# LLaVA-VL/LLaVA-Plus-Codebase

Measured on NVIDIA H100. Metric: prefill+decode tokens/s, higher is better.
Workload: dtype bf16

## Files before the change

llava-plus-codebase_b200/csrc/decode_mega.cu:

```cuda
#include <limits.h>
#include <math.h>

#include "common.cuh"
#include "kernels.h"

namespace b2 {
namespace {

constexpr int MK_CONS_WARPS = 16;
constexpr int MK_CONS = MK_CONS_WARPS * 32;
constexpr int MK_PROD_WARPS = 4;
constexpr int MK_THREADS = MK_CONS + 32 * MK_PROD_WARPS;
constexpr int MK_D = 128;
constexpr int MK_U = 4;
constexpr int MK_KT = 2048;
constexpr int MK_ROW_PAD = 64;
constexpr int MK_ROW_STRIDE = MK_KT * 2 + MK_ROW_PAD;
constexpr int MK_TILE_BYTES = 8 * MK_ROW_STRIDE;
constexpr int MK_MAXNB = 32;
constexpr int MK_MAXL = 48;
constexpr int MK_MAX_STAGES = 12;

__device__ __forceinline__ void unpack8(const uint4& u, float (&f)[8]) {
    f[0] = bf16_lo(u.x); f[1] = bf16_hi(u.x); f[2] = bf16_lo(u.y); f[3] = bf16_hi(u.y);
    f[4] = bf16_lo(u.z); f[5] = bf16_hi(u.z); f[6] = bf16_lo(u.w); f[7] = bf16_hi(u.w);
}
__device__ __forceinline__ uint4 ldcg16(const void* p) { return __ldcg(reinterpret_cast<const uint4*>(p)); }

__device__ __forceinline__ void cons_sync() { asm volatile("bar.sync 1, %0;" ::"n"(MK_CONS) : "memory"); }

__device__ __forceinline__ void grid_sync(unsigned int* counter, unsigned int target) {
    cons_sync();
    if (threadIdx.x == 0) {
        asm volatile("red.release.gpu.global.add.u32 [%0], 1;" ::"l"(counter) : "memory");
        unsigned int cur, spins = 0;
        do {
            asm volatile("ld.acquire.gpu.global.u32 %0, [%1];" : "=r"(cur) : "l"(counter) : "memory");
            if (++spins > (1u << 26)) asm volatile("trap;");
        } while ((int)(cur - target) < 0);
    }
    cons_sync();
}

__device__ __forceinline__ void bulk_g2s(void* smem_dst, const void* gsrc, uint32_t bytes, uint64_t* bar) {
    asm volatile("cp.async.bulk.shared::cluster.global.mbarrier::complete_tx::bytes [%0], [%1], %2, [%3];" ::"r"(
                     smem_u32(smem_dst)),
                 "l"(gsrc), "r"(bytes), "r"(smem_u32(bar))
                 : "memory");
}

struct GemvCtx {
    const __nv_bfloat16* W;
    int K, act;
    int u_lo, nu;
    int nb;
    int nchunk;
};
struct PhaseIO {
    const __nv_bfloat16* xin;
    const __nv_bfloat16* gamma;
    const __nv_bfloat16* residual;
    void* out;
    int ld_out, out_fp32;
};

__device__ __forceinline__ int mk_phys_row(const GemvCtx& c, int rb, int g, bool& valid) {
    if (c.act == ACT_SWIGLU) {
        const int lc = rb * 4 + (g & 3);
        valid = lc < c.nu;
        const int ch = c.u_lo + lc;
        return (ch >> 6) * 128 + (ch & 63) + ((g >> 2) ? 64 : 0);
    }
    const int lr = rb * 8 + g;
    valid = lr < c.nu;
    return c.u_lo + lr;
}

__device__ __forceinline__ int mk_rows_in_block(const GemvCtx& c, int rb) {
    if (c.act == ACT_SWIGLU) return 2 * min(4, c.nu - rb * 4);
    return min(8, c.nu - rb * 8);
}

__device__ __forceinline__ bool mk_is_attention(const MegaParams& p, int ph) { return ph % 5 == 1 && ph < 5 * p.L; }

__device__ __forceinline__ PhaseIO mk_phase_io(const MegaParams& p, const MegaLayer* layers, int ph) {
    PhaseIO c;
    const int l = ph / 5, k = ph % 5;
    c.gamma = nullptr; c.residual = nullptr; c.out_fp32 = 0;
    if (l >= p.L) { c.xin = p.x; c.gamma = p.final_norm; c.out = p.logits; c.ld_out = p.V; c.out_fp32 = 1; }
    else if (k <= 1) { c.xin = p.x; c.gamma = layers[l].ln1; c.out = p.qkv; c.ld_out = 3 * p.h; }
    else if (k == 2) { c.xin = p.attn; c.residual = p.x; c.out = p.x; c.ld_out = p.h; }
    else if (k == 3) { c.xin = p.x; c.gamma = layers[l].ln2; c.out = p.act; c.ld_out = p.I; }
    else { c.xin = p.act; c.residual = p.x; c.out = p.x; c.ld_out = p.h; }
    return c;
}
__device__ __forceinline__ GemvCtx mk_phase_ctx(const MegaParams& p, const MegaLayer* layers, int ph) {
    GemvCtx c;
    const int l = ph / 5, k = ph % 5;
    int N;
    c.act = ACT_NONE;
    if (l >= p.L) { c.W = p.lm_head; N = p.V; c.K = p.h; }
    else if (k <= 1) { c.W = layers[l].wqkv; N = 3 * p.h; c.K = p.h; }
    else if (k == 2) { c.W = layers[l].wo; N = p.h; c.K = p.h; }
    else if (k == 3) { c.W = layers[l].wgu; N = 2 * p.I; c.K = p.h; c.act = ACT_SWIGLU; }
    else { c.W = layers[l].wd; N = p.h; c.K = p.I; }
    const long long units = c.act == ACT_SWIGLU ? (N >> 1) : N;
    c.u_lo = (int)((units * blockIdx.x) / gridDim.x);
    c.nu = (int)((units * (blockIdx.x + 1)) / gridDim.x) - c.u_lo;
    c.nb = c.act == ACT_SWIGLU ? (c.nu + 3) >> 2 : (c.nu + 7) >> 3;
    c.nchunk = (c.K + MK_KT - 1) / MK_KT;
    return c;
}

template <int NB>
__device__ __forceinline__ void mk_prologue(const PhaseIO& c, int K, int B, float eps, int tid, int lane, int warp,
                                            __nv_bfloat16* xs, float (*s_red)[NB], float* s_rstd,
                                            const __nv_bfloat16* gamma_smem) {
    const int nvec = K >> 3;
    float ss[NB];
#pragma unroll
    for (int b = 0; b < NB; ++b) ss[b] = 0.f;
    for (int i = tid; i < nvec; i += MK_CONS) {
#pragma unroll
        for (int b = 0; b < NB; ++b) {
            uint4 u = make_uint4(0, 0, 0, 0);
            if (b < B) u = ldcg16(c.xin + (size_t)b * K + i * 8);
            *reinterpret_cast<uint4*>(xs + (size_t)b * K + i * 8) = u;
            if (c.gamma != nullptr) {
                float f[8];
                unpack8(u, f);
#pragma unroll
                for (int e = 0; e < 8; ++e) ss[b] += f[e] * f[e];
            }
        }
    }
    if (c.gamma != nullptr) {
#pragma unroll
        for (int b = 0; b < NB; ++b) {
            const float v = warp_sum(ss[b]);
            if (lane == 0) s_red[warp][b] = v;
        }
        cons_sync();
        if (tid < NB) {
            float t = 0.f;
            for (int i = 0; i < MK_CONS_WARPS; ++i) t += s_red[i][tid];
            s_rstd[tid] = rsqrtf(t / K + eps);
        }
        cons_sync();
        if (gamma_smem != nullptr) asm volatile("cp.async.wait_all;" ::: "memory");
        const __nv_bfloat16* gsrc = gamma_smem != nullptr ? gamma_smem : c.gamma;
        for (int i = tid; i < nvec; i += MK_CONS) {
            float gf[8];
            unpack8(*reinterpret_cast<const uint4*>(gsrc + i * 8), gf);
#pragma unroll
            for (int b = 0; b < NB; ++b) {
                uint4* px = reinterpret_cast<uint4*>(xs + (size_t)b * K + i * 8);
                float f[8], o[8];
                unpack8(*px, f);
                const float rstd = s_rstd[b];
#pragma unroll
                for (int e = 0; e < 8; ++e) o[e] = gf[e] * round_bf16(f[e] * rstd);
                *px = make_uint4(pack_bf16(o[0], o[1]), pack_bf16(o[2], o[3]), pack_bf16(o[4], o[5]),
                                 pack_bf16(o[6], o[7]));
            }
        }
    }
    cons_sync();
}

template <int NB>
__device__ __forceinline__ void mk_prologue_fast(const PhaseIO& c, int K, float eps, int tid, int lane, int warp,
                                                 __nv_bfloat16* xs, float (*s_red)[NB], const uint4 (&gpre)[2]) {
    const int nvec = K >> 3;
    if (c.gamma == nullptr) {
        constexpr int J = 3;
        for (int i0 = 0; i0 < nvec; i0 += J * MK_CONS) {
            uint4 u[NB][J];
#pragma unroll
            for (int j = 0; j < J; ++j) {
                const int idx = i0 + j * MK_CONS + tid;
#pragma unroll
                for (int b = 0; b < NB; ++b)
                    u[b][j] = idx < nvec ? ldcg16(c.xin + (size_t)b * K + idx * 8) : make_uint4(0, 0, 0, 0);
            }
#pragma unroll
            for (int j = 0; j < J; ++j) {
                const int idx = i0 + j * MK_CONS + tid;
                if (idx < nvec) {
#pragma unroll
                    for (int b = 0; b < NB; ++b) *reinterpret_cast<uint4*>(xs + (size_t)b * K + idx * 8) = u[b][j];
                }
            }
        }
        cons_sync();
        return;
    }
    uint4 u[NB][2];
    float ss[NB];
#pragma unroll
    for (int b = 0; b < NB; ++b) ss[b] = 0.f;
#pragma unroll
    for (int j = 0; j < 2; ++j) {
        const int idx = j * MK_CONS + tid;
#pragma unroll
        for (int b = 0; b < NB; ++b)
            u[b][j] = idx < nvec ? ldcg16(c.xin + (size_t)b * K + idx * 8) : make_uint4(0, 0, 0, 0);
    }
#pragma unroll
    for (int j = 0; j < 2; ++j) {
#pragma unroll
        for (int b = 0; b < NB; ++b) {
            float f[8];
            unpack8(u[b][j], f);
#pragma unroll
            for (int e = 0; e < 8; ++e) ss[b] += f[e] * f[e];
        }
    }
#pragma unroll
    for (int b = 0; b < NB; ++b) {
        const float v = warp_sum(ss[b]);
        if (lane == 0) s_red[warp][b] = v;
    }
    cons_sync();
    float rstd[NB];
#pragma unroll
    for (int b = 0; b < NB; ++b) {
        float t = 0.f;
#pragma unroll
        for (int i = 0; i < MK_CONS_WARPS; ++i) t += s_red[i][b];
        rstd[b] = rsqrtf(t / K + eps);
    }
#pragma unroll
    for (int j = 0; j < 2; ++j) {
        const int idx = j * MK_CONS + tid;
        if (idx < nvec) {
            float gf[8];
            unpack8(gpre[j], gf);
#pragma unroll
            for (int b = 0; b < NB; ++b) {
                float f[8], o[8];
                unpack8(u[b][j], f);
#pragma unroll
                for (int e = 0; e < 8; ++e) o[e] = gf[e] * round_bf16(f[e] * rstd[b]);
                *reinterpret_cast<uint4*>(xs + (size_t)b * K + idx * 8) =
                    make_uint4(pack_bf16(o[0], o[1]), pack_bf16(o[2], o[3]), pack_bf16(o[4], o[5]), pack_bf16(o[6], o[7]));
            }
        }
    }
    cons_sync();
}

__device__ __forceinline__ bool mk_gamma_preload(const MegaParams& p, const MegaLayer* layers, int ph, int n_phases,
                                                 int tid, uint4 (&gpre)[2]) {
    if (ph >= n_phases || mk_is_attention(p, ph)) return false;
    const PhaseIO io = mk_phase_io(p, layers, ph);
    const int nvec = p.h >> 3;
    if (io.gamma == nullptr || nvec > 2 * MK_CONS) return false;
#pragma unroll
    for (int j = 0; j < 2; ++j) {
        const int idx = j * MK_CONS + tid;
        gpre[j] = idx < nvec ? __ldg(reinterpret_cast<const uint4*>(io.gamma) + idx) : make_uint4(0, 0, 0, 0);
    }
    return true;
}

__device__ __forceinline__ void mk_mma(float (&c)[4], uint32_t a0, uint32_t a2, uint32_t b0, uint32_t b1) {
    asm volatile(
        "mma.sync.aligned.m16n8k16.row.col.f32.bf16.bf16.f32 {%0,%1,%2,%3}, {%4,%5,%6,%7}, {%8,%9}, {%0,%1,%2,%3};"
        : "+f"(c[0]), "+f"(c[1]), "+f"(c[2]), "+f"(c[3])
        : "r"(a0), "r"(0u), "r"(a2), "r"(0u), "r"(b0), "r"(b1));
}

template <int NB>
__device__ __forceinline__ float mk_row_value(const float* s_gpart, int rb, int b, int r) {
    float v = 0.f;
#pragma unroll
    for (int ww = 0; ww < MK_CONS_WARPS; ++ww) v += s_gpart[(((size_t)ww * MK_MAXNB + rb) * NB + b) * 8 + r];
    return v;
}

template <int NB>
__device__ __forceinline__ void mk_epilogue(const MegaParams& p, const MegaLayer* layers, int ph, const GemvCtx& c,
                                            int B, int tid, const float* s_gpart, float res_pref, bool have_res_pref) {
    const PhaseIO io = mk_phase_io(p, layers, ph);
    if (c.act == ACT_SWIGLU) {
        const int nch = c.nu;
        for (int idx = tid; idx < nch * B; idx += MK_CONS) {
            const int b = idx / nch, r = idx - b * nch;
            const int rb = r >> 2, q = r & 3;
            const float gt = mk_row_value<NB>(s_gpart, rb, b, q);
            const float up = mk_row_value<NB>(s_gpart, rb, b, q + 4);
            reinterpret_cast<__nv_bfloat16*>(io.out)[(size_t)b * io.ld_out + (size_t)c.u_lo + r] =
                __float2bfloat16_rn(gt / (1.0f + __expf(-gt)) * up);
        }
    } else {
        const int nr = c.nu;
        for (int idx = tid; idx < nr * B; idx += MK_CONS) {
            const int b = idx / nr, r = idx - b * nr;
            float y = mk_row_value<NB>(s_gpart, r >> 3, b, r & 7);
            const size_t o = (size_t)b * io.ld_out + (size_t)c.u_lo + r;
            if (io.residual != nullptr) y += have_res_pref ? res_pref : __bfloat162float(__ldcg(io.residual + o));
            if (io.out_fp32) reinterpret_cast<float*>(io.out)[o] = y;
            else reinterpret_cast<__nv_bfloat16*>(io.out)[o] = __float2bfloat16_rn(y);
        }
    }
}

__device__ __forceinline__ void mk_attention(const MegaParams& p, const MegaLayer& Lw, int tid, int lane, int warp,
                                             float (*s_part)[MK_D + 2], int* s_flag, const float* s_cos,
                                             const float* s_sin) {
    const int h = p.h, H = p.H;
    const int pairs = p.B * H;
    const int grid = gridDim.x;
    const int G = pairs <= grid ? grid / pairs : 1;
    const int hw = lane >> 4, c = lane & 15;
    const int split = pairs <= grid ? (int)blockIdx.x % G : 0;
    for (int pair = pairs <= grid ? (int)blockIdx.x / G : (int)blockIdx.x; pair < pairs;
         pair += (pairs <= grid ? pairs : grid)) {
        const int head = pair % H, b = pair / H;
        const int pos = p.cur_len[b];
        const int total = pos + 1;
        const int cchunk = (total + G - 1) / G;
        const int cb = split * cchunk;
        const int ce = min(cb + cchunk, total);
        const int wchunk = (max(ce - cb, 0) + MK_CONS_WARPS - 1) / MK_CONS_WARPS;
        const int k_begin = cb + warp * wchunk;
        const int k_end = min(k_begin + wchunk, ce);
        const __nv_bfloat16* qrow = p.qkv + (size_t)b * 3 * h + head * MK_D;
        float qreg[8], knew[8], vnew[8];
        {
            float qa[8], qb[8], ka[8], kb[8];
            unpack8(ldcg16(qrow + c * 8), qa);
            unpack8(ldcg16(qrow + (c ^ 8) * 8), qb);
            unpack8(ldcg16(qrow + h + c * 8), ka);
            unpack8(ldcg16(qrow + h + (c ^ 8) * 8), kb);
            unpack8(ldcg16(qrow + 2 * h + c * 8), vnew);
            const float sign = (c < 8) ? -1.f : 1.f;
#pragma unroll
            for (int e = 0; e < 8; ++e) {
                const int i = ((c & 7) * 8 + e);
                const float cbf = s_cos[b * 64 + i], sbf = s_sin[b * 64 + i];
                qreg[e] = round_bf16(round_bf16(qa[e] * cbf) + round_bf16(sign * qb[e] * sbf));
                knew[e] = round_bf16(round_bf16(ka[e] * cbf) + round_bf16(sign * kb[e] * sbf));
            }
        }
        const size_t cbase = ((size_t)b * H + head) * p.Smax * MK_D;
        if (pos >= k_begin && pos < k_end && hw == 0) {
            *reinterpret_cast<uint4*>(Lw.kcache + cbase + (size_t)pos * MK_D + c * 8) =
                make_uint4(pack_bf16(knew[0], knew[1]), pack_bf16(knew[2], knew[3]),
                           pack_bf16(knew[4], knew[5]), pack_bf16(knew[6], knew[7]));
            *reinterpret_cast<uint4*>(Lw.vcache + cbase + (size_t)pos * MK_D + c * 8) =
                make_uint4(pack_bf16(vnew[0], vnew[1]), pack_bf16(vnew[2], vnew[3]),
                           pack_bf16(vnew[4], vnew[5]), pack_bf16(vnew[6], vnew[7]));
        }
        float m_run = -INFINITY, l_run = 0.f, av[8];
#pragma unroll
        for (int e = 0; e < 8; ++e) av[e] = 0.f;
        const __nv_bfloat16* kb_ = Lw.kcache + cbase + c * 8;
        const __nv_bfloat16* vb_ = Lw.vcache + cbase + c * 8;
        for (int kbase = k_begin; kbase < k_end; kbase += 2 * MK_U) {
            uint4 kraw[MK_U], vraw[MK_U];
#pragma unroll
            for (int u = 0; u < MK_U; ++u) {
                const int key = kbase + hw + 2 * u;
                if (key < k_end && key != pos) {
                    kraw[u] = ld_stream_16(kb_ + (size_t)key * MK_D);
                    vraw[u] = ld_stream_16(vb_ + (size_t)key * MK_D);
                } else {
                    kraw[u] = make_uint4(0, 0, 0, 0);
                    vraw[u] = make_uint4(0, 0, 0, 0);
                }
            }
#pragma unroll
            for (int u = 0; u < MK_U; ++u) {
                const int key = kbase + hw + 2 * u;
                float kf[8], vf[8];
                unpack8(kraw[u], kf);
                unpack8(vraw[u], vf);
                if (key == pos) {
#pragma unroll
                    for (int e = 0; e < 8; ++e) { kf[e] = knew[e]; vf[e] = vnew[e]; }
                }
                float dot = 0.f;
#pragma unroll
                for (int e = 0; e < 8; ++e) dot += qreg[e] * kf[e];
                dot += __shfl_xor_sync(0xffffffffu, dot, 8);
                dot += __shfl_xor_sync(0xffffffffu, dot, 4);
                dot += __shfl_xor_sync(0xffffffffu, dot, 2);
                dot += __shfl_xor_sync(0xffffffffu, dot, 1);
                if (key < k_end) {
                    const float sc = dot * p.scale_log2;
                    const float m_new = fmaxf(m_run, sc);
                    const float corr = exp2f(m_run - m_new);
                    const float pr = exp2f(sc - m_new);
                    l_run = l_run * corr + pr;
#pragma unroll
                    for (int e = 0; e < 8; ++e) av[e] = av[e] * corr + pr * vf[e];
                    m_run = m_new;
                }
            }
        }
        {
            const float m_o = __shfl_xor_sync(0xffffffffu, m_run, 16);
            const float l_o = __shfl_xor_sync(0xffffffffu, l_run, 16);
            const float m_c = fmaxf(m_run, m_o);
            const float w_s = (m_run == -INFINITY) ? 0.f : exp2f(m_run - m_c);
            const float w_o = (m_o == -INFINITY) ? 0.f : exp2f(m_o - m_c);
#pragma unroll
            for (int e = 0; e < 8; ++e) {
                const float a_o = __shfl_xor_sync(0xffffffffu, av[e], 16);
                av[e] = av[e] * w_s + a_o * w_o;
            }
            l_run = l_run * w_s + l_o * w_o;
            m_run = m_c;
        }
        if (hw == 0) {
#pragma unroll
            for (int e = 0; e < 8; ++e) s_part[warp][c * 8 + e] = av[e];
            if (c == 0) { s_part[warp][MK_D] = m_run; s_part[warp][MK_D + 1] = l_run; }
        }
        cons_sync();
        float m_cta = -INFINITY, l_cta = 0.f, o_cta = 0.f;
        if (tid < MK_D) {
#pragma unroll
            for (int i = 0; i < MK_CONS_WARPS; ++i) m_cta = fmaxf(m_cta, s_part[i][MK_D]);
#pragma unroll
            for (int i = 0; i < MK_CONS_WARPS; ++i) {
                const float ms = s_part[i][MK_D];
                const float wgt = (ms == -INFINITY) ? 0.f : exp2f(ms - m_cta);
                l_cta += s_part[i][MK_D + 1] * wgt;
                o_cta += s_part[i][tid] * wgt;
            }
        }
        if (G == 1) {
            if (tid < MK_D) p.attn[(size_t)b * h + head * MK_D + tid] = __float2bfloat16_rn(o_cta / l_cta);
        } else {
            float* part = p.attn_partial + ((size_t)pair * G + split) * (MK_D + 2);
            if (tid < MK_D) {
                part[tid] = o_cta;
                if (tid == 0) { part[MK_D] = m_cta; part[MK_D + 1] = l_cta; }
            }
            __threadfence();
            cons_sync();
            if (tid == 0) *s_flag = (atomicAdd(&p.attn_counters[pair], 1) == G - 1) ? 1 : 0;
            cons_sync();
            if (*s_flag) {
                __threadfence();
                if (tid < MK_D) {
                    const float* pb = p.attn_partial + (size_t)pair * G * (MK_D + 2);
                    float m_all = -INFINITY;
                    for (int sidx = 0; sidx < G; ++sidx) m_all = fmaxf(m_all, __ldcg(pb + (size_t)sidx * (MK_D + 2) + MK_D));
                    float l_all = 0.f, o_all = 0.f;
                    for (int sidx = 0; sidx < G; ++sidx) {
                        const float ms = __ldcg(pb + (size_t)sidx * (MK_D + 2) + MK_D);
                        const float wgt = (ms == -INFINITY) ? 0.f : exp2f(ms - m_all);
                        l_all += __ldcg(pb + (size_t)sidx * (MK_D + 2) + MK_D + 1) * wgt;
                        o_all += __ldcg(pb + (size_t)sidx * (MK_D + 2) + tid) * wgt;
                    }
                    p.attn[(size_t)b * h + head * MK_D + tid] = __float2bfloat16_rn(o_all / l_all);
                    if (tid == 0) p.attn_counters[pair] = 0;
                }
            }
        }
        cons_sync();
    }
}

struct TileCursor {
    GemvCtx c;
    int ph, rb, kc;
    uint32_t tile;
    bool valid;
};
__device__ __forceinline__ void cursor_seek(TileCursor& t, const MegaParams& p, const MegaLayer* layers, int n_phases) {
    while (t.ph < n_phases) {
        if (!mk_is_attention(p, t.ph)) {
            t.c = mk_phase_ctx(p, layers, t.ph);
            if (t.c.nb > 0) { t.rb = 0; t.kc = 0; t.valid = true; return; }
        }
        ++t.ph;
    }
    t.valid = false;
}
__device__ __forceinline__ void cursor_begin(TileCursor& t, const MegaParams& p, const MegaLayer* layers, int n_phases) {
    t.ph = 0; t.tile = 0; t.rb = 0; t.kc = 0;
    cursor_seek(t, p, layers, n_phases);
}
__device__ __forceinline__ void cursor_next(TileCursor& t, const MegaParams& p, const MegaLayer* layers, int n_phases) {
    ++t.tile;
    if (++t.kc < t.c.nchunk) return;
    t.kc = 0;
    if (++t.rb < t.c.nb) return;
    ++t.ph;
    cursor_seek(t, p, layers, n_phases);
}
__device__ __forceinline__ void prefetch_l2_line(const void* gsrc) {
    asm volatile("prefetch.global.L2 [%0];" ::"l"(gsrc) : "memory");
}
__device__ __forceinline__ void bulk_prefetch_l2(const void* gsrc, uint32_t bytes) {
    asm volatile("cp.async.bulk.prefetch.L2.global [%0], %1;" ::"l"(gsrc), "r"(bytes) : "memory");
}

template <int NB>
__global__ void __launch_bounds__(MK_THREADS, 1) decode_mega_kernel(MegaParams p, int n_stages) {
    extern __shared__ __align__(128) uint8_t mk_smem[];
    uint8_t* ring = mk_smem;
    __nv_bfloat16* xs = reinterpret_cast<__nv_bfloat16*>(ring + (size_t)n_stages * MK_TILE_BYTES);
    float* s_gpart = reinterpret_cast<float*>(reinterpret_cast<uint8_t*>(xs) + (size_t)NB * (p.h > p.I ? p.h : p.I) * 2);
    uint64_t* full_bar = reinterpret_cast<uint64_t*>(s_gpart + (size_t)MK_CONS_WARPS * MK_MAXNB * NB * 8);
    uint64_t* empty_bar = full_bar + MK_MAX_STAGES;
    __shared__ float s_red[MK_CONS_WARPS][NB];
    __shared__ float s_rstd[NB];
    __shared__ float s_av[MK_CONS_WARPS];
    __shared__ int s_ai[MK_CONS_WARPS];
    __shared__ float s_part[MK_CONS_WARPS][MK_D + 2];
    __shared__ int s_flag;
    __shared__ float s_cos[NB * 64], s_sin[NB * 64];
    __shared__ __align__(16) MegaLayer s_layers[MK_MAXL];

    const int tid = threadIdx.x, lane = tid & 31, warp = tid >> 5;
    const int B = p.B;
    const int n_phases = 5 * p.L + 1;

    {
        const uint4* src = reinterpret_cast<const uint4*>(p.layers);
        uint4* dst = reinterpret_cast<uint4*>(s_layers);
        for (int i = tid; i < p.L * (int)(sizeof(MegaLayer) / 16); i += MK_THREADS) dst[i] = src[i];
        if (tid == 0) {
            for (int s = 0; s < n_stages; ++s) {
                mbar_init(&full_bar[s], 1);
                mbar_init(&empty_bar[s], MK_CONS_WARPS);
            }
            fence_barrier_init();
        }
        __syncthreads();
    }

    if (warp >= MK_CONS_WARPS) {
        const uint32_t pw = (uint32_t)(warp - MK_CONS_WARPS);
        const uint32_t ahead = (uint32_t)p.l2_ahead;
        TileCursor cp, pf;
        cursor_begin(cp, p, s_layers, n_phases);
        cursor_begin(pf, p, s_layers, n_phases);
        while (cp.valid) {
            if (cp.tile % (uint32_t)MK_PROD_WARPS == pw) {
                if (ahead != 0) {
                    while (pf.valid && pf.tile < cp.tile + ahead) cursor_next(pf, p, s_layers, n_phases);
                    if (pf.valid) {
                        const uint32_t pbytes = (uint32_t)min(MK_KT, pf.c.K - pf.kc * MK_KT) * 2u;
                        if (p.l2_mode == 2) {
                            bool pvalid;
                            const int pfrow = mk_phys_row(pf.c, pf.rb, lane & 7, pvalid);
                            if (lane < 8 && pvalid)
                                bulk_prefetch_l2(pf.c.W + (size_t)pfrow * pf.c.K + (size_t)pf.kc * MK_KT, pbytes);
                        } else {
                            bool pvalid;
                            const int pfrow = mk_phys_row(pf.c, pf.rb, lane >> 2, pvalid);
                            if (pvalid) {
                                const char* base = reinterpret_cast<const char*>(pf.c.W + (size_t)pfrow * pf.c.K +
                                                                                 (size_t)pf.kc * MK_KT);
                                for (uint32_t off = (uint32_t)(lane & 3) * 128u; off < pbytes; off += 512u)
                                    prefetch_l2_line(base + off);
                            }
                        }
                    }
                }
                const uint32_t stage = cp.tile % (uint32_t)n_stages;
                const uint32_t parity = (cp.tile / (uint32_t)n_stages) & 1u;
                const uint32_t row_bytes = (uint32_t)min(MK_KT, cp.c.K - cp.kc * MK_KT) * 2u;
                if (lane == 0) {
                    mbar_wait(&empty_bar[stage], parity ^ 1u);
                    mbar_arrive_expect_tx(&full_bar[stage], (uint32_t)mk_rows_in_block(cp.c, cp.rb) * row_bytes);
                }
                __syncwarp();
                bool row_valid;
                const int prow = mk_phys_row(cp.c, cp.rb, lane & 7, row_valid);
                if (lane < 8 && row_valid)
                    bulk_g2s(ring + (size_t)stage * MK_TILE_BYTES + (size_t)lane * MK_ROW_STRIDE,
                             cp.c.W + (size_t)prow * cp.c.K + (size_t)cp.kc * MK_KT, row_bytes, &full_bar[stage]);
            }
            cursor_next(cp, p, s_layers, n_phases);
        }
        return;
    }

    for (int i = tid; i < B * 64; i += MK_CONS) {
        const int b = i >> 6, f = i & 63;
        const float inv_freq = exp2f(-(2.0f * f / MK_D) * log2f(p.theta));
        float sv, cv;
        sincosf((float)p.cur_len[b] * inv_freq, &sv, &cv);
        s_cos[i] = round_bf16(cv);
        s_sin[i] = round_bf16(sv);
    }
    if (blockIdx.x < B) {
        int t = p.tok[blockIdx.x];
        t = t < 0 ? 0 : (t >= p.V ? p.V - 1 : t);
        const uint4* src = reinterpret_cast<const uint4*>(p.embed + (size_t)t * p.h);
        uint4* dst = reinterpret_cast<uint4*>(p.x + (size_t)blockIdx.x * p.h);
        for (int i = tid; i < p.h / 8; i += MK_CONS) dst[i] = src[i];
    }
    uint4 gpre[2] = {make_uint4(0, 0, 0, 0), make_uint4(0, 0, 0, 0)};
    bool gpre_ok = p.fast_prologue != 0 && mk_gamma_preload(p, s_layers, 0, n_phases, tid, gpre);
    __nv_bfloat16* gsm = xs + (size_t)NB * p.h;
    const bool gsm_fits = p.gamma_smem != 0 && (size_t)(NB + 1) * p.h <= (size_t)NB * (p.h > p.I ? p.h : p.I);
    auto gamma_prefetch = [&](int ph) -> bool {
        if (!gsm_fits || ph >= n_phases || mk_is_attention(p, ph)) return false;
        const PhaseIO io = mk_phase_io(p, s_layers, ph);
        if (io.gamma == nullptr) return false;
        for (int i = tid; i < (p.h >> 3); i += MK_CONS)
            asm volatile("cp.async.cg.shared.global [%0], [%1], 16;" ::"r"(smem_u32(gsm + i * 8)), "l"(io.gamma + i * 8) : "memory");
        asm volatile("cp.async.commit_group;" ::: "memory");
        return true;
    };
    bool gsm_ok = gamma_prefetch(0);
    unsigned int bar_target = p.bar_base + gridDim.x;
    grid_sync(p.bar_count, bar_target);

    const bool tracing = p.trace != nullptr && blockIdx.x == 0 && tid == 0;
    const int g = lane >> 2, t4 = lane & 3;
    uint32_t tile = 0;
#pragma unroll 1
    for (int ph = 0; ph < n_phases; ++ph) {
        if (tracing) p.trace[ph * 4 + 0] = clock64();
        if (mk_is_attention(p, ph)) {
            mk_attention(p, s_layers[ph / 5], tid, lane, warp, s_part, &s_flag, s_cos, s_sin);
        } else {
            const GemvCtx c = mk_phase_ctx(p, s_layers, ph);
            const PhaseIO io = mk_phase_io(p, s_layers, ph);
            const bool have_res = io.residual != nullptr && c.nu * B <= MK_CONS;
            float res_pref = 0.f;
            if (have_res && tid < c.nu * B) {
                const int b = tid / c.nu, r = tid - b * c.nu;
                res_pref = __bfloat162float(__ldcg(io.residual + (size_t)b * io.ld_out + (size_t)c.u_lo + r));
            }
            if (p.fast_prologue != 0 && (io.gamma == nullptr || gpre_ok))
                mk_prologue_fast<NB>(io, c.K, p.eps, tid, lane, warp, xs, s_red, gpre);
            else
                mk_prologue<NB>(io, c.K, B, p.eps, tid, lane, warp, xs, s_red, s_rstd, gsm_ok ? gsm : nullptr);
            if (tracing) p.trace[ph * 4 + 1] = clock64();
#pragma unroll 1
            for (int rb = 0; rb < c.nb; ++rb) {
                float acc[4] = {0.f, 0.f, 0.f, 0.f}, acc2[4] = {0.f, 0.f, 0.f, 0.f};
#pragma unroll 1
                for (int kc = 0; kc < c.nchunk; ++kc, ++tile) {
                    const uint32_t stage = tile % (uint32_t)n_stages;
                    const uint32_t parity = (tile / (uint32_t)n_stages) & 1u;
                    const int nk32 = min(MK_KT, c.K - kc * MK_KT) >> 5;
                    mbar_wait(&full_bar[stage], parity);
                    const uint8_t* trow = ring + (size_t)stage * MK_TILE_BYTES + (size_t)g * MK_ROW_STRIDE + t4 * 16;
                    const __nv_bfloat16* xrow = xs + (size_t)g * c.K + (size_t)kc * MK_KT + t4 * 8;
#pragma unroll 4
                    for (int k32 = warp; k32 < nk32; k32 += MK_CONS_WARPS) {
                        const uint4 wv = *reinterpret_cast<const uint4*>(trow + k32 * 64);
                        uint4 xv = make_uint4(0, 0, 0, 0);
                        if (g < B) xv = *reinterpret_cast<const uint4*>(xrow + k32 * 32);
                        mk_mma(acc, xv.x, xv.y, wv.x, wv.y);
                        mk_mma(acc2, xv.z, xv.w, wv.z, wv.w);
                    }
                    __syncwarp();
                    if (lane == 0) mbar_arrive(&empty_bar[stage]);
                }
                if (g < NB)
                    *reinterpret_cast<float2*>(s_gpart + (((size_t)warp * MK_MAXNB + rb) * NB + g) * 8 + t4 * 2) =
                        make_float2(acc[0] + acc2[0], acc[1] + acc2[1]);
            }
            cons_sync();
            if (tracing) p.trace[ph * 4 + 2] = clock64();
            mk_epilogue<NB>(p, s_layers, ph, c, B, tid, s_gpart, res_pref, have_res);
        }
        if (tracing) p.trace[ph * 4 + 3] = clock64();
        gpre_ok = p.fast_prologue != 0 && mk_gamma_preload(p, s_layers, ph + 1, n_phases, tid, gpre);
        gsm_ok = gamma_prefetch(ph + 1);
        bar_target += gridDim.x;
        grid_sync(p.bar_count, bar_target);
    }
    if (tracing) p.trace[n_phases * 4] = clock64();

    if (blockIdx.x < B) {
        const int b = blockIdx.x;
        const float* row = p.logits + (size_t)b * p.V;
        float best = -INFINITY;
        int bi = INT_MAX;
        for (int i = tid; i < p.V; i += MK_CONS) {
            const float v = __ldcg(row + i);
            if (v == v && (bi == INT_MAX || v > best)) { best = v; bi = i; }
        }
#pragma unroll
        for (int o = 16; o > 0; o >>= 1) {
            const float ov = __shfl_xor_sync(0xffffffffu, best, o);
            const int oi = __shfl_xor_sync(0xffffffffu, bi, o);
            if (ov > best || (ov == best && oi < bi)) { best = ov; bi = oi; }
        }
        if (lane == 0) { s_av[warp] = best; s_ai[warp] = bi; }
        cons_sync();
        if (warp == 0) {
            best = lane < MK_CONS_WARPS ? s_av[lane] : -INFINITY;
            bi = lane < MK_CONS_WARPS ? s_ai[lane] : INT_MAX;
#pragma unroll
            for (int o = 16; o > 0; o >>= 1) {
                const float ov = __shfl_xor_sync(0xffffffffu, best, o);
                const int oi = __shfl_xor_sync(0xffffffffu, bi, o);
                if (ov > best || (ov == best && oi < bi)) { best = ov; bi = oi; }
            }
            if (lane == 0) {
                const int tk = bi == INT_MAX ? 0 : bi;
                p.tok[b] = tk;
                p.out_tokens[(size_t)(*p.step_counter) * B + b] = tk;
                if (p.rows == nullptr || p.rows[b].active) p.cur_len[b] += 1;
                if (p.ring != nullptr) {
                    const int pub = p.sstate->pub_counter, tag0 = p.sstate->tag;
                    if (tag0 != 0) {
                        const int tag = 1 + (tag0 - 1 + pub / p.ring_cap) % 2047;
                        reinterpret_cast<volatile int32_t*>(p.ring)[(size_t)(pub % p.ring_cap) * B + b] = (tag << 20) | (tk & 0xFFFFF);
                        __threadfence_system();
                    }
                }
            }
        }
    }
    cons_sync();
    if (tid == 0) {
        __threadfence();
        if (atomicAdd(p.done_count, 1u) == gridDim.x - 1) {
            *p.done_count = 0u;
            *p.step_counter += 1;
            if (p.ring != nullptr) p.sstate->pub_counter += 1;
        }
    }
}

size_t mega_fixed_bytes(int NB, int h, int I) {
    return (size_t)NB * (h > I ? h : I) * 2 + (size_t)MK_CONS_WARPS * MK_MAXNB * NB * 8 * 4 + 2 * MK_MAX_STAGES * 8;
}
size_t mega_static_bytes(int NB) {
    return (size_t)(MK_CONS_WARPS + 1) * NB * 4 + MK_CONS_WARPS * (MK_D + 2 + 2) * 4 + NB * 512 +
           MK_MAXL * sizeof(MegaLayer) + 1024;
}
int mega_stages(int NB, int h, int I) {
    const long long avail = 227 * 1024 - (long long)mega_fixed_bytes(NB, h, I) - (long long)mega_static_bytes(NB);
    long long s = avail / MK_TILE_BYTES;
    return (int)(s > MK_MAX_STAGES ? MK_MAX_STAGES : s);
}

}

bool decode_mega_fits(int B, int h, int I) {
    if (B < 1 || B > 2) return false;
    return mega_stages(B, h, I) >= 4;
}

int decode_mega(const MegaParams& p, cudaStream_t stream) {
    B2_CHECK_ARG(p.B >= 1 && p.B <= 2, "decode_mega: batch must be 1..2");
    B2_CHECK_ARG(p.L <= MK_MAXL, "decode_mega: %d layers exceed the shared layer table (%d)", p.L, MK_MAXL);
    B2_CHECK_ARG(p.h % 256 == 0 && p.I % 256 == 0 && p.V % 8 == 0 && p.h / p.H == MK_D,
                 "decode_mega: unsupported dims h=%d I=%d V=%d H=%d", p.h, p.I, p.V, p.H);
    {
        const int grid = num_sms();
        const int nmax = p.V > 3 * p.h ? (p.V > 2 * p.I ? p.V : 2 * p.I) : (3 * p.h > 2 * p.I ? 3 * p.h : 2 * p.I);
        B2_CHECK_ARG((nmax / 8 + grid - 1) / grid + 1 <= MK_MAXNB,
                     "decode_mega: %d output rows per CTA exceed the shared-memory block table", nmax / grid);
    }
    const int NB = p.B;
    const int stages = mega_stages(NB, p.h, p.I);
    B2_CHECK_ARG(stages >= 4, "decode_mega: shared memory too small for the weight ring (B=%d h=%d I=%d)", p.B, p.h, p.I);
    const size_t smem = (size_t)stages * MK_TILE_BYTES + mega_fixed_bytes(NB, p.h, p.I);
    void* fn = NB == 1 ? (void*)decode_mega_kernel<1> : (void*)decode_mega_kernel<2>;
    static size_t attr_smem[3] = {0, 0, 0};
    if (smem > attr_smem[NB]) {
        B2_CUDA_CHECK(cudaFuncSetAttribute(fn, cudaFuncAttributeMaxDynamicSharedMemorySize, (int)smem));
        attr_smem[NB] = smem;
    }
    MegaParams pp = p;
    int n_stages = stages;
    void* args[] = {&pp, &n_stages};
    B2_CUDA_CHECK(cudaLaunchCooperativeKernel(fn, dim3(num_sms()), dim3(MK_THREADS), args, smem, stream));
    B2_LAUNCH_CHECK();
    return 0;
}

}
```

llava-plus-codebase_b200/csrc/kernels.h:

```cpp
#pragma once
#include <cuda_bf16.h>
#include <cuda_runtime.h>
#include <stdint.h>

namespace b2 {

enum { ACT_NONE = 0, ACT_QUICK_GELU = 1, ACT_GELU_ERF = 2, ACT_SWIGLU = 3, ACT_ROPE_QKV = 4 };

struct RopeQkv {
    const void* table = nullptr;
    void* kcache = nullptr;
    void* vcache = nullptr;
    int S = 0, H = 0, Smax = 0;
    const int32_t* pos0 = nullptr;
};
enum { DT_BF16 = 0, DT_F16 = 1, DT_F32 = 2 };

int num_sms();

struct GemmArgs {
    const void* A = nullptr; int lda = 0;
    const void* W = nullptr; int ldw = 0;
    const void* bias = nullptr;
    const void* residual = nullptr; int ld_res = 0;
    void* out = nullptr; int ld_out = 0; int out_fp32 = 0;
    int M = 0, N = 0, K = 0;
    int act = ACT_NONE;
    int bn_override = 0;
    RopeQkv rope;
};
int gemm_bf16(const GemmArgs& g, cudaStream_t stream);
int projector_fused_bf16(const void* X, int ldx, const void* W1, const void* b1, const void* W2, const void* b2, void* H,
                         void* out, int ld_out, int M, int K1, int N1, int N2, int* row_done, cudaStream_t stream);
int gemm_bf16_2cta(const GemmArgs& g, cudaStream_t stream);

struct SkinnyArgs {
    const void* x = nullptr; int ldx = 0;
    const void* W = nullptr; int ldw = 0;
    const void* residual = nullptr; int ld_res = 0;
    void* out = nullptr; int ld_out = 0; int out_fp32 = 0;
    int B = 0, N = 0, K = 0;
    int act = ACT_NONE;
    float* partial = nullptr; size_t partial_bytes = 0;
    int* counters = nullptr;
    const float* w_scale = nullptr;
    const float* x_scale = nullptr;
};
int gemm_skinny_bf16(const SkinnyArgs& g, cudaStream_t stream);
int gemm_skinny_fp8(const SkinnyArgs& g, cudaStream_t stream);
size_t gemm_skinny_workspace_bytes(int B, int N, int K);
size_t gemm_skinny_counter_bytes(int N);

int quantize_rows_e4m3(const void* x, int64_t ldx, int rows, int K, void* q, int64_t ldq, float* scale, cudaStream_t stream);
int rmsnorm_quant_e4m3(const void* x, int64_t x_row_stride, const void* gamma, void* q, int64_t ldq, float* scale, int rows,
                       int cols, float eps, cudaStream_t stream);

struct GemvArgs {
    const void* x = nullptr; int64_t ldx = 0;
    const void* W = nullptr; int ldw = 0;
    const void* norm_gamma = nullptr; float eps = 0.f;
    const void* residual = nullptr; int ld_res = 0;
    void* out = nullptr; int ld_out = 0; int out_fp32 = 0;
    int B = 0, N = 0, K = 0;
    int act = ACT_NONE;
};
int gemv_bf16(const GemvArgs& g, cudaStream_t stream);
bool gemv_fits(int B, int N, int K, int act);

int quantize_nf4(const void* w, int64_t ldw, int N, int K, void* q, float* absmax, int gemv_order, cudaStream_t stream);
struct Nf4Matrix {
    const void* q = nullptr; const float* absmax = nullptr;
    void* out = nullptr;
    int N = 0, K = 0;
};
int dequantize_nf4(const Nf4Matrix* mats, int n, int gemv_order, cudaStream_t stream);
int gemv_nf4(const GemvArgs& g, const void* q, const float* absmax, cudaStream_t stream);
bool gemv_nf4_fits(int B, int N, int K, int act);

int layernorm_bf16(const void* x, const void* gamma, const void* beta, void* y, int rows, int cols, float eps,
                   cudaStream_t stream);
int rmsnorm_bf16(const void* x, int64_t x_row_stride, const void* gamma, void* y, int rows, int cols, float eps,
                 cudaStream_t stream);
int rmsnorm_gather_bf16(const void* x, const int32_t* row_index, const void* gamma, void* y, int rows, int cols,
                        float eps, cudaStream_t stream);

int vit_im2col(const void* pixels, void* out, int B, int img, int patch, int kpad, cudaStream_t stream);
int vit_embed_ln(const void* patch_out, const void* cls, const void* pos, const void* gamma, const void* beta,
                 void* hidden, int B, int P, int D, float eps, cudaStream_t stream);
int vit_drop_cls(const void* hidden, void* out, int B, int P, int D, cudaStream_t stream);

struct FlashArgs {
    const void* q = nullptr; int64_t q_bs = 0, q_ts = 0, q_hs = 0;
    const void* k = nullptr; int64_t k_bs = 0, k_ts = 0, k_hs = 0;
    const void* v = nullptr; int64_t v_bs = 0, v_ts = 0, v_hs = 0;
    void* o = nullptr;       int64_t o_bs = 0, o_ts = 0, o_hs = 0;
    const int32_t* seq_lens = nullptr;
    const int32_t* pos0 = nullptr;
    int Skv = 0;
    int B = 0, H = 0, S = 0, D = 0;
    int causal = 0;
    float scale = 1.f;
};
int flash_attn_bf16(const FlashArgs& a, cudaStream_t stream);
int flash_attn_tc_bf16(const FlashArgs& a, cudaStream_t stream);
int flash_attn_mma_bf16(const FlashArgs& a, cudaStream_t stream);

int rope_table_build(void* table, int Smax, int D, float theta, cudaStream_t stream);
int rope_kv_write(void* qkv, void* kcache, void* vcache, int B, int S, int H, int D, int Smax, float theta,
                  cudaStream_t stream, const int32_t* pos0 = nullptr);

struct DecodeAttnArgs {
    const void* qkv = nullptr;
    void* kcache = nullptr; void* vcache = nullptr;
    float* kscale = nullptr; float* vscale = nullptr;
    const int32_t* cur_len = nullptr;
    void* out = nullptr;
    float* partial = nullptr;
    int32_t* counters = nullptr;
    int B = 0, H = 0, D = 128, Smax = 0, nsplit = 1;
    float theta = 10000.f, scale = 1.f;
};
int decode_attn_ctas_per_sm();
int decode_attn_bf16(const DecodeAttnArgs& a, cudaStream_t stream);
int decode_attn_e4m3_ctas_per_sm();
int decode_attn_e4m3(const DecodeAttnArgs& a, cudaStream_t stream);
int kv_quantize_e4m3(const void* ksrc, const void* vsrc, void* k8, void* v8, float* kscale, float* vscale,
                     const int32_t* seq_lens, int B, int S, int H, int D, int Smax, cudaStream_t stream,
                     const int32_t* pos0 = nullptr, int S_src = 0);
int kv_dequantize_e4m3(const void* k8, const void* v8, const float* kscale, const float* vscale, const int32_t* pos0, void* kdst,
                       void* vdst, int B, int H, int Smax, int S_dst, cudaStream_t stream);

struct MegaLayer {
    const __nv_bfloat16 *ln1, *wqkv, *wo, *ln2, *wgu, *wd;
    __nv_bfloat16 *kcache, *vcache;
};
struct MegaParams {
    const MegaLayer* layers = nullptr;
    int L = 0, h = 0, I = 0, H = 0, V = 0, B = 0, Smax = 0, nsplit = 1;
    const __nv_bfloat16 *embed = nullptr, *final_norm = nullptr, *lm_head = nullptr;
    int32_t *tok = nullptr, *cur_len = nullptr, *out_tokens = nullptr, *step_counter = nullptr;
    __nv_bfloat16 *x = nullptr, *qkv = nullptr, *attn = nullptr, *act = nullptr;
    float* logits = nullptr;
    float* attn_partial = nullptr;
    int32_t* attn_counters = nullptr;
    unsigned int *bar_count = nullptr, *done_count = nullptr;
    unsigned int bar_base = 0;
    float eps = 1e-5f, theta = 10000.f, scale_log2 = 1.f;
    int l2_ahead = 0;
    int l2_mode = 1;
    int fast_prologue = 0;
    int gamma_smem = 0;
    long long* trace = nullptr;
    struct SampleState* sstate = nullptr;
    int32_t* ring = nullptr;
    int ring_cap = 0;
    const struct RowState* rows = nullptr;
};
int decode_mega(const MegaParams& p, cudaStream_t stream);
bool decode_mega_fits(int B, int h, int I);

struct SampleState {
    int do_sample;
    float temperature, top_p;
    int top_k;
    unsigned long long seed;
    int tag;
    int pub_counter;
    unsigned int done;
    int per_row;
};
struct RowState {
    int active;
    int do_sample; float temperature, top_p; int top_k;
    unsigned long long seed;
    int index;
};
enum { SP_SELECT = 1,
       SP_WRITE_OUT = 2,
       SP_BUMP = 4 };
int sample_state_set(SampleState* st_dev, const SampleState& v, cudaStream_t stream);
int sample_publish(const float* logits, int V, int B, SampleState* st_dev, RowState* rows_dev, int32_t* tok, int32_t* out_tokens,
                   int32_t* step_counter, int32_t* cur_len, int32_t* ring_dev, int ring_cap, int flags, int step_offset,
                   cudaStream_t stream);
int row_state_set(RowState* row_dev, const RowState& v, int32_t* tok_dev, int token, cudaStream_t stream);

size_t beam_topk_workspace_bytes(int B, int nb, int K);
int beam_topk(const float* logits, const int32_t* row_of_beam, const float* beam_scores, int B, int nb, int V, int K,
              void* workspace, float* out_scores, int32_t* out_tokens, int32_t* out_beams, cudaStream_t stream);
struct KvCopyPairs {
    static constexpr int kMax = 64;
    int32_t src[kMax], dst[kMax], end[kMax];
};
int kv_copy_slots(void* k, void* v, float* kscale, float* vscale, const int32_t* src, const int32_t* dst, const int32_t* end, int n,
                  int row_begin, int L, int H, int max_batch, int pitch, int row_bytes, int32_t* len_dev, cudaStream_t stream);

struct PreprocessArgs {
    const uint8_t* img = nullptr; int H = 0, W = 0;
    int pad_top = 0, pad_left = 0; uint8_t bg[3] = {0, 0, 0};
    const int32_t *h_bounds = nullptr, *h_kk = nullptr; int h_ksize = 0, h_identity = 0;
    const int32_t *v_bounds = nullptr, *v_kk = nullptr; int v_ksize = 0, v_identity = 0;
    int y0 = 0, rows = 0;
    int x_lo = 0, y_lo = 0;
    int cols = 0, out = 0;
    uint8_t* tmp = nullptr;
    float mean[3] = {0, 0, 0}, stdv[3] = {1, 1, 1}, rescale = 1.f / 255.f;
    void* pixels = nullptr;
    uint8_t* u8_out = nullptr;
};
int preprocess_clip_image(const PreprocessArgs& a, cudaStream_t stream);

int splice_embed(const int32_t* src_index, const void* table, const void* feats, void* out, int rows, int h, int vocab,
                 int n_feat_rows, int* err_flag, cudaStream_t stream);
int splice_index(const long long* ids, int B, int Lt, int k_per_row, const int32_t* feat_offsets_host, int n_img, int image_token,
                 int S, int32_t* src_index, int* err_flag, cudaStream_t stream);
int embed_tokens(const int32_t* tokens, const void* table, void* out, int rows, int h, int vocab, int* err_flag,
                 cudaStream_t stream);
enum { B2_ERR_TOKEN_RANGE = 1, B2_ERR_IMAGE_ROW_RANGE = 2, B2_ERR_SPLICE_SLOTS = 4 };
int argmax_f32(const float* logits, int B, int V, int32_t* out, cudaStream_t stream);
struct I32Pack { int32_t v[128]; };
int set_i32_pairs(int32_t* dst_a, const int32_t* a_host, int32_t* dst_b, const int32_t* b_host, int n, cudaStream_t stream);
int add_i32(int32_t* x, int n, int delta, cudaStream_t stream);
int convert_to_bf16(const void* src, int src_dtype, void* dst, int64_t n, cudaStream_t stream);
int interleave_gate_up(const void* gate, const void* up, void* out, int I, int h, cudaStream_t stream);
int store_token(const int32_t* src, int32_t* dst_base, const int32_t* step_counter, int B, cudaStream_t stream);

}
```

llava-plus-codebase_b200/csrc/model.cu:

```cuda
#include <cuda_fp16.h>
#include <limits.h>
#include <stdarg.h>
#include <stdio.h>
#include <stdlib.h>
#include <string.h>
#include <time.h>

#include <atomic>
#include <utility>
#include <mutex>
#include <string>
#include <vector>

#include "../../include/b2llava.h"
#include "common.cuh"
#include "kernels.h"

namespace b2 {

static thread_local char g_err[1024] = {0};
unsigned long long g_launch_count = 0;

bool pdl_enabled() {
    const char* e = getenv("B2_PDL");
    return !(e != nullptr && e[0] == '0');
}

void set_error(const char* fmt, ...) {
    va_list ap;
    va_start(ap, fmt);
    vsnprintf(g_err, sizeof(g_err), fmt, ap);
    va_end(ap);
}

namespace {
typedef __nv_bfloat16 bf16;

struct DevBuf {
    void* p = nullptr;
    size_t bytes = 0;
    int alloc(size_t n) {
        free();
        if (n == 0) return 0;
        cudaError_t e = cudaMalloc(&p, n);
        if (e != cudaSuccess) {
            p = nullptr;
            set_error("cudaMalloc(%zu bytes) failed: %s", n, cudaGetErrorString(e));
            return -2;
        }
        bytes = n;
        return 0;
    }
    void free() {
        if (p) cudaFree(p);
        p = nullptr;
        bytes = 0;
    }
    template <typename T>
    T* as() const { return reinterpret_cast<T*>(p); }
};

struct VitLayer {
    DevBuf ln1_g, ln1_b, wqkv, bqkv, wo, bo, ln2_g, ln2_b, w1, b1, w2, b2;
    unsigned qkv_w = 0, qkv_b = 0;
};
struct LlamaLayer {
    DevBuf ln1, wqkv, wo, ln2, wgu, wd;
    unsigned qkv_parts = 0;
    DevBuf wqkv8, wo8, wgu8, wd8, s_qkv, s_o, s_gu, s_d;
    DevBuf tmp_gate, tmp_up;
    DevBuf q_qkv, a_qkv, q_o, a_o, q_gu, a_gu, q_d, a_d;
    bool has_gate = false, has_up = false;
};
}
}

using namespace b2;

struct b2_model {
    b2_model_desc d;
    int device = 0;
    std::mutex mu;
    bool finalized = false;
    int P = 0, T = 0, kpad = 0, vit_live = 0, vit_hd = 64, hd = 128;
    DevBuf patch_w, cls, pos, pre_g, pre_b;
    std::vector<VitLayer> vit;
    DevBuf p0_w, p0_b, p2_w, p2_b;
    DevBuf embed, final_norm, lm_head;
    std::vector<LlamaLayer> ll;
    int* err_host = nullptr;
    int* err_dev = nullptr;
    cudaEvent_t ws_event = nullptr;
    cudaStream_t ws_stream = nullptr;
    bool ws_valid = false;
    DevBuf v_col, v_patch, v_hidden, v_xn, v_qkv, v_attn, v_mlp, v_feats, p_mid, p_done;
    DevBuf x, xn, qkv, attn, act, last_idx, xlast, logits, splice_idx;
    DevBuf chunk_pos;
    DevBuf enc_pixels, enc_out;
    std::vector<cudaGraphExec_t> enc_graph;
    std::vector<char> enc_warm;
    cudaStream_t enc_stream = nullptr;
    cudaEvent_t enc_fork = nullptr, enc_join = nullptr;
    int enc_launches = 0;
    bool fp8_decode = false;
    DevBuf lm_head8, s_head, xq8, xscale;
    DevBuf kstage, vstage;
    bool nf4 = false;
    DevBuf nf4_scratch;
    std::atomic<int> kv_live{0};
};

struct b2_kv {
    b2_model* m = nullptr;
    int max_batch = 0, max_seq = 0;
    int dtype = B2_KV_BF16;
    int pitch = 0;
    DevBuf k, v;
    DevBuf kscale, vscale;
    DevBuf len_dev, tok, step_counter, out_tokens, attn_partial, attn_counters;
    DevBuf sk_partial, sk_counters;
    std::vector<int32_t> len_host;
    int out_capacity = 0;
    cudaGraphExec_t graph = nullptr;
    int graph_B = 0;
    unsigned int mega_bar_base = 0;
    DevBuf mega_layers, mega_sync;
    DevBuf rope_tab;
    cudaStream_t own_stream = nullptr;
    cudaEvent_t ev_fork = nullptr, ev_join = nullptr;
    int warm_B = 0;
    DevBuf sstate;
    SampleState samp_host = {};
    bool samp_valid = false;
    int32_t* ring_host = nullptr;
    int32_t* ring_dev = nullptr;
    int ring_cap = 0;
    int epoch = 0;
    int stream_B = 0, stream_tag = 0, stream_scheduled = 0;
    DevBuf rows_dev;
    std::vector<RowState> rows_host;
    DevBuf beam_in, beam_ws, beam_out;
    bool counted = false;
    bool e4m3() const { return dtype == B2_KV_E4M3; }
    size_t elem_bytes() const { return e4m3() ? 1 : 2; }
    size_t layer_rows() const { return (size_t)max_batch * m->d.heads * pitch; }
    size_t layer_stride() const { return layer_rows() * m->hd; }
    char* k_layer(int l) const { return k.as<char>() + (size_t)l * layer_stride() * elem_bytes(); }
    char* v_layer(int l) const { return v.as<char>() + (size_t)l * layer_stride() * elem_bytes(); }
};

namespace {

bool starts_with(const std::string& s, const char* p) { return s.rfind(p, 0) == 0; }

int ingest(const void* src, int dtype, void* dst, int64_t n, cudaStream_t st) {
    if (dtype == DT_BF16) {
        B2_CUDA_CHECK(cudaMemcpyAsync(dst, src, (size_t)n * 2, cudaMemcpyDefault, st));
        B2_CUDA_CHECK(cudaStreamSynchronize(st));
        return 0;
    }
    const size_t esz = dtype == DT_F32 ? 4 : 2;
    cudaPointerAttributes attr;
    bool on_device = false;
    if (cudaPointerGetAttributes(&attr, src) == cudaSuccess)
        on_device = attr.type == cudaMemoryTypeDevice || attr.type == cudaMemoryTypeManaged;
    else
        cudaGetLastError();
    DevBuf tmp;
    const void* dsrc = src;
    if (!on_device) {
        B2_TRY(tmp.alloc((size_t)n * esz));
        B2_CUDA_CHECK(cudaMemcpy(tmp.p, src, (size_t)n * esz, cudaMemcpyDefault));
        dsrc = tmp.p;
    }
    int r = convert_to_bf16(dsrc, dtype, dst, n, st);
    cudaError_t e = cudaStreamSynchronize(st);
    tmp.free();
    if (r != 0) return r;
    B2_CUDA_CHECK(e);
    return 0;
}

int64_t numel(const int64_t* shape, int ndim) {
    int64_t n = 1;
    for (int i = 0; i < ndim; ++i) n *= shape[i];
    return n;
}

int expect_shape(const char* key, const int64_t* shape, int ndim, int64_t a, int64_t b = -1) {
    const int64_t n = numel(shape, ndim);
    const int64_t want = b < 0 ? a : a * b;
    bool ok = n == want;
    if (ok && b >= 0 && ndim >= 2) ok = shape[0] == a;
    if (!ok) {
        set_error("set_weight(%s): unexpected shape (numel %lld, expected %lld x %lld)", key, (long long)n,
                  (long long)a, (long long)(b < 0 ? 1 : b));
        return -1;
    }
    return 0;
}

int put(DevBuf& buf, size_t total_elems, size_t off, const void* src, int dtype, int64_t n) {
    if (buf.p == nullptr) B2_TRY(buf.alloc(total_elems * 2));
    return ingest(src, dtype, buf.as<bf16>() + off, n, 0);
}

int gemm(const void* A, int lda, const void* W, int ldw, const void* bias, const void* res, int ld_res, void* out,
         int ld_out, int out_fp32, int M, int N, int K, int act, cudaStream_t st) {
    GemmArgs g;
    g.A = A; g.lda = lda; g.W = W; g.ldw = ldw; g.bias = bias; g.residual = res; g.ld_res = ld_res;
    g.out = out; g.ld_out = ld_out; g.out_fp32 = out_fp32; g.M = M; g.N = N; g.K = K; g.act = act;
    return gemm_bf16(g, st);
}

int gemv(const void* x, int64_t ldx, const void* W, int ldw, const void* gamma, float eps, const void* res,
         int ld_res, void* out, int ld_out, int out_fp32, int B, int N, int K, int act, cudaStream_t st) {
    GemvArgs g;
    g.x = x; g.ldx = ldx; g.W = W; g.ldw = ldw; g.norm_gamma = gamma; g.eps = eps; g.residual = res;
    g.ld_res = ld_res; g.out = out; g.ld_out = ld_out; g.out_fp32 = out_fp32; g.B = B; g.N = N; g.K = K;
    g.act = act;
    return gemv_bf16(g, st);
}

int skinny(b2_kv* kv, const void* x, int ldx, const void* W, int ldw, const void* res, int ld_res, void* out, int ld_out,
           int out_fp32, int B, int N, int K, int act, cudaStream_t st) {
    SkinnyArgs g;
    g.x = x; g.ldx = ldx; g.W = W; g.ldw = ldw; g.residual = res; g.ld_res = ld_res;
    g.out = out; g.ld_out = ld_out; g.out_fp32 = out_fp32; g.B = B; g.N = N; g.K = K; g.act = act;
    g.partial = kv->sk_partial.as<float>(); g.partial_bytes = kv->sk_partial.bytes;
    g.counters = kv->sk_counters.as<int>();
    return gemm_skinny_bf16(g, st);
}
int skinny8(b2_model* m, b2_kv* kv, const void* W8, const float* w_scale, const void* res, int ld_res, void* out, int ld_out,
            int out_fp32, int B, int N, int K, int act, cudaStream_t st) {
    SkinnyArgs g;
    g.x = m->xq8.p; g.ldx = K; g.W = W8; g.ldw = K; g.residual = res; g.ld_res = ld_res;
    g.out = out; g.ld_out = ld_out; g.out_fp32 = out_fp32; g.B = B; g.N = N; g.K = K; g.act = act;
    g.partial = kv->sk_partial.as<float>(); g.partial_bytes = kv->sk_partial.bytes;
    g.counters = kv->sk_counters.as<int>();
    g.w_scale = w_scale; g.x_scale = m->xscale.as<float>();
    return gemm_skinny_fp8(g, st);
}
bool use_skinny(const b2_kv* kv, int B) {
    const char* e0 = getenv("B2_DECODE_SKINNY");
    const int lo = (e0 != nullptr && e0[0] == '3') ? 3 : 7;
    if (B < lo || B > 128 || kv->sk_partial.p == nullptr) return false;
    const char* e = getenv("B2_DECODE_SKINNY");
    return !(e != nullptr && e[0] == '0');
}

struct LayerW { const void *wqkv, *wo, *wgu, *wd; };
int layer_weights(b2_model* m, int l, LayerW* w, cudaStream_t st) {
    LlamaLayer& L = m->ll[l];
    if (!m->nf4) { *w = {L.wqkv.p, L.wo.p, L.wgu.p, L.wd.p}; return 0; }
    const int h = m->d.hidden, I = m->d.inter;
    bf16* s = m->nf4_scratch.as<bf16>();
    Nf4Matrix mt[4];
    const DevBuf* q[4] = {&L.q_qkv, &L.q_o, &L.q_gu, &L.q_d};
    const DevBuf* a[4] = {&L.a_qkv, &L.a_o, &L.a_gu, &L.a_d};
    const int N[4] = {3 * h, h, 2 * I, h}, K[4] = {h, h, h, I};
    bf16* out = s;
    for (int i = 0; i < 4; ++i) {
        mt[i].q = q[i]->p; mt[i].absmax = a[i]->as<float>(); mt[i].out = out; mt[i].N = N[i]; mt[i].K = K[i];
        out += (size_t)N[i] * K[i];
    }
    B2_TRY(dequantize_nf4(mt, 4, 1, st));
    *w = {mt[0].out, mt[1].out, mt[2].out, mt[3].out};
    return 0;
}
bool use_gemv_nf4(const b2_model* m, int B) {
    const int h = m->d.hidden, I = m->d.inter;
    return m->nf4 && B <= 8 && gemv_nf4_fits(B, 3 * h, h, ACT_NONE) && gemv_nf4_fits(B, h, h, ACT_NONE) &&
           gemv_nf4_fits(B, 2 * I, h, ACT_SWIGLU) && gemv_nf4_fits(B, h, I, ACT_NONE);
}
int gemv4(const void* x, int64_t ldx, const DevBuf& q, const DevBuf& a, const void* gamma, float eps, const void* res, int ld_res,
          void* out, int ld_out, int B, int N, int K, int act, cudaStream_t st) {
    GemvArgs g;
    g.x = x; g.ldx = ldx; g.norm_gamma = gamma; g.eps = eps; g.residual = res; g.ld_res = ld_res;
    g.out = out; g.ld_out = ld_out; g.B = B; g.N = N; g.K = K; g.act = act;
    return gemv_nf4(g, q.p, a.as<float>(), st);
}

int decode_nsplit(int B, int H, int max_seq, int ctas_per_sm) {
    const char* e = getenv("B2_DECODE_NSPLIT");
    if (e != nullptr && atoi(e) >= 1) return atoi(e) > 32 ? 32 : atoi(e);
    const int cap = ctas_per_sm * num_sms();
    int n = cap / (B * H);
    if (n < 3) n = 3;
    if (n > 16) n = 16;
    const int n_hi = max_seq / 64;
    if (n > n_hi) n = n_hi < 1 ? 1 : n_hi;
    return n;
}

int set_vision_weight(b2_model* m, const std::string& k, const void* ptr, const int64_t* shape, int ndim, int dt) {
    const int D = m->d.vit_hidden, I = m->d.vit_inter;
    const char* key = k.c_str();
    if (k == "embeddings.class_embedding") {
        B2_TRY(expect_shape(key, shape, ndim, D));
        return put(m->cls, D, 0, ptr, dt, D);
    }
    if (k == "embeddings.patch_embedding.weight") {
        const int kk = 3 * m->d.patch_size * m->d.patch_size;
        B2_TRY(expect_shape(key, shape, ndim, D, kk));
        DevBuf tmp;
        B2_TRY(tmp.alloc((size_t)D * kk * 2));
        B2_TRY(ingest(ptr, dt, tmp.p, (int64_t)D * kk, 0));
        if (m->patch_w.p == nullptr) B2_TRY(m->patch_w.alloc((size_t)D * m->kpad * 2));
        B2_CUDA_CHECK(cudaMemset(m->patch_w.p, 0, (size_t)D * m->kpad * 2));
        B2_CUDA_CHECK(cudaMemcpy2D(m->patch_w.p, (size_t)m->kpad * 2, tmp.p, (size_t)kk * 2, (size_t)kk * 2, D,
                                   cudaMemcpyDeviceToDevice));
        return 0;
    }
    if (k == "embeddings.position_embedding.weight") {
        B2_TRY(expect_shape(key, shape, ndim, m->T, D));
        return put(m->pos, (size_t)m->T * D, 0, ptr, dt, (int64_t)m->T * D);
    }
    if (k == "embeddings.position_ids") return 0;
    if (k == "pre_layrnorm.weight") { B2_TRY(expect_shape(key, shape, ndim, D)); return put(m->pre_g, D, 0, ptr, dt, D); }
    if (k == "pre_layrnorm.bias") { B2_TRY(expect_shape(key, shape, ndim, D)); return put(m->pre_b, D, 0, ptr, dt, D); }
    if (starts_with(k, "post_layernorm.")) return 0;
    if (starts_with(k, "encoder.layers.")) {
        int li = -1, consumed = 0;
        if (sscanf(key, "encoder.layers.%d.%n", &li, &consumed) != 1 || li < 0 || li >= m->d.vit_layers) {
            set_error("set_weight: bad vision layer index in '%s'", key);
            return -1;
        }
        if (li >= m->vit_live) return 0;
        VitLayer& L = m->vit[li];
        const std::string s = k.substr(consumed);
        if (s == "layer_norm1.weight") { B2_TRY(expect_shape(key, shape, ndim, D)); return put(L.ln1_g, D, 0, ptr, dt, D); }
        if (s == "layer_norm1.bias") { B2_TRY(expect_shape(key, shape, ndim, D)); return put(L.ln1_b, D, 0, ptr, dt, D); }
        if (s == "layer_norm2.weight") { B2_TRY(expect_shape(key, shape, ndim, D)); return put(L.ln2_g, D, 0, ptr, dt, D); }
        if (s == "layer_norm2.bias") { B2_TRY(expect_shape(key, shape, ndim, D)); return put(L.ln2_b, D, 0, ptr, dt, D); }
        const char* names[3] = {"self_attn.q_proj.", "self_attn.k_proj.", "self_attn.v_proj."};
        for (int j = 0; j < 3; ++j) {
            if (starts_with(s, names[j])) {
                if (s == std::string(names[j]) + "weight") {
                    B2_TRY(expect_shape(key, shape, ndim, D, D));
                    B2_TRY(put(L.wqkv, (size_t)3 * D * D, (size_t)j * D * D, ptr, dt, (int64_t)D * D));
                    L.qkv_w |= 1u << j;
                    return 0;
                }
                if (s != std::string(names[j]) + "bias") break;
                B2_TRY(expect_shape(key, shape, ndim, D));
                B2_TRY(put(L.bqkv, (size_t)3 * D, (size_t)j * D, ptr, dt, D));
                L.qkv_b |= 1u << j;
                return 0;
            }
        }
        if (s == "self_attn.out_proj.weight") { B2_TRY(expect_shape(key, shape, ndim, D, D)); return put(L.wo, (size_t)D * D, 0, ptr, dt, (int64_t)D * D); }
        if (s == "self_attn.out_proj.bias") { B2_TRY(expect_shape(key, shape, ndim, D)); return put(L.bo, D, 0, ptr, dt, D); }
        if (s == "mlp.fc1.weight") { B2_TRY(expect_shape(key, shape, ndim, I, D)); return put(L.w1, (size_t)I * D, 0, ptr, dt, (int64_t)I * D); }
        if (s == "mlp.fc1.bias") { B2_TRY(expect_shape(key, shape, ndim, I)); return put(L.b1, I, 0, ptr, dt, I); }
        if (s == "mlp.fc2.weight") { B2_TRY(expect_shape(key, shape, ndim, D, I)); return put(L.w2, (size_t)D * I, 0, ptr, dt, (int64_t)D * I); }
        if (s == "mlp.fc2.bias") { B2_TRY(expect_shape(key, shape, ndim, D)); return put(L.b2, D, 0, ptr, dt, D); }
    }
    set_error("set_weight: unknown vision key '%s'", key);
    return -1;
}

int set_llama_layer_weight(b2_model* m, int li, const std::string& s, const char* key, const void* ptr,
                           const int64_t* shape, int ndim, int dt) {
    const int h = m->d.hidden, I = m->d.inter;
    LlamaLayer& L = m->ll[li];
    if (m->nf4 && (starts_with(s, "self_attn.") || starts_with(s, "mlp.")) && s != "self_attn.rotary_emb.inv_freq") {
        set_error("set_weight(%s): the decoder Linears of this model are NF4 (b2_model_enable_nf4); they cannot be reloaded", key);
        return -1;
    }
    if (s == "input_layernorm.weight") { B2_TRY(expect_shape(key, shape, ndim, h)); return put(L.ln1, h, 0, ptr, dt, h); }
    if (s == "post_attention_layernorm.weight") { B2_TRY(expect_shape(key, shape, ndim, h)); return put(L.ln2, h, 0, ptr, dt, h); }
    const char* names[3] = {"self_attn.q_proj.weight", "self_attn.k_proj.weight", "self_attn.v_proj.weight"};
    for (int j = 0; j < 3; ++j) {
        if (s == names[j]) {
            B2_TRY(expect_shape(key, shape, ndim, h, h));
            B2_TRY(put(L.wqkv, (size_t)3 * h * h, (size_t)j * h * h, ptr, dt, (int64_t)h * h));
            L.qkv_parts |= 1u << j;
            return 0;
        }
    }
    if (s == "self_attn.o_proj.weight") { B2_TRY(expect_shape(key, shape, ndim, h, h)); return put(L.wo, (size_t)h * h, 0, ptr, dt, (int64_t)h * h); }
    if (s == "mlp.down_proj.weight") { B2_TRY(expect_shape(key, shape, ndim, h, I)); return put(L.wd, (size_t)h * I, 0, ptr, dt, (int64_t)h * I); }
    if (s == "mlp.gate_proj.weight" || s == "mlp.up_proj.weight") {
        B2_TRY(expect_shape(key, shape, ndim, I, h));
        const bool is_gate = s == "mlp.gate_proj.weight";
        DevBuf& tmp = is_gate ? L.tmp_gate : L.tmp_up;
        B2_TRY(put(tmp, (size_t)I * h, 0, ptr, dt, (int64_t)I * h));
        (is_gate ? L.has_gate : L.has_up) = true;
        if (L.has_gate && L.has_up) {
            if (L.wgu.p == nullptr) B2_TRY(L.wgu.alloc((size_t)2 * I * h * 2));
            B2_TRY(interleave_gate_up(L.tmp_gate.p, L.tmp_up.p, L.wgu.p, I, h, 0));
            B2_CUDA_CHECK(cudaStreamSynchronize(0));
            L.tmp_gate.free();
            L.tmp_up.free();
            L.has_gate = L.has_up = false;
        }
        return 0;
    }
    if (s == "self_attn.rotary_emb.inv_freq") return 0;
    set_error("set_weight: unknown decoder key '%s'", key);
    return -1;
}

int vit_forward_chunk(b2_model* m, const void* pixels, int B, void* out_feats, cudaStream_t st) {
    const b2_model_desc& d = m->d;
    const int D = d.vit_hidden, I = d.vit_inter, H = d.vit_heads, P = m->P, T = m->T;
    const int rows = B * T;
    B2_TRY(vit_im2col(pixels, m->v_col.p, B, d.image_size, d.patch_size, m->kpad, st));
    B2_TRY(gemm(m->v_col.p, m->kpad, m->patch_w.p, m->kpad, nullptr, nullptr, 0, m->v_patch.p, D, 0, B * P, D,
                m->kpad, ACT_NONE, st));
    B2_TRY(vit_embed_ln(m->v_patch.p, m->cls.p, m->pos.p, m->pre_g.p, m->pre_b.p, m->v_hidden.p, B, P, D,
                        d.vit_ln_eps, st));
    for (int l = 0; l < m->vit_live; ++l) {
        VitLayer& L = m->vit[l];
        B2_TRY(layernorm_bf16(m->v_hidden.p, L.ln1_g.p, L.ln1_b.p, m->v_xn.p, rows, D, d.vit_ln_eps, st));
        B2_TRY(gemm(m->v_xn.p, D, L.wqkv.p, D, L.bqkv.p, nullptr, 0, m->v_qkv.p, 3 * D, 0, rows, 3 * D, D,
                    ACT_NONE, st));
        FlashArgs fa;
        bf16* qkv = m->v_qkv.as<bf16>();
        fa.q = qkv;         fa.q_bs = (int64_t)T * 3 * D; fa.q_ts = 3 * D; fa.q_hs = m->vit_hd;
        fa.k = qkv + D;     fa.k_bs = fa.q_bs; fa.k_ts = 3 * D; fa.k_hs = m->vit_hd;
        fa.v = qkv + 2 * D; fa.v_bs = fa.q_bs; fa.v_ts = 3 * D; fa.v_hs = m->vit_hd;
        fa.o = m->v_attn.p; fa.o_bs = (int64_t)T * D; fa.o_ts = D; fa.o_hs = m->vit_hd;
        fa.B = B; fa.H = H; fa.S = T; fa.D = m->vit_hd; fa.causal = 0;
        fa.scale = 1.0f / sqrtf((float)m->vit_hd);
        B2_TRY(flash_attn_bf16(fa, st));
        B2_TRY(gemm(m->v_attn.p, D, L.wo.p, D, L.bo.p, m->v_hidden.p, D, m->v_hidden.p, D, 0, rows, D, D, ACT_NONE,
                    st));
        B2_TRY(layernorm_bf16(m->v_hidden.p, L.ln2_g.p, L.ln2_b.p, m->v_xn.p, rows, D, d.vit_ln_eps, st));
        B2_TRY(gemm(m->v_xn.p, D, L.w1.p, D, L.b1.p, nullptr, 0, m->v_mlp.p, I, 0, rows, I, D, ACT_QUICK_GELU, st));
        B2_TRY(gemm(m->v_mlp.p, I, L.w2.p, I, L.b2.p, m->v_hidden.p, D, m->v_hidden.p, D, 0, rows, D, I, ACT_NONE,
                    st));
    }
    B2_TRY(vit_drop_cls(m->v_hidden.p, out_feats, B, P, D, st));
    return 0;
}

int project_rows(b2_model* m, const void* feats, int rows, void* out, cudaStream_t st) {
    const int D = m->d.vit_hidden, h = m->d.hidden;
    const int max_rows = m->d.max_images * m->P;
    for (int r0 = 0; r0 < rows; r0 += max_rows) {
        const int n = rows - r0 < max_rows ? rows - r0 : max_rows;
        const bf16* a = reinterpret_cast<const bf16*>(feats) + (size_t)r0 * D;
        bf16* o = reinterpret_cast<bf16*>(out) + (size_t)r0 * h;
        const char* pf = getenv("B2_PROJECTOR_FUSED");
        if (!(pf != nullptr && pf[0] == '0')) {
            B2_TRY(projector_fused_bf16(a, D, m->p0_w.p, m->p0_b.p, m->p2_w.p, m->p2_b.p, m->p_mid.p, o, h, n, D, h, h,
                                        m->p_done.as<int>(), st));
        } else {
            B2_TRY(gemm(a, D, m->p0_w.p, D, m->p0_b.p, nullptr, 0, m->p_mid.p, h, 0, n, h, D, ACT_GELU_ERF, st));
            B2_TRY(gemm(m->p_mid.p, h, m->p2_w.p, h, m->p2_b.p, nullptr, 0, o, h, 0, n, h, h, ACT_NONE, st));
        }
    }
    return 0;
}

int encode_chunk(b2_model* m, const void* pixels, int n, void* out, cudaStream_t st) {
    const b2_model_desc& d = m->d;
    const char* eg = getenv("B2_ENCODE_GRAPH");
    if (eg != nullptr && eg[0] == '0') {
        B2_TRY(vit_forward_chunk(m, pixels, n, m->v_feats.p, st));
        return project_rows(m, m->v_feats.p, n * m->P, out, st);
    }
    const size_t in_bytes = (size_t)n * 3 * d.image_size * d.image_size * 2, out_bytes = (size_t)n * m->P * d.hidden * 2;
    cudaStream_t run = st;
    if (st == nullptr || st == cudaStreamLegacy) {
        if (m->enc_stream == nullptr) {
            B2_CUDA_CHECK(cudaStreamCreateWithFlags(&m->enc_stream, cudaStreamNonBlocking));
            B2_CUDA_CHECK(cudaEventCreateWithFlags(&m->enc_fork, cudaEventDisableTiming));
            B2_CUDA_CHECK(cudaEventCreateWithFlags(&m->enc_join, cudaEventDisableTiming));
        }
        B2_CUDA_CHECK(cudaEventRecord(m->enc_fork, st));
        B2_CUDA_CHECK(cudaStreamWaitEvent(m->enc_stream, m->enc_fork, 0));
        run = m->enc_stream;
    }
    B2_CUDA_CHECK(cudaMemcpyAsync(m->enc_pixels.p, pixels, in_bytes, cudaMemcpyDeviceToDevice, run));
    if (!m->enc_warm[n]) {
        B2_TRY(vit_forward_chunk(m, m->enc_pixels.p, n, m->v_feats.p, run));
        B2_TRY(project_rows(m, m->v_feats.p, n * m->P, m->enc_out.p, run));
        m->enc_warm[n] = 1;
    } else {
        if (m->enc_graph[n] == nullptr) {
            cudaGraph_t graph = nullptr;
            B2_CUDA_CHECK(cudaStreamBeginCapture(run, cudaStreamCaptureModeThreadLocal));
            const unsigned long long launches_before = g_launch_count;
            int r = vit_forward_chunk(m, m->enc_pixels.p, n, m->v_feats.p, run);
            if (r == 0) r = project_rows(m, m->v_feats.p, n * m->P, m->enc_out.p, run);
            m->enc_launches = (int)(g_launch_count - launches_before);
            g_launch_count = launches_before;
            cudaError_t e = cudaStreamEndCapture(run, &graph);
            if (r != 0) { if (graph) cudaGraphDestroy(graph); return r; }
            B2_CUDA_CHECK(e);
            e = cudaGraphInstantiate(&m->enc_graph[n], graph, 0);
            cudaGraphDestroy(graph);
            B2_CUDA_CHECK(e);
        }
        B2_CUDA_CHECK(cudaGraphLaunch(m->enc_graph[n], run));
        g_launch_count += (unsigned long long)m->enc_launches;
    }
    B2_CUDA_CHECK(cudaMemcpyAsync(out, m->enc_out.p, out_bytes, cudaMemcpyDeviceToDevice, run));
    if (run != st) {
        B2_CUDA_CHECK(cudaEventRecord(m->enc_join, run));
        B2_CUDA_CHECK(cudaStreamWaitEvent(st, m->enc_join, 0));
    }
    return 0;
}

int decode_step_launch(b2_model* m, b2_kv* kv, int B, cudaStream_t st) {
    const b2_model_desc& d = m->d;
    const int h = d.hidden, I = d.inter, H = d.heads, V = d.vocab;
    const int nsplit = decode_nsplit(B, H, kv->max_seq, kv->e4m3() ? decode_attn_e4m3_ctas_per_sm() : decode_attn_ctas_per_sm());
    B2_TRY(embed_tokens(kv->tok.as<int32_t>(), m->embed.p, m->x.p, B, h, V, m->err_dev, st));
    const bool small4 = use_gemv_nf4(m, B);
    const bool sk = !small4 && use_skinny(kv, B);
    const bool small = !m->nf4 && !sk && B <= 8 && gemv_fits(B, h, I, ACT_NONE) && gemv_fits(B, 2 * I, h, ACT_SWIGLU) &&
                       gemv_fits(B, 3 * h, h, ACT_NONE) && gemv_fits(B, V, h, ACT_NONE);
    const bool f8 = sk && m->fp8_decode;
    for (int l = 0; l < d.layers; ++l) {
        LlamaLayer& L = m->ll[l];
        LayerW lw = {};
        if (!small4) B2_TRY(layer_weights(m, l, &lw, st));
        if (small4) {
            B2_TRY(gemv4(m->x.p, h, L.q_qkv, L.a_qkv, L.ln1.p, d.rms_eps, nullptr, 0, m->qkv.p, 3 * h, B, 3 * h, h, ACT_NONE, st));
        } else if (f8) {
            B2_TRY(rmsnorm_quant_e4m3(m->x.p, h, L.ln1.p, m->xq8.p, h, m->xscale.as<float>(), B, h, d.rms_eps, st));
            B2_TRY(skinny8(m, kv, L.wqkv8.p, L.s_qkv.as<float>(), nullptr, 0, m->qkv.p, 3 * h, 0, B, 3 * h, h, ACT_NONE, st));
        } else if (small) {
            B2_TRY(gemv(m->x.p, h, L.wqkv.p, h, L.ln1.p, d.rms_eps, nullptr, 0, m->qkv.p, 3 * h, 0, B, 3 * h, h,
                        ACT_NONE, st));
        } else if (sk) {
            B2_TRY(rmsnorm_bf16(m->x.p, h, L.ln1.p, m->xn.p, B, h, d.rms_eps, st));
            B2_TRY(skinny(kv, m->xn.p, h, lw.wqkv, h, nullptr, 0, m->qkv.p, 3 * h, 0, B, 3 * h, h, ACT_NONE, st));
        } else {
            B2_TRY(rmsnorm_bf16(m->x.p, h, L.ln1.p, m->xn.p, B, h, d.rms_eps, st));
            B2_TRY(gemm(m->xn.p, h, lw.wqkv, h, nullptr, nullptr, 0, m->qkv.p, 3 * h, 0, B, 3 * h, h, ACT_NONE, st));
        }
        DecodeAttnArgs da;
        da.qkv = m->qkv.p;
        da.kcache = kv->k_layer(l);
        da.vcache = kv->v_layer(l);
        da.cur_len = kv->len_dev.as<int32_t>();
        da.out = m->attn.p;
        da.partial = kv->attn_partial.as<float>();
        da.counters = kv->attn_counters.as<int32_t>();
        da.B = B; da.H = H; da.D = m->hd; da.Smax = kv->pitch; da.nsplit = nsplit;
        da.theta = d.rope_theta;
        da.scale = 1.0f / sqrtf((float)m->hd);
        if (kv->e4m3()) {
            da.kscale = kv->kscale.as<float>() + (size_t)l * kv->layer_rows();
            da.vscale = kv->vscale.as<float>() + (size_t)l * kv->layer_rows();
            B2_TRY(decode_attn_e4m3(da, st));
        } else {
            B2_TRY(decode_attn_bf16(da, st));
        }
        if (small4) {
            B2_TRY(gemv4(m->attn.p, h, L.q_o, L.a_o, nullptr, 0.f, m->x.p, h, m->x.p, h, B, h, h, ACT_NONE, st));
            B2_TRY(gemv4(m->x.p, h, L.q_gu, L.a_gu, L.ln2.p, d.rms_eps, nullptr, 0, m->act.p, I, B, 2 * I, h, ACT_SWIGLU, st));
            B2_TRY(gemv4(m->act.p, I, L.q_d, L.a_d, nullptr, 0.f, m->x.p, h, m->x.p, h, B, h, I, ACT_NONE, st));
        } else if (f8) {
            B2_TRY(quantize_rows_e4m3(m->attn.p, h, B, h, m->xq8.p, h, m->xscale.as<float>(), st));
            B2_TRY(skinny8(m, kv, L.wo8.p, L.s_o.as<float>(), m->x.p, h, m->x.p, h, 0, B, h, h, ACT_NONE, st));
            B2_TRY(rmsnorm_quant_e4m3(m->x.p, h, L.ln2.p, m->xq8.p, h, m->xscale.as<float>(), B, h, d.rms_eps, st));
            B2_TRY(skinny8(m, kv, L.wgu8.p, L.s_gu.as<float>(), nullptr, 0, m->act.p, I, 0, B, 2 * I, h, ACT_SWIGLU, st));
            B2_TRY(quantize_rows_e4m3(m->act.p, I, B, I, m->xq8.p, I, m->xscale.as<float>(), st));
            B2_TRY(skinny8(m, kv, L.wd8.p, L.s_d.as<float>(), m->x.p, h, m->x.p, h, 0, B, h, I, ACT_NONE, st));
        } else if (small) {
            B2_TRY(gemv(m->attn.p, h, L.wo.p, h, nullptr, 0.f, m->x.p, h, m->x.p, h, 0, B, h, h, ACT_NONE, st));
            B2_TRY(gemv(m->x.p, h, L.wgu.p, h, L.ln2.p, d.rms_eps, nullptr, 0, m->act.p, I, 0, B, 2 * I, h,
                        ACT_SWIGLU, st));
            B2_TRY(gemv(m->act.p, I, L.wd.p, I, nullptr, 0.f, m->x.p, h, m->x.p, h, 0, B, h, I, ACT_NONE, st));
        } else if (sk) {
            B2_TRY(skinny(kv, m->attn.p, h, lw.wo, h, m->x.p, h, m->x.p, h, 0, B, h, h, ACT_NONE, st));
            B2_TRY(rmsnorm_bf16(m->x.p, h, L.ln2.p, m->xn.p, B, h, d.rms_eps, st));
            B2_TRY(skinny(kv, m->xn.p, h, lw.wgu, h, nullptr, 0, m->act.p, I, 0, B, 2 * I, h, ACT_SWIGLU, st));
            B2_TRY(skinny(kv, m->act.p, I, lw.wd, I, m->x.p, h, m->x.p, h, 0, B, h, I, ACT_NONE, st));
        } else {
            B2_TRY(gemm(m->attn.p, h, lw.wo, h, nullptr, m->x.p, h, m->x.p, h, 0, B, h, h, ACT_NONE, st));
            B2_TRY(rmsnorm_bf16(m->x.p, h, L.ln2.p, m->xn.p, B, h, d.rms_eps, st));
            B2_TRY(gemm(m->xn.p, h, lw.wgu, h, nullptr, nullptr, 0, m->act.p, I, 0, B, 2 * I, h, ACT_SWIGLU, st));
            B2_TRY(gemm(m->act.p, I, lw.wd, I, nullptr, m->x.p, h, m->x.p, h, 0, B, h, I, ACT_NONE, st));
        }
    }
    if (f8) {
        B2_TRY(rmsnorm_quant_e4m3(m->x.p, h, m->final_norm.p, m->xq8.p, h, m->xscale.as<float>(), B, h, d.rms_eps, st));
        B2_TRY(skinny8(m, kv, m->lm_head8.p, m->s_head.as<float>(), nullptr, 0, m->logits.p, V, 1, B, V, h, ACT_NONE, st));
    } else if (small || (small4 && gemv_fits(B, V, h, ACT_NONE))) {
        B2_TRY(gemv(m->x.p, h, m->lm_head.p, h, m->final_norm.p, d.rms_eps, nullptr, 0, m->logits.p, V, 1, B, V, h,
                    ACT_NONE, st));
    } else if (sk) {
        B2_TRY(rmsnorm_bf16(m->x.p, h, m->final_norm.p, m->xn.p, B, h, d.rms_eps, st));
        B2_TRY(skinny(kv, m->xn.p, h, m->lm_head.p, h, nullptr, 0, m->logits.p, V, 1, B, V, h, ACT_NONE, st));
    } else {
        B2_TRY(rmsnorm_bf16(m->x.p, h, m->final_norm.p, m->xn.p, B, h, d.rms_eps, st));
        B2_TRY(gemm(m->xn.p, h, m->lm_head.p, h, nullptr, nullptr, 0, m->logits.p, V, 1, B, V, h, ACT_NONE, st));
    }
    {
        const char* e = getenv("B2_SAMPLE_LEGACY");
        if (e != nullptr && e[0] == '1' && kv->samp_host.do_sample == 0 && kv->samp_host.tag == 0 && kv->samp_host.per_row == 0) {
            B2_TRY(argmax_f32(m->logits.as<float>(), B, V, kv->tok.as<int32_t>(), st));
            B2_TRY(store_token(kv->tok.as<int32_t>(), kv->out_tokens.as<int32_t>(), kv->step_counter.as<int32_t>(), B, st));
            B2_TRY(add_i32(kv->step_counter.as<int32_t>(), 1, 1, st));
            B2_TRY(add_i32(kv->len_dev.as<int32_t>(), B, 1, st));
            return 0;
        }
    }
    B2_TRY(sample_publish(m->logits.as<float>(), V, B, kv->sstate.as<SampleState>(), kv->rows_dev.as<RowState>(), kv->tok.as<int32_t>(),
                          kv->out_tokens.as<int32_t>(), kv->step_counter.as<int32_t>(), kv->len_dev.as<int32_t>(),
                          kv->ring_dev, kv->ring_cap, SP_SELECT | SP_WRITE_OUT | SP_BUMP, 0, st));
    return 0;
}

int fork_stream(b2_kv* kv, cudaStream_t st, cudaStream_t* run) {
    if (st != nullptr && st != cudaStreamLegacy) { *run = st; return 0; }
    if (kv->own_stream == nullptr) {
        B2_CUDA_CHECK(cudaStreamCreateWithFlags(&kv->own_stream, cudaStreamNonBlocking));
        B2_CUDA_CHECK(cudaEventCreateWithFlags(&kv->ev_fork, cudaEventDisableTiming));
        B2_CUDA_CHECK(cudaEventCreateWithFlags(&kv->ev_join, cudaEventDisableTiming));
    }
    B2_CUDA_CHECK(cudaEventRecord(kv->ev_fork, st));
    B2_CUDA_CHECK(cudaStreamWaitEvent(kv->own_stream, kv->ev_fork, 0));
    *run = kv->own_stream;
    return 0;
}
int join_stream(b2_kv* kv, cudaStream_t st, cudaStream_t run) {
    if (run == st) return 0;
    B2_CUDA_CHECK(cudaEventRecord(kv->ev_join, run));
    B2_CUDA_CHECK(cudaStreamWaitEvent(st, kv->ev_join, 0));
    return 0;
}

bool use_mega(const b2_model* m, const b2_kv* kv, int B) {
    if (kv->e4m3()) return false;
    if (m->nf4) return false;
    if (!decode_mega_fits(B, m->d.hidden, m->d.inter) || m->d.layers > 48) return false;
    static int flag = -1;
    if (flag < 0) {
        const char* e = getenv("B2_DECODE_MEGA");
        flag = (e != nullptr && e[0] == '0') ? 0 : 1;
    }
    return flag == 1;
}

constexpr int kMegaL2AheadDefault = 0;
constexpr int kMegaFastPrologueDefault = 0;

int decode_step_mega(b2_model* m, b2_kv* kv, int B, cudaStream_t st) {
    const b2_model_desc& d = m->d;
    MegaParams p;
    p.layers = kv->mega_layers.as<MegaLayer>();
    p.L = d.layers; p.h = d.hidden; p.I = d.inter; p.H = d.heads; p.V = d.vocab; p.B = B; p.Smax = kv->pitch;
    int ns = (num_sms() * 16) / (B * d.heads);
    p.nsplit = ns < 1 ? 1 : (ns > 64 ? 64 : ns);
    p.embed = m->embed.as<bf16>(); p.final_norm = m->final_norm.as<bf16>(); p.lm_head = m->lm_head.as<bf16>();
    p.tok = kv->tok.as<int32_t>(); p.cur_len = kv->len_dev.as<int32_t>();
    p.out_tokens = kv->out_tokens.as<int32_t>(); p.step_counter = kv->step_counter.as<int32_t>();
    p.x = m->x.as<bf16>(); p.qkv = m->qkv.as<bf16>(); p.attn = m->attn.as<bf16>(); p.act = m->act.as<bf16>();
    p.logits = m->logits.as<float>();
    p.attn_partial = kv->attn_partial.as<float>(); p.attn_counters = kv->attn_counters.as<int32_t>();
    unsigned int* sync = kv->mega_sync.as<unsigned int>();
    p.bar_count = sync; p.done_count = sync + 2;
    p.bar_base = kv->mega_bar_base;
    kv->mega_bar_base += (unsigned int)(5 * d.layers + 2) * (unsigned int)num_sms();
    p.eps = d.rms_eps; p.theta = d.rope_theta;
    p.scale_log2 = (1.0f / sqrtf((float)m->hd)) * 1.4426950408889634f;
    const bool sampling = kv->samp_host.do_sample != 0 || kv->samp_host.per_row != 0;
    if (!sampling && kv->samp_host.tag != 0) { p.sstate = kv->sstate.as<SampleState>(); p.ring = kv->ring_dev; p.ring_cap = kv->ring_cap; }
    if (kv->samp_host.per_row) p.rows = kv->rows_dev.as<RowState>();
    {
        const char* e = getenv("B2_MEGA_L2_AHEAD");
        int ahead = e ? atoi(e) : kMegaL2AheadDefault;
        p.l2_ahead = ahead < 0 ? 0 : (ahead > 64 ? 64 : ahead) / 4 * 4;
        e = getenv("B2_MEGA_L2_MODE");
        p.l2_mode = (e && e[0] == '2') ? 2 : 1;
        e = getenv("B2_MEGA_FAST_PROLOGUE");
        p.fast_prologue = e ? (e[0] != '0') : kMegaFastPrologueDefault;
        e = getenv("B2_MEGA_GAMMA_SMEM");
        p.gamma_smem = e ? (e[0] != '0') : 1;
    }
    static int trace_mode = -1;
    if (trace_mode < 0) { const char* e = getenv("B2_MEGA_TRACE"); trace_mode = (e && e[0] != 0) ? 1 : 0; }
    if (trace_mode == 1) {
        static int steps_seen = 0;
        if (++steps_seen == 40) {
            const int n = (5 * d.layers + 2) * 4;
            DevBuf tb;
            B2_TRY(tb.alloc((size_t)n * 8));
            cudaMemset(tb.p, 0, (size_t)n * 8);
            p.trace = tb.as<long long>();
            int r = decode_mega(p, st);
            cudaStreamSynchronize(st);
            std::vector<long long> host(n);
            cudaMemcpy(host.data(), tb.p, (size_t)n * 8, cudaMemcpyDeviceToHost);
            FILE* f = fopen(getenv("B2_MEGA_TRACE"), "w");
            if (f) {
                for (int ph = 0; ph <= 5 * d.layers; ++ph)
                    fprintf(f, "%d %lld %lld %lld %lld %lld\n", ph, host[ph * 4], host[ph * 4 + 1], host[ph * 4 + 2],
                            host[ph * 4 + 3], host[(ph + 1) * 4]);
                fclose(f);
            }
            tb.free();
            return r;
        }
    }
    B2_TRY(decode_mega(p, st));
    if (sampling)
        B2_TRY(sample_publish(m->logits.as<float>(), d.vocab, B, kv->sstate.as<SampleState>(), kv->rows_dev.as<RowState>(), kv->tok.as<int32_t>(),
                              kv->out_tokens.as<int32_t>(), kv->step_counter.as<int32_t>(), kv->len_dev.as<int32_t>(),
                              kv->ring_dev, kv->ring_cap, SP_SELECT | SP_WRITE_OUT, -1, st));
    return 0;
}

int decode_step_run(b2_model* m, b2_kv* kv, int B, cudaStream_t st) {
    if (use_mega(m, kv, B)) return decode_step_mega(m, kv, B, st);
    if (kv->warm_B != B) {
        if (kv->graph) { cudaGraphExecDestroy(kv->graph); kv->graph = nullptr; kv->graph_B = 0; }
        B2_TRY(decode_step_launch(m, kv, B, st));
        kv->warm_B = B;
        return 0;
    }
    if (kv->graph == nullptr || kv->graph_B != B) {
        if (kv->graph) { cudaGraphExecDestroy(kv->graph); kv->graph = nullptr; }
        cudaGraph_t graph = nullptr;
        B2_CUDA_CHECK(cudaStreamBeginCapture(st, cudaStreamCaptureModeThreadLocal));
        const unsigned long long launches_before = g_launch_count;
        int r = decode_step_launch(m, kv, B, st);
        g_launch_count = launches_before;
        cudaError_t e = cudaStreamEndCapture(st, &graph);
        if (r != 0) { if (graph) cudaGraphDestroy(graph); return r; }
        B2_CUDA_CHECK(e);
        e = cudaGraphInstantiate(&kv->graph, graph, 0);
        cudaGraphDestroy(graph);
        B2_CUDA_CHECK(e);
        kv->graph_B = B;
    }
    B2_CUDA_CHECK(cudaGraphLaunch(kv->graph, st));
    if (m->nf4) {
        const bool small4 = use_gemv_nf4(m, B);
        const bool head_gemv = small4 && gemv_fits(B, m->d.vocab, m->d.hidden, ACT_NONE);
        g_launch_count += 1 + (unsigned long long)m->d.layers * (small4 ? 5 : 8) + (head_gemv ? 1 : 2) + 1;
        return 0;
    }
    const bool small = !use_skinny(kv, B) && B <= 8 && gemv_fits(B, m->d.hidden, m->d.inter, ACT_NONE) &&
                       gemv_fits(B, m->d.vocab, m->d.hidden, ACT_NONE);
    const int per_layer = small ? 5 : ((m->fp8_decode && use_skinny(kv, B)) ? 9 : 7);
    g_launch_count += 1 + (unsigned long long)m->d.layers * per_layer + (small ? 1 : 2) + 1;
    return 0;
}

struct DeviceGuard {
    int prev = -1;
    explicit DeviceGuard(int dev) {
        if (cudaGetDevice(&prev) != cudaSuccess) prev = -1;
        if (prev != dev) cudaSetDevice(dev); else prev = -1;
    }
    ~DeviceGuard() { if (prev >= 0) cudaSetDevice(prev); }
    DeviceGuard(const DeviceGuard&) = delete;
    DeviceGuard& operator=(const DeviceGuard&) = delete;
};

int ws_enter(b2_model* m, cudaStream_t st) {
    if (m->ws_valid && m->ws_stream != st) B2_CUDA_CHECK(cudaStreamWaitEvent(st, m->ws_event, 0));
    return 0;
}
int ws_leave(b2_model* m, cudaStream_t st) {
    B2_CUDA_CHECK(cudaEventRecord(m->ws_event, st));
    m->ws_stream = st;
    m->ws_valid = true;
    return 0;
}

}

extern "C" {

int b2_init(int device) {
    B2_CUDA_CHECK(cudaSetDevice(device));
    cudaDeviceProp prop;
    B2_CUDA_CHECK(cudaGetDeviceProperties(&prop, device));
    if (prop.major != 9) {
        set_error("b2_init: device %d is sm_%d%d; this library only contains sm_90a code (no fallback path)", device,
                  prop.major, prop.minor);
        return -3;
    }
    return 0;
}

const char* b2_last_error(void) { return g_err; }
int b2_version(void) { return 5; }
unsigned long long b2_launch_count(void) { return g_launch_count; }

int b2_model_create(const b2_model_desc* desc, b2_model** out) {
    B2_CHECK_ARG(desc != nullptr && out != nullptr, "b2_model_create: null argument");
    const b2_model_desc& d = *desc;
    B2_CHECK_ARG(d.vit_hidden > 0 && d.vit_heads > 0 && d.vit_hidden / d.vit_heads == 64 &&
                     d.vit_hidden % 256 == 0 && d.vit_hidden <= 2048,
                 "b2_model_create: vision head_dim must be 64 and hidden a multiple of 256 (hidden=%d heads=%d)",
                 d.vit_hidden, d.vit_heads);
    B2_CHECK_ARG(d.hidden > 0 && d.heads > 0 && d.hidden / d.heads == 128 && d.hidden % 256 == 0,
                 "b2_model_create: decoder head_dim must be 128 and hidden a multiple of 256 (hidden=%d heads=%d)",
                 d.hidden, d.heads);
    B2_CHECK_ARG(d.inter % 256 == 0 && d.vit_inter % 8 == 0 && d.vocab % 8 == 0,
                 "b2_model_create: inter %% 256, vit_inter %% 8, vocab %% 8 must be 0");
    B2_CHECK_ARG(d.image_size % d.patch_size == 0, "b2_model_create: image_size not a multiple of patch_size");
    B2_CHECK_ARG(d.max_batch >= 1 && d.max_seq >= 1 && d.max_images >= 1, "b2_model_create: bad workspace sizing");
    const int live = d.vit_select_layer < 0 ? d.vit_layers + 1 + d.vit_select_layer : d.vit_select_layer;
    B2_CHECK_ARG(live >= 0 && live <= d.vit_layers, "b2_model_create: vit_select_layer %d out of range",
                 d.vit_select_layer);
    b2_model* m = new b2_model();
    m->d = d;
    cudaGetDevice(&m->device);
    const int g = d.image_size / d.patch_size;
    m->P = g * g;
    m->T = m->P + 1;
    const int kk = 3 * d.patch_size * d.patch_size;
    m->kpad = (kk + 7) / 8 * 8;
    m->vit_live = live;
    m->vit.resize(live);
    m->ll.resize(d.layers);
    *out = m;
    return 0;
}

int b2_model_set_weight(b2_model* m, const char* hf_key, const void* ptr, const int64_t* shape, int ndim, int dtype) {
    B2_CHECK_ARG(m && hf_key && ptr && shape, "b2_model_set_weight: null argument");
    B2_CHECK_ARG(dtype == DT_BF16 || dtype == DT_F16 || dtype == DT_F32, "b2_model_set_weight: bad dtype %d", dtype);
    std::lock_guard<std::mutex> lk(m->mu);
    DeviceGuard dg(m->device);
    std::string k(hf_key);
    const int h = m->d.hidden, V = m->d.vocab, D = m->d.vit_hidden;
    int r = -1;
    size_t pos;
    if ((pos = k.find("vision_model.")) != std::string::npos) {
        r = set_vision_weight(m, k.substr(pos + strlen("vision_model.")), ptr, shape, ndim, dtype);
    } else if (k == "model.embed_tokens.weight") {
        B2_TRY(expect_shape(hf_key, shape, ndim, V, h));
        r = put(m->embed, (size_t)V * h, 0, ptr, dtype, (int64_t)V * h);
    } else if (k == "model.norm.weight") {
        B2_TRY(expect_shape(hf_key, shape, ndim, h));
        r = put(m->final_norm, h, 0, ptr, dtype, h);
    } else if (k == "lm_head.weight") {
        B2_TRY(expect_shape(hf_key, shape, ndim, V, h));
        r = put(m->lm_head, (size_t)V * h, 0, ptr, dtype, (int64_t)V * h);
    } else if (m->nf4 && (k == "model.mm_projector.0.weight" || k == "model.mm_projector.2.weight")) {
        set_error("set_weight(%s): the projector of this model holds its NF4 w_hat (b2_model_enable_nf4); it cannot be reloaded", hf_key);
        return -1;
    } else if (k == "model.mm_projector.0.weight") {
        B2_TRY(expect_shape(hf_key, shape, ndim, h, D));
        r = put(m->p0_w, (size_t)h * D, 0, ptr, dtype, (int64_t)h * D);
    } else if (k == "model.mm_projector.0.bias") {
        B2_TRY(expect_shape(hf_key, shape, ndim, h));
        r = put(m->p0_b, h, 0, ptr, dtype, h);
    } else if (k == "model.mm_projector.2.weight") {
        B2_TRY(expect_shape(hf_key, shape, ndim, h, h));
        r = put(m->p2_w, (size_t)h * h, 0, ptr, dtype, (int64_t)h * h);
    } else if (k == "model.mm_projector.2.bias") {
        B2_TRY(expect_shape(hf_key, shape, ndim, h));
        r = put(m->p2_b, h, 0, ptr, dtype, h);
    } else if (starts_with(k, "model.layers.")) {
        int li = -1, consumed = 0;
        if (sscanf(hf_key, "model.layers.%d.%n", &li, &consumed) != 1 || li < 0 || li >= m->d.layers) {
            set_error("set_weight: bad decoder layer index in '%s'", hf_key);
            return -1;
        }
        r = set_llama_layer_weight(m, li, k.substr(consumed), hf_key, ptr, shape, ndim, dtype);
    } else {
        set_error("set_weight: unknown key '%s'", hf_key);
        return -1;
    }
    return r;
}

int b2_model_finalize(b2_model* m) {
    B2_CHECK_ARG(m != nullptr, "b2_model_finalize: null model");
    std::lock_guard<std::mutex> lk(m->mu);
    DeviceGuard dg(m->device);
    const b2_model_desc& d = m->d;
    std::string missing;
    auto need = [&](const DevBuf& b, const char* name) {
        if (b.p == nullptr) { if (missing.size() < 600) { missing += name; missing += ' '; } }
    };
    need(m->patch_w, "patch_embedding"); need(m->cls, "class_embedding"); need(m->pos, "position_embedding");
    need(m->pre_g, "pre_layrnorm.weight"); need(m->pre_b, "pre_layrnorm.bias");
    for (size_t i = 0; i < m->vit.size(); ++i) {
        VitLayer& L = m->vit[i];
        const DevBuf* bs[12] = {&L.ln1_g, &L.ln1_b, &L.wqkv, &L.bqkv, &L.wo, &L.bo, &L.ln2_g, &L.ln2_b, &L.w1, &L.b1, &L.w2, &L.b2};
        for (int j = 0; j < 12; ++j)
            if (bs[j]->p == nullptr) { char t[64]; snprintf(t, sizeof t, "vision.layer%zu.#%d", i, j); need(*bs[j], t); }
    }
    need(m->p0_w, "mm_projector.0.weight"); need(m->p0_b, "mm_projector.0.bias");
    need(m->p2_w, "mm_projector.2.weight"); need(m->p2_b, "mm_projector.2.bias");
    need(m->embed, "embed_tokens"); need(m->final_norm, "model.norm"); need(m->lm_head, "lm_head");
    for (size_t i = 0; i < m->ll.size(); ++i) {
        LlamaLayer& L = m->ll[i];
        const DevBuf* bs[6] = {&L.ln1, &L.wqkv, &L.wo, &L.ln2, &L.wgu, &L.wd};
        for (int j = 0; j < 6; ++j)
            if (bs[j]->p == nullptr) { char t[64]; snprintf(t, sizeof t, "layers.%zu.#%d", i, j); need(*bs[j], t); }
    }
    if (!missing.empty()) {
        set_error("b2_model_finalize: missing weights: %s", missing.c_str());
        return -3;
    }
    for (size_t i = 0; i < m->vit.size(); ++i)
        if (m->vit[i].qkv_w != 7u || m->vit[i].qkv_b != 7u) {
            set_error("b2_model_finalize: vision layer %zu is missing q/k/v parts (weights mask %u, bias mask %u of 7)", i,
                      m->vit[i].qkv_w, m->vit[i].qkv_b);
            return -3;
        }
    for (size_t i = 0; i < m->ll.size(); ++i)
        if (m->ll[i].qkv_parts != 7u) {
            set_error("b2_model_finalize: decoder layer %zu is missing q/k/v projections (mask %u of 7)", i, m->ll[i].qkv_parts);
            return -3;
        }
    if (m->err_host == nullptr) {
        B2_CUDA_CHECK(cudaHostAlloc(reinterpret_cast<void**>(&m->err_host), 8 * sizeof(int), cudaHostAllocMapped));
        memset(m->err_host, 0, 8 * sizeof(int));
        B2_CUDA_CHECK(cudaHostGetDevicePointer(reinterpret_cast<void**>(&m->err_dev), m->err_host, 0));
        B2_CUDA_CHECK(cudaEventCreateWithFlags(&m->ws_event, cudaEventDisableTiming));
    }
    const int D = d.vit_hidden, I = d.vit_inter, h = d.hidden;
    const size_t vrows = (size_t)d.max_images * m->T, prow = (size_t)d.max_images * m->P;
    B2_TRY(m->v_col.alloc(prow * m->kpad * 2));
    B2_TRY(m->v_patch.alloc(prow * D * 2));
    B2_TRY(m->v_hidden.alloc(vrows * D * 2));
    B2_TRY(m->v_xn.alloc(vrows * D * 2));
    B2_TRY(m->v_qkv.alloc(vrows * 3 * D * 2));
    B2_TRY(m->v_attn.alloc(vrows * D * 2));
    B2_TRY(m->v_mlp.alloc(vrows * I * 2));
    B2_TRY(m->v_feats.alloc(prow * D * 2));
    B2_TRY(m->p_mid.alloc(prow * h * 2));
    B2_TRY(m->p_done.alloc(((prow + 127) / 128 + 1) * sizeof(int)));
    B2_TRY(m->enc_pixels.alloc((size_t)d.max_images * 3 * d.image_size * d.image_size * 2));
    B2_TRY(m->enc_out.alloc(prow * h * 2));
    m->enc_graph.assign(d.max_images + 1, nullptr);
    m->enc_warm.assign(d.max_images + 1, 0);
    const size_t rows = (size_t)d.max_batch * d.max_seq;
    B2_TRY(m->x.alloc(rows * h * 2));
    B2_TRY(m->xn.alloc(rows * h * 2));
    B2_TRY(m->qkv.alloc(rows * 3 * h * 2));
    B2_TRY(m->attn.alloc(rows * h * 2));
    B2_TRY(m->act.alloc(rows * d.inter * 2));
    B2_TRY(m->last_idx.alloc((size_t)d.max_batch * 4));
    B2_TRY(m->chunk_pos.alloc((size_t)d.max_batch * 2 * 4));
    B2_TRY(m->splice_idx.alloc(rows * 4));
    B2_TRY(m->xlast.alloc((size_t)d.max_batch * h * 2));
    B2_TRY(m->logits.alloc((size_t)d.max_batch * d.vocab * 4));
    m->finalized = true;
    return 0;
}

int b2_model_destroy(b2_model* m) {
    if (m == nullptr) return 0;
    DeviceGuard dg(m->device);
    cudaDeviceSynchronize();
    if (m->err_host) cudaFreeHost(m->err_host);
    if (m->ws_event) cudaEventDestroy(m->ws_event);
    for (cudaGraphExec_t g : m->enc_graph) if (g) cudaGraphExecDestroy(g);
    if (m->enc_stream) cudaStreamDestroy(m->enc_stream);
    if (m->enc_fork) cudaEventDestroy(m->enc_fork);
    if (m->enc_join) cudaEventDestroy(m->enc_join);
    DevBuf* top[] = {&m->patch_w, &m->cls, &m->pos, &m->pre_g, &m->pre_b, &m->p0_w, &m->p0_b, &m->p2_w, &m->p2_b,
                     &m->embed, &m->final_norm, &m->lm_head, &m->v_col, &m->v_patch, &m->v_hidden, &m->v_xn,
                     &m->v_qkv, &m->v_attn, &m->v_mlp, &m->v_feats, &m->p_mid, &m->p_done, &m->enc_pixels, &m->enc_out, &m->x, &m->xn, &m->qkv, &m->attn,
                     &m->act, &m->last_idx, &m->chunk_pos, &m->xlast, &m->logits, &m->splice_idx, &m->lm_head8, &m->s_head, &m->xq8, &m->xscale,
                     &m->kstage, &m->vstage, &m->nf4_scratch};
    for (DevBuf* b : top) b->free();
    for (VitLayer& L : m->vit) {
        DevBuf* bs[12] = {&L.ln1_g, &L.ln1_b, &L.wqkv, &L.bqkv, &L.wo, &L.bo, &L.ln2_g, &L.ln2_b, &L.w1, &L.b1, &L.w2, &L.b2};
        for (DevBuf* b : bs) b->free();
    }
    for (LlamaLayer& L : m->ll) {
        DevBuf* bs[24] = {&L.ln1, &L.wqkv, &L.wo, &L.ln2, &L.wgu, &L.wd, &L.tmp_gate, &L.tmp_up,
                          &L.wqkv8, &L.wo8, &L.wgu8, &L.wd8, &L.s_qkv, &L.s_o, &L.s_gu, &L.s_d,
                          &L.q_qkv, &L.a_qkv, &L.q_o, &L.a_o, &L.q_gu, &L.a_gu, &L.q_d, &L.a_d};
        for (DevBuf* b : bs) b->free();
    }
    delete m;
    return 0;
}

int b2_model_enable_fp8_decode(b2_model* m) {
    B2_CHECK_ARG(m != nullptr, "b2_model_enable_fp8_decode: null model");
    B2_CHECK_ARG(m->finalized, "b2_model_enable_fp8_decode: model not finalized");
    std::lock_guard<std::mutex> lk(m->mu);
    DeviceGuard dg(m->device);
    if (m->fp8_decode) return 0;
    B2_CHECK_ARG(!m->nf4, "b2_model_enable_fp8_decode: the decoder Linears are NF4 (b2_model_enable_nf4); the two formats do not combine");
    const b2_model_desc& d = m->d;
    const int h = d.hidden, I = d.inter, V = d.vocab;
    B2_CHECK_ARG(h % 16 == 0 && I % 16 == 0, "b2_model_enable_fp8_decode: hidden/inter must be multiples of 16");
    auto quant = [&](DevBuf& w, int N, int K, DevBuf& w8, DevBuf& sc) -> int {
        B2_TRY(w8.alloc((size_t)N * K));
        B2_TRY(sc.alloc((size_t)N * sizeof(float)));
        return quantize_rows_e4m3(w.p, K, N, K, w8.p, K, sc.as<float>(), nullptr);
    };
    for (LlamaLayer& L : m->ll) {
        B2_TRY(quant(L.wqkv, 3 * h, h, L.wqkv8, L.s_qkv));
        B2_TRY(quant(L.wo, h, h, L.wo8, L.s_o));
        B2_TRY(quant(L.wgu, 2 * I, h, L.wgu8, L.s_gu));
        B2_TRY(quant(L.wd, h, I, L.wd8, L.s_d));
    }
    B2_TRY(quant(m->lm_head, V, h, m->lm_head8, m->s_head));
    const int mb = d.max_batch > 128 ? 128 : d.max_batch;
    B2_TRY(m->xq8.alloc((size_t)mb * (h > I ? h : I)));
    B2_TRY(m->xscale.alloc((size_t)mb * sizeof(float)));
    B2_CUDA_CHECK(cudaDeviceSynchronize());
    m->fp8_decode = true;
    return 0;
}

int b2_model_enable_nf4(b2_model* m) {
    B2_CHECK_ARG(m != nullptr, "b2_model_enable_nf4: null model");
    std::lock_guard<std::mutex> lk(m->mu);
    DeviceGuard dg(m->device);
    B2_CHECK_ARG(m->finalized, "b2_model_enable_nf4: model not finalized");
    if (m->nf4) return 0;
    B2_CHECK_ARG(!m->fp8_decode, "b2_model_enable_nf4: e4m3 decode weights are enabled (b2_model_enable_fp8_decode); the two formats do not combine");
    B2_CHECK_ARG(m->kv_live.load() == 0, "b2_model_enable_nf4: %d KV cache(s) exist; enable NF4 before creating any (the megakernel "
                 "tables of existing caches point at the bf16 weights)", m->kv_live.load());
    const b2_model_desc& d = m->d;
    const int h = d.hidden, I = d.inter, D = d.vit_hidden;
    auto quant = [&](const DevBuf& w, int N, int K, DevBuf& q, DevBuf& a) -> int {
        B2_TRY(q.alloc((size_t)N * K / 2));
        B2_TRY(a.alloc((size_t)N * (K / 64) * sizeof(float)));
        return quantize_nf4(w.p, K, N, K, q.p, a.as<float>(), 1, nullptr);
    };
    int r = 0;
    for (LlamaLayer& L : m->ll) {
        if ((r = quant(L.wqkv, 3 * h, h, L.q_qkv, L.a_qkv)) != 0 || (r = quant(L.wo, h, h, L.q_o, L.a_o)) != 0 ||
            (r = quant(L.wgu, 2 * I, h, L.q_gu, L.a_gu)) != 0 || (r = quant(L.wd, h, I, L.q_d, L.a_d)) != 0)
            break;
    }
    DevBuf pq, pa;
    auto roundtrip = [&](const DevBuf& w, int N, int K, DevBuf& out) -> int {
        B2_TRY(pq.alloc((size_t)N * K / 2));
        B2_TRY(pa.alloc((size_t)N * (K / 64) * sizeof(float)));
        B2_TRY(out.alloc((size_t)N * K * 2));
        B2_TRY(quantize_nf4(w.p, K, N, K, pq.p, pa.as<float>(), 0, nullptr));
        Nf4Matrix mt;
        mt.q = pq.p; mt.absmax = pa.as<float>(); mt.out = out.p; mt.N = N; mt.K = K;
        B2_TRY(dequantize_nf4(&mt, 1, 0, nullptr));
        B2_CUDA_CHECK(cudaStreamSynchronize(nullptr));
        return 0;
    };
    DevBuf p0_hat, p2_hat;
    if (r == 0) r = m->nf4_scratch.alloc(((size_t)4 * h * h + (size_t)3 * I * h) * 2);
    if (r == 0 && cudaDeviceSynchronize() != cudaSuccess) { set_error("b2_model_enable_nf4: quantisation failed: %s", cudaGetErrorString(cudaGetLastError())); r = -2; }
    if (r == 0) r = roundtrip(m->p0_w, h, D, p0_hat);
    if (r == 0) r = roundtrip(m->p2_w, h, h, p2_hat);
    pq.free();
    pa.free();
    if (r != 0) {
        for (LlamaLayer& L : m->ll)
            for (DevBuf* b : {&L.q_qkv, &L.a_qkv, &L.q_o, &L.a_o, &L.q_gu, &L.a_gu, &L.q_d, &L.a_d}) b->free();
        m->nf4_scratch.free();
        p0_hat.free();
        p2_hat.free();
        return r;
    }
    std::swap(m->p0_w, p0_hat);
    std::swap(m->p2_w, p2_hat);
    p0_hat.free();
    p2_hat.free();
    for (LlamaLayer& L : m->ll)
        for (DevBuf* b : {&L.wqkv, &L.wo, &L.wgu, &L.wd}) b->free();
    m->nf4 = true;
    return 0;
}

int64_t b2_model_weight_bytes(b2_model* m) {
    B2_CHECK_ARG(m != nullptr, "b2_model_weight_bytes: null model");
    std::lock_guard<std::mutex> lk(m->mu);
    size_t n = 0;
    for (const DevBuf* b : {&m->patch_w, &m->cls, &m->pos, &m->pre_g, &m->pre_b, &m->p0_w, &m->p0_b, &m->p2_w, &m->p2_b, &m->embed,
                            &m->final_norm, &m->lm_head, &m->lm_head8, &m->s_head})
        n += b->bytes;
    for (const VitLayer& L : m->vit)
        for (const DevBuf* b : {&L.ln1_g, &L.ln1_b, &L.wqkv, &L.bqkv, &L.wo, &L.bo, &L.ln2_g, &L.ln2_b, &L.w1, &L.b1, &L.w2, &L.b2})
            n += b->bytes;
    for (const LlamaLayer& L : m->ll)
        for (const DevBuf* b : {&L.ln1, &L.wqkv, &L.wo, &L.ln2, &L.wgu, &L.wd, &L.wqkv8, &L.wo8, &L.wgu8, &L.wd8, &L.s_qkv, &L.s_o,
                                &L.s_gu, &L.s_d, &L.q_qkv, &L.a_qkv, &L.q_o, &L.a_o, &L.q_gu, &L.a_gu, &L.q_d, &L.a_d})
            n += b->bytes;
    return (int64_t)n;
}

int b2_kv_create(b2_model* m, int max_batch, int max_seq, b2_kv** out) {
    return b2_kv_create_ex(m, max_batch, max_seq, B2_KV_BF16, out);
}

int b2_kv_create_ex(b2_model* m, int max_batch, int max_seq, int kv_dtype, b2_kv** out) {
    B2_CHECK_ARG(m && out, "b2_kv_create: null argument");
    B2_CHECK_ARG(kv_dtype == B2_KV_BF16 || kv_dtype == B2_KV_E4M3, "b2_kv_create: unknown kv_dtype %d (B2_KV_BF16 = 0, B2_KV_E4M3 = 1)",
                 kv_dtype);
    B2_CHECK_ARG(max_batch >= 1 && max_batch <= m->d.max_batch, "b2_kv_create: max_batch %d exceeds model max_batch %d",
                 max_batch, m->d.max_batch);
    B2_CHECK_ARG(max_seq >= 1, "b2_kv_create: max_seq must be positive");
    std::lock_guard<std::mutex> lk(m->mu);
    DeviceGuard dg(m->device);
    b2_kv* kv = new b2_kv();
    kv->m = m;
    kv->max_batch = max_batch;
    kv->max_seq = max_seq;
    kv->dtype = kv_dtype;
    kv->pitch = kv->e4m3() ? (max_seq + 3) / 4 * 4 : max_seq;
    const size_t per = (size_t)m->d.layers * kv->layer_stride() * kv->elem_bytes();
    const size_t per_scale = kv->e4m3() ? (size_t)m->d.layers * kv->layer_rows() * sizeof(float) : 0;
    int r = 0;
    if (kv->e4m3() && m->kstage.p == nullptr) {
        const size_t stage = (size_t)m->d.max_batch * m->d.max_seq * m->d.hidden * 2;
        if ((r = m->kstage.alloc(stage)) != 0 || (r = m->vstage.alloc(stage)) != 0) {
            m->kstage.free();
            delete kv;
            return r;
        }
    }
    if ((r = kv->k.alloc(per)) != 0 || (r = kv->v.alloc(per)) != 0 ||
        (r = kv->kscale.alloc(per_scale)) != 0 || (r = kv->vscale.alloc(per_scale)) != 0 ||
        (r = kv->len_dev.alloc((size_t)max_batch * 4)) != 0 || (r = kv->tok.alloc((size_t)max_batch * 4)) != 0 ||
        (r = kv->step_counter.alloc(4)) != 0) {
        b2_kv_destroy(kv);
        return r;
    }
    kv->out_capacity = max_seq;
    const int max_split = 64;
    if (!m->nf4) {
        std::vector<MegaLayer> tbl(m->d.layers);
        for (int l = 0; l < m->d.layers; ++l) {
            LlamaLayer& L = m->ll[l];
            tbl[l].ln1 = L.ln1.as<bf16>(); tbl[l].wqkv = L.wqkv.as<bf16>(); tbl[l].wo = L.wo.as<bf16>();
            tbl[l].ln2 = L.ln2.as<bf16>(); tbl[l].wgu = L.wgu.as<bf16>(); tbl[l].wd = L.wd.as<bf16>();
            tbl[l].kcache = reinterpret_cast<bf16*>(kv->k_layer(l));
            tbl[l].vcache = reinterpret_cast<bf16*>(kv->v_layer(l));
        }
        if ((r = kv->mega_layers.alloc(tbl.size() * sizeof(MegaLayer))) != 0 || (r = kv->mega_sync.alloc(64)) != 0) {
            b2_kv_destroy(kv);
            return r;
        }
        cudaMemcpy(kv->mega_layers.p, tbl.data(), tbl.size() * sizeof(MegaLayer), cudaMemcpyHostToDevice);
        cudaMemset(kv->mega_sync.p, 0, 64);
    }
    if ((r = kv->out_tokens.alloc((size_t)kv->out_capacity * max_batch * 4)) != 0 ||
        (r = kv->attn_partial.alloc(((size_t)max_batch * m->d.heads * max_split + 1024) * (128 + 2) * 4)) != 0 ||
        (r = kv->attn_counters.alloc((size_t)max_batch * m->d.heads * 4)) != 0) {
        b2_kv_destroy(kv);
        return r;
    }
    if (max_batch >= 3 && max_batch <= 128) {
        const int h = m->d.hidden, I = m->d.inter, V = m->d.vocab;
        size_t ws = 0;
        const int shapes[5][2] = {{3 * h, h}, {h, h}, {2 * I, h}, {h, I}, {V, h}};
        int nmax = 0;
        for (auto& sh : shapes) {
            const size_t b = gemm_skinny_workspace_bytes(max_batch, sh[0], sh[1]);
            ws = b > ws ? b : ws;
            nmax = sh[0] > nmax ? sh[0] : nmax;
        }
        if ((r = kv->sk_partial.alloc(ws)) != 0 || (r = kv->sk_counters.alloc(gemm_skinny_counter_bytes(nmax))) != 0) {
            b2_kv_destroy(kv);
            return r;
        }
        cudaMemset(kv->sk_counters.p, 0, gemm_skinny_counter_bytes(nmax));
    }
    kv->ring_cap = max_seq;
    if ((r = kv->sstate.alloc(sizeof(SampleState))) != 0 || (r = kv->rows_dev.alloc((size_t)max_batch * sizeof(RowState))) != 0) {
        b2_kv_destroy(kv);
        return r;
    }
    cudaMemset(kv->sstate.p, 0, sizeof(SampleState));
    cudaMemset(kv->rows_dev.p, 0, (size_t)max_batch * sizeof(RowState));
    kv->rows_host.assign(max_batch, RowState{});
    if (cudaHostAlloc(reinterpret_cast<void**>(&kv->ring_host), (size_t)kv->ring_cap * max_batch * 4, cudaHostAllocMapped) != cudaSuccess ||
        cudaHostGetDevicePointer(reinterpret_cast<void**>(&kv->ring_dev), kv->ring_host, 0) != cudaSuccess) {
        set_error("b2_kv_create: cannot allocate the pinned token ring (%d x %d)", kv->ring_cap, max_batch);
        cudaGetLastError();
        b2_kv_destroy(kv);
        return -2;
    }
    memset(kv->ring_host, 0, (size_t)kv->ring_cap * max_batch * 4);
    cudaMemset(kv->k.p, 0, per);
    cudaMemset(kv->v.p, 0, per);
    if (per_scale) { cudaMemset(kv->kscale.p, 0, per_scale); cudaMemset(kv->vscale.p, 0, per_scale); }
    cudaMemset(kv->len_dev.p, 0, (size_t)max_batch * 4);
    cudaMemset(kv->tok.p, 0, (size_t)max_batch * 4);
    cudaMemset(kv->step_counter.p, 0, 4);
    cudaMemset(kv->attn_counters.p, 0, (size_t)max_batch * m->d.heads * 4);
    if ((r = kv->rope_tab.alloc((size_t)max_seq * (m->hd / 2) * sizeof(uint32_t))) != 0 ||
        (r = rope_table_build(kv->rope_tab.p, max_seq, m->hd, m->d.rope_theta, nullptr)) != 0) {
        b2_kv_destroy(kv);
        return r;
    }
    B2_CUDA_CHECK(cudaDeviceSynchronize());
    kv->len_host.assign(max_batch, 0);
    kv->counted = true;
    m->kv_live++;
    *out = kv;
    return 0;
}

int b2_kv_reset(b2_kv* kv) {
    B2_CHECK_ARG(kv != nullptr, "b2_kv_reset: null");
    std::lock_guard<std::mutex> lk(kv->m->mu);
    DeviceGuard dg(kv->m->device);
    kv->len_host.assign(kv->max_batch, 0);
    {
        const char* e = getenv("B2_KV_RESET_GRAPH");
        if (e != nullptr && e[0] == '1') {
            if (kv->graph) { cudaGraphExecDestroy(kv->graph); kv->graph = nullptr; kv->graph_B = 0; }
            kv->warm_B = 0;
        }
    }
    return 0;
}

int b2_kv_destroy(b2_kv* kv) {
    if (kv == nullptr) return 0;
    DeviceGuard dg(kv->m->device);
    cudaDeviceSynchronize();
    if (kv->counted) kv->m->kv_live--;
    if (kv->ring_host) cudaFreeHost(kv->ring_host);
    if (kv->graph) cudaGraphExecDestroy(kv->graph);
    if (kv->own_stream) cudaStreamDestroy(kv->own_stream);
    if (kv->ev_fork) cudaEventDestroy(kv->ev_fork);
    if (kv->ev_join) cudaEventDestroy(kv->ev_join);
    DevBuf* bs[] = {&kv->k, &kv->v, &kv->kscale, &kv->vscale, &kv->len_dev, &kv->tok, &kv->step_counter, &kv->out_tokens, &kv->attn_partial,
                    &kv->attn_counters, &kv->mega_layers, &kv->mega_sync, &kv->sk_partial, &kv->sk_counters, &kv->sstate, &kv->rows_dev, &kv->rope_tab,
                    &kv->beam_in, &kv->beam_ws, &kv->beam_out};
    for (DevBuf* b : bs) b->free();
    delete kv;
    return 0;
}

int b2_kv_dtype(b2_kv* kv) {
    B2_CHECK_ARG(kv != nullptr, "b2_kv_dtype: null");
    return kv->dtype;
}

int64_t b2_kv_bytes(b2_kv* kv) {
    B2_CHECK_ARG(kv != nullptr, "b2_kv_bytes: null");
    return (int64_t)(kv->k.bytes + kv->v.bytes + kv->kscale.bytes + kv->vscale.bytes);
}

int b2_kv_lengths(b2_kv* kv, int32_t* lens_host, int n) {
    B2_CHECK_ARG(kv && lens_host && n >= 0 && n <= kv->max_batch, "b2_kv_lengths: bad argument");
    for (int i = 0; i < n; ++i) lens_host[i] = kv->len_host[i];
    return 0;
}

int b2_vit_encode(b2_model* m, const void* pixels, int B, void* out_feats, void* stream) {
    B2_CHECK_ARG(m && pixels && out_feats && B >= 1, "b2_vit_encode: bad argument");
    B2_CHECK_ARG(m->finalized, "b2_vit_encode: model not finalized");
    std::lock_guard<std::mutex> lk(m->mu);
    DeviceGuard dg(m->device);
    cudaStream_t st = reinterpret_cast<cudaStream_t>(stream);
    B2_TRY(ws_enter(m, st));
    const size_t img_elems = (size_t)3 * m->d.image_size * m->d.image_size;
    for (int b0 = 0; b0 < B; b0 += m->d.max_images) {
        const int n = B - b0 < m->d.max_images ? B - b0 : m->d.max_images;
        B2_TRY(vit_forward_chunk(m, reinterpret_cast<const bf16*>(pixels) + b0 * img_elems, n,
                                 reinterpret_cast<bf16*>(out_feats) + (size_t)b0 * m->P * m->d.vit_hidden, st));
    }
    return ws_leave(m, st);
}

int b2_project(b2_model* m, const void* feats, int rows, void* out, void* stream) {
    B2_CHECK_ARG(m && feats && out && rows >= 1, "b2_project: bad argument");
    B2_CHECK_ARG(m->finalized, "b2_project: model not finalized");
    std::lock_guard<std::mutex> lk(m->mu);
    DeviceGuard dg(m->device);
    cudaStream_t st = reinterpret_cast<cudaStream_t>(stream);
    B2_TRY(ws_enter(m, st));
    B2_TRY(project_rows(m, feats, rows, out, st));
    return ws_leave(m, st);
}

int b2_encode_images(b2_model* m, const void* pixels, int B, void* out, void* stream) {
    B2_CHECK_ARG(m && pixels && out && B >= 1, "b2_encode_images: bad argument");
    B2_CHECK_ARG(m->finalized, "b2_encode_images: model not finalized");
    std::lock_guard<std::mutex> lk(m->mu);
    DeviceGuard dg(m->device);
    cudaStream_t st = reinterpret_cast<cudaStream_t>(stream);
    B2_TRY(ws_enter(m, st));
    const size_t img_elems = (size_t)3 * m->d.image_size * m->d.image_size;
    for (int b0 = 0; b0 < B; b0 += m->d.max_images) {
        const int n = B - b0 < m->d.max_images ? B - b0 : m->d.max_images;
        B2_TRY(encode_chunk(m, reinterpret_cast<const bf16*>(pixels) + b0 * img_elems, n,
                            reinterpret_cast<bf16*>(out) + (size_t)b0 * m->P * m->d.hidden, st));
    }
    return ws_leave(m, st);
}

int b2_splice(b2_model* m, const int32_t* src_index, const void* image_feats, int n_feat_rows, int rows, void* embeds_out,
              void* stream) {
    B2_CHECK_ARG(m && src_index && embeds_out && rows >= 1 && n_feat_rows >= 0, "b2_splice: bad argument");
    B2_CHECK_ARG(image_feats != nullptr || n_feat_rows == 0, "b2_splice: n_feat_rows=%d without image_feats", n_feat_rows);
    B2_CHECK_ARG(m->finalized, "b2_splice: model not finalized");
    std::lock_guard<std::mutex> lk(m->mu);
    DeviceGuard dg(m->device);
    return splice_embed(src_index, m->embed.p, image_feats, embeds_out, rows, m->d.hidden, m->d.vocab, n_feat_rows,
                        m->err_dev, reinterpret_cast<cudaStream_t>(stream));
}

int b2_splice_ids(b2_model* m, const int64_t* input_ids, int B, int Lt, int k_per_row, const int32_t* feat_offsets_host, int n_img,
                  const void* image_feats, int S, void* embeds_out, void* stream) {
    B2_CHECK_ARG(m && input_ids && feat_offsets_host && embeds_out, "b2_splice_ids: null argument");
    B2_CHECK_ARG(m->finalized, "b2_splice_ids: model not finalized");
    B2_CHECK_ARG(B >= 1 && S >= 1 && (size_t)B * S <= (size_t)m->d.max_batch * m->d.max_seq,
                 "b2_splice_ids: B*S=%d exceeds the workspace (%d rows)", B * S, m->d.max_batch * m->d.max_seq);
    B2_CHECK_ARG(image_feats != nullptr || n_img == 0, "b2_splice_ids: image slots without image_feats");
    std::lock_guard<std::mutex> lk(m->mu);
    DeviceGuard dg(m->device);
    cudaStream_t st = reinterpret_cast<cudaStream_t>(stream);
    B2_TRY(ws_enter(m, st));
    B2_TRY(splice_index(reinterpret_cast<const long long*>(input_ids), B, Lt, k_per_row, feat_offsets_host, n_img, -200, S,
                        m->splice_idx.as<int32_t>(), m->err_dev, st));
    B2_TRY(splice_embed(m->splice_idx.as<int32_t>(), m->embed.p, image_feats, embeds_out, B * S, m->d.hidden, m->d.vocab,
                        n_img > 0 ? feat_offsets_host[n_img] : 0, m->err_dev, st));
    return ws_leave(m, st);
}

int b2_async_error(b2_model* m, int* code_out) {
    B2_CHECK_ARG(m && code_out, "b2_async_error: null argument");
    int code = 0;
    if (m->err_host != nullptr)
        for (int i = 0; i < 8; ++i)
            if (reinterpret_cast<volatile int*>(m->err_host)[i] != 0) {
                code |= 1 << i;
                reinterpret_cast<volatile int*>(m->err_host)[i] = 0;
            }
    *code_out = code;
    if (code != 0)
        set_error("device-side input check failed:%s%s%s", (code & B2_ERR_TOKEN_RANGE) ? " token id outside [0, vocab) (or an image placeholder without image features)" : "",
                  (code & B2_ERR_IMAGE_ROW_RANGE) ? " image-feature row outside the encoded images" : "",
                  (code & B2_ERR_SPLICE_SLOTS) ? " more image placeholders than images" : "");
    return 0;
}

int b2_prefill(b2_model* m, b2_kv* kv, const void* embeds, const int32_t* seq_lens_host, int B, int S,
               void* logits_out, int logits_mode, void* stream) {
    return b2_prefill_at(m, kv, embeds, nullptr, seq_lens_host, B, S, 0, logits_out, logits_mode, stream);
}

int b2_prefill_slots(b2_model* m, b2_kv* kv, const void* embeds, const int32_t* seq_lens_host, int B, int S, int slot0,
                     void* logits_out, int logits_mode, void* stream) {
    return b2_prefill_at(m, kv, embeds, nullptr, seq_lens_host, B, S, slot0, logits_out, logits_mode, stream);
}

int b2_prefill_at(b2_model* m, b2_kv* kv, const void* embeds, const int32_t* start_host, const int32_t* seq_lens_host, int B,
                  int S, int slot0, void* logits_out, int logits_mode, void* stream) {
    B2_CHECK_ARG(m && kv && embeds && kv->m == m, "b2_prefill: bad handle");
    B2_CHECK_ARG(m->finalized, "b2_prefill: model not finalized");
    B2_CHECK_ARG(B >= 1 && slot0 >= 0 && slot0 + B <= kv->max_batch && S >= 1 && S <= kv->max_seq,
                 "b2_prefill: B=%d S=%d slot0=%d exceed the KV cache (max_batch=%d max_seq=%d)", B, S, slot0, kv->max_batch, kv->max_seq);
    B2_CHECK_ARG((size_t)B * S <= (size_t)m->d.max_batch * m->d.max_seq,
                 "b2_prefill: B*S=%d exceeds the workspace (%d rows)", B * S, m->d.max_batch * m->d.max_seq);
    B2_CHECK_ARG(logits_mode == B2_LOGITS_NONE || logits_out != nullptr, "b2_prefill: logits_out is null");
    std::lock_guard<std::mutex> lk(m->mu);
    DeviceGuard dg(m->device);
    cudaStream_t st = reinterpret_cast<cudaStream_t>(stream);
    const b2_model_desc& d = m->d;
    const int h = d.hidden, I = d.inter, H = d.heads, V = d.vocab, T = B * S;

    std::vector<int32_t> lens(B), last(B), start(B, 0), total(B);
    int max_start = 0;
    for (int b = 0; b < B; ++b) {
        lens[b] = seq_lens_host ? seq_lens_host[b] : S;
        B2_CHECK_ARG(lens[b] >= 1 && lens[b] <= S, "b2_prefill: seq_lens[%d]=%d out of range (S=%d)", b, lens[b], S);
        if (start_host != nullptr) {
            start[b] = start_host[b];
            B2_CHECK_ARG(start[b] >= 0 && start[b] <= kv->len_host[slot0 + b],
                         "b2_prefill_at: start[%d]=%d outside [0, current length %d]", b, start[b], kv->len_host[slot0 + b]);
            B2_CHECK_ARG(start[b] + lens[b] <= kv->max_seq, "b2_prefill_at: start[%d]=%d + %d tokens exceed the cache (max_seq=%d)",
                         b, start[b], lens[b], kv->max_seq);
        }
        max_start = start[b] > max_start ? start[b] : max_start;
        total[b] = start[b] + lens[b];
        last[b] = b * S + lens[b] - 1;
    }
    const bool offset = max_start > 0;
    const bool q8 = kv->e4m3();
    const int kv_pitch = !q8 ? kv->pitch : (offset ? (max_start + S < kv->max_seq ? max_start + S : kv->max_seq) : S);
    B2_CHECK_ARG(!q8 || (size_t)B * kv_pitch <= (size_t)d.max_batch * d.max_seq,
                 "b2_prefill_at: %d samples x %d rows exceed the staging slab (%d rows)", B, kv_pitch, d.max_batch * d.max_seq);
    B2_TRY(ws_enter(m, st));
    B2_TRY(set_i32_pairs(kv->len_dev.as<int32_t>() + slot0, total.data(), m->last_idx.as<int32_t>(), last.data(), B, st));
    int32_t* pos_dev = m->chunk_pos.as<int32_t>();
    int32_t* clen_dev = pos_dev + d.max_batch;
    if (offset) B2_TRY(set_i32_pairs(pos_dev, start.data(), clen_dev, lens.data(), B, st));
    for (int b = 0; b < B; ++b) kv->len_host[slot0 + b] = total[b];
    const size_t slot_rows = (size_t)slot0 * H * kv->pitch;

    B2_CUDA_CHECK(cudaMemcpyAsync(m->x.p, embeds, (size_t)T * h * 2, cudaMemcpyDeviceToDevice, st));
    bool rope_fused = T >= 512 && m->hd == 128 && h % 256 == 0;
    { const char* e = getenv("B2_ROPE_FUSED"); if (e != nullptr && e[0] == '0') rope_fused = false; }
    for (int l = 0; l < d.layers; ++l) {
        LlamaLayer& L = m->ll[l];
        LayerW lw;
        B2_TRY(layer_weights(m, l, &lw, st));
        bf16* kc = q8 ? m->kstage.as<bf16>() : reinterpret_cast<bf16*>(kv->k_layer(l)) + slot_rows * m->hd;
        bf16* vc = q8 ? m->vstage.as<bf16>() : reinterpret_cast<bf16*>(kv->v_layer(l)) + slot_rows * m->hd;
        const size_t row0 = (size_t)l * kv->layer_rows() + slot_rows;
        if (q8 && offset)
            B2_TRY(kv_dequantize_e4m3(kv->k.as<uint8_t>() + row0 * m->hd, kv->v.as<uint8_t>() + row0 * m->hd,
                                      kv->kscale.as<float>() + row0, kv->vscale.as<float>() + row0, pos_dev, kc, vc, B, H,
                                      kv->pitch, kv_pitch, st));
        B2_TRY(rmsnorm_bf16(m->x.p, h, L.ln1.p, m->xn.p, T, h, d.rms_eps, st));
        if (rope_fused) {
            GemmArgs g;
            g.A = m->xn.p; g.lda = h; g.W = lw.wqkv; g.ldw = h; g.out = m->qkv.p; g.ld_out = 3 * h;
            g.M = T; g.N = 3 * h; g.K = h; g.act = ACT_ROPE_QKV;
            g.rope.table = kv->rope_tab.p; g.rope.kcache = kc; g.rope.vcache = vc; g.rope.S = S; g.rope.H = H; g.rope.Smax = kv_pitch;
            g.rope.pos0 = offset ? pos_dev : nullptr;
            B2_TRY(gemm_bf16_2cta(g, st));
        } else {
            B2_TRY(gemm(m->xn.p, h, lw.wqkv, h, nullptr, nullptr, 0, m->qkv.p, 3 * h, 0, T, 3 * h, h, ACT_NONE, st));
            B2_TRY(rope_kv_write(m->qkv.p, kc, vc, B, S, H, m->hd, kv_pitch, d.rope_theta, st, offset ? pos_dev : nullptr));
        }
        FlashArgs fa;
        fa.q = m->qkv.p; fa.q_bs = (int64_t)S * 3 * h; fa.q_ts = 3 * h; fa.q_hs = m->hd;
        fa.k = kc; fa.k_bs = (int64_t)H * kv_pitch * m->hd; fa.k_ts = m->hd; fa.k_hs = (int64_t)kv_pitch * m->hd;
        fa.v = vc; fa.v_bs = fa.k_bs; fa.v_ts = m->hd; fa.v_hs = fa.k_hs;
        fa.o = m->attn.p; fa.o_bs = (int64_t)S * h; fa.o_ts = h; fa.o_hs = m->hd;
        fa.seq_lens = offset ? clen_dev : kv->len_dev.as<int32_t>() + slot0;
        if (offset) { fa.pos0 = pos_dev; fa.Skv = kv_pitch; }
        fa.B = B; fa.H = H; fa.S = S; fa.D = m->hd; fa.causal = 1;
        fa.scale = 1.0f / sqrtf((float)m->hd);
        B2_TRY(flash_attn_bf16(fa, st));
        if (q8) {
            B2_TRY(kv_quantize_e4m3(kc, vc, kv->k.as<uint8_t>() + row0 * m->hd, kv->v.as<uint8_t>() + row0 * m->hd,
                                    kv->kscale.as<float>() + row0, kv->vscale.as<float>() + row0,
                                    offset ? clen_dev : kv->len_dev.as<int32_t>() + slot0, B, S, H, m->hd, kv->pitch, st,
                                    offset ? pos_dev : nullptr, kv_pitch));
        }
        B2_TRY(gemm(m->attn.p, h, lw.wo, h, nullptr, m->x.p, h, m->x.p, h, 0, T, h, h, ACT_NONE, st));
        B2_TRY(rmsnorm_bf16(m->x.p, h, L.ln2.p, m->xn.p, T, h, d.rms_eps, st));
        B2_TRY(gemm(m->xn.p, h, lw.wgu, h, nullptr, nullptr, 0, m->act.p, I, 0, T, 2 * I, h, ACT_SWIGLU, st));
        B2_TRY(gemm(m->act.p, I, lw.wd, I, nullptr, m->x.p, h, m->x.p, h, 0, T, h, I, ACT_NONE, st));
    }
    if (logits_mode == B2_LOGITS_LAST) {
        B2_TRY(rmsnorm_gather_bf16(m->x.p, m->last_idx.as<int32_t>(), m->final_norm.p, m->xlast.p, B, h, d.rms_eps, st));
        if (B <= 8 && gemv_fits(B, V, h, ACT_NONE))
            B2_TRY(gemv(m->xlast.p, h, m->lm_head.p, h, nullptr, 0.f, nullptr, 0, logits_out, V, 1, B, V, h, ACT_NONE, st));
        else
            B2_TRY(gemm(m->xlast.p, h, m->lm_head.p, h, nullptr, nullptr, 0, logits_out, V, 1, B, V, h, ACT_NONE, st));
    } else if (logits_mode == B2_LOGITS_ALL) {
        B2_TRY(rmsnorm_bf16(m->x.p, h, m->final_norm.p, m->xn.p, T, h, d.rms_eps, st));
        B2_TRY(gemm(m->xn.p, h, m->lm_head.p, h, nullptr, nullptr, 0, logits_out, V, 1, T, V, h, ACT_NONE, st));
    }
    return ws_leave(m, st);
}

static int copy_tokens_in(b2_kv* kv, const int32_t* tokens, int B, cudaStream_t st) {
    B2_CUDA_CHECK(cudaMemcpyAsync(kv->tok.p, tokens, (size_t)B * 4, cudaMemcpyDefault, st));
    return 0;
}

static int set_sampling(b2_kv* kv, const SampleState& v, bool force, cudaStream_t st) {
    const SampleState& c = kv->samp_host;
    if (!force && kv->samp_valid && c.do_sample == v.do_sample && c.temperature == v.temperature && c.top_p == v.top_p &&
        c.top_k == v.top_k && c.seed == v.seed && c.tag == v.tag && c.per_row == v.per_row)
        return 0;
    B2_TRY(sample_state_set(kv->sstate.as<SampleState>(), v, st));
    kv->samp_host = v;
    kv->samp_valid = true;
    return 0;
}
static int set_greedy_unpublished(b2_kv* kv, cudaStream_t st) {
    SampleState v = {};
    v.temperature = 1.f; v.top_p = 1.f;
    kv->stream_B = 0;
    return set_sampling(kv, v, false, st);
}
static bool is_device_pointer(const void* p) {
    cudaPointerAttributes attr;
    if (cudaPointerGetAttributes(&attr, p) != cudaSuccess) { cudaGetLastError(); return false; }
    return attr.type == cudaMemoryTypeDevice || attr.type == cudaMemoryTypeManaged;
}

int b2_decode_step(b2_model* m, b2_kv* kv, const int32_t* tokens, int B, void* logits_out, int32_t* next_tokens_out,
                   void* stream) {
    B2_CHECK_ARG(m && kv && tokens && kv->m == m, "b2_decode_step: bad handle");
    B2_CHECK_ARG(m->finalized, "b2_decode_step: model not finalized");
    B2_CHECK_ARG(B >= 1 && B <= kv->max_batch, "b2_decode_step: B=%d exceeds cache batch %d", B, kv->max_batch);
    std::lock_guard<std::mutex> lk(m->mu);
    DeviceGuard dg(m->device);
    cudaStream_t st = reinterpret_cast<cudaStream_t>(stream);
    for (int b = 0; b < B; ++b)
        B2_CHECK_ARG(kv->len_host[b] >= 1 && kv->len_host[b] < kv->max_seq,
                     "b2_decode_step: sample %d has cache length %d (capacity %d; prefill first)", b, kv->len_host[b],
                     kv->max_seq);
    B2_TRY(ws_enter(m, st));
    B2_TRY(copy_tokens_in(kv, tokens, B, st));
    B2_CUDA_CHECK(cudaMemsetAsync(kv->step_counter.p, 0, 4, st));
    B2_TRY(set_greedy_unpublished(kv, st));
    cudaStream_t run = nullptr;
    B2_TRY(fork_stream(kv, st, &run));
    B2_TRY(decode_step_run(m, kv, B, run));
    B2_TRY(join_stream(kv, st, run));
    for (int b = 0; b < B; ++b) kv->len_host[b]++;
    if (logits_out)
        B2_CUDA_CHECK(cudaMemcpyAsync(logits_out, m->logits.p, (size_t)B * m->d.vocab * 4, cudaMemcpyDefault, st));
    if (next_tokens_out)
        B2_CUDA_CHECK(cudaMemcpyAsync(next_tokens_out, kv->tok.p, (size_t)B * 4, cudaMemcpyDefault, st));
    B2_TRY(ws_leave(m, st));
    if (next_tokens_out && !is_device_pointer(next_tokens_out)) B2_CUDA_CHECK(cudaStreamSynchronize(st));
    return 0;
}

int b2_decode_greedy(b2_model* m, b2_kv* kv, const int32_t* first_tokens, int B, int n_steps, int32_t* out_tokens,
                     void* stream) {
    B2_CHECK_ARG(m && kv && first_tokens && out_tokens && kv->m == m, "b2_decode_greedy: bad handle");
    B2_CHECK_ARG(m->finalized, "b2_decode_greedy: model not finalized");
    B2_CHECK_ARG(B >= 1 && B <= kv->max_batch && n_steps >= 1, "b2_decode_greedy: bad B=%d n_steps=%d", B, n_steps);
    B2_CHECK_ARG(n_steps <= kv->out_capacity, "b2_decode_greedy: n_steps=%d exceeds capacity %d", n_steps,
                 kv->out_capacity);
    std::lock_guard<std::mutex> lk(m->mu);
    DeviceGuard dg(m->device);
    cudaStream_t st = reinterpret_cast<cudaStream_t>(stream);
    for (int b = 0; b < B; ++b)
        B2_CHECK_ARG(kv->len_host[b] >= 1 && kv->len_host[b] + n_steps <= kv->max_seq,
                     "b2_decode_greedy: sample %d cache length %d + %d steps exceeds capacity %d", b, kv->len_host[b],
                     n_steps, kv->max_seq);
    B2_TRY(ws_enter(m, st));
    B2_TRY(copy_tokens_in(kv, first_tokens, B, st));
    B2_CUDA_CHECK(cudaMemsetAsync(kv->step_counter.p, 0, 4, st));
    B2_TRY(set_greedy_unpublished(kv, st));
    cudaStream_t run = nullptr;
    B2_TRY(fork_stream(kv, st, &run));
    for (int s = 0; s < n_steps; ++s) B2_TRY(decode_step_run(m, kv, B, run));
    B2_TRY(join_stream(kv, st, run));
    for (int b = 0; b < B; ++b) kv->len_host[b] += n_steps;
    B2_CUDA_CHECK(cudaMemcpyAsync(out_tokens, kv->out_tokens.p, (size_t)n_steps * B * 4, cudaMemcpyDefault, st));
    B2_TRY(ws_leave(m, st));
    if (!is_device_pointer(out_tokens)) B2_CUDA_CHECK(cudaStreamSynchronize(st));
    return 0;
}

static int check_copies(b2_kv* kv, const int32_t* src, const int32_t* dst, int n, int row_begin, std::vector<int32_t>& end) {
    B2_CHECK_ARG(n >= 0 && n <= kv->max_batch && (n == 0 || (src != nullptr && dst != nullptr)) && row_begin >= 0,
                 "b2_kv_copy_slots: bad argument (n=%d row_begin=%d)", n, row_begin);
    std::vector<char> is_src(kv->max_batch, 0), is_dst(kv->max_batch, 0);
    end.assign(n, 0);
    for (int i = 0; i < n; ++i) {
        B2_CHECK_ARG(src[i] >= 0 && src[i] < kv->max_batch && dst[i] >= 0 && dst[i] < kv->max_batch,
                     "b2_kv_copy_slots: pair %d (%d -> %d) outside the cache's %d slots", i, src[i], dst[i], kv->max_batch);
        B2_CHECK_ARG(row_begin <= kv->len_host[src[i]], "b2_kv_copy_slots: row_begin %d beyond the length %d of slot %d", row_begin,
                     kv->len_host[src[i]], src[i]);
        is_src[src[i]] = 1;
        end[i] = kv->len_host[src[i]];
    }
    for (int i = 0; i < n; ++i) {
        B2_CHECK_ARG(!is_dst[dst[i]], "b2_kv_copy_slots: slot %d is the destination of two copies", dst[i]);
        B2_CHECK_ARG(!is_src[dst[i]], "b2_kv_copy_slots: slot %d is both a source and a destination", dst[i]);
        is_dst[dst[i]] = 1;
    }
    return 0;
}

static int launch_copies(b2_model* m, b2_kv* kv, const int32_t* src, const int32_t* dst, const std::vector<int32_t>& end, int n,
                         int row_begin, cudaStream_t st) {
    if (n == 0) return 0;
    B2_TRY(kv_copy_slots(kv->k.p, kv->v.p, kv->e4m3() ? kv->kscale.as<float>() : nullptr, kv->e4m3() ? kv->vscale.as<float>() : nullptr,
                         src, dst, end.data(), n, row_begin, m->d.layers, m->d.heads, kv->max_batch, kv->pitch,
                         (int)(m->hd * kv->elem_bytes()), kv->len_dev.as<int32_t>(), st));
    for (int i = 0; i < n; ++i) kv->len_host[dst[i]] = end[i];
    return 0;
}

int b2_kv_copy_slots(b2_model* m, b2_kv* kv, const int32_t* src_host, const int32_t* dst_host, int n, int row_begin, void* stream) {
    B2_CHECK_ARG(m && kv && kv->m == m, "b2_kv_copy_slots: bad handle");
    std::lock_guard<std::mutex> lk(m->mu);
    DeviceGuard dg(m->device);
    std::vector<int32_t> end;
    B2_TRY(check_copies(kv, src_host, dst_host, n, row_begin, end));
    return launch_copies(m, kv, src_host, dst_host, end, n, row_begin, reinterpret_cast<cudaStream_t>(stream));
}

int b2_op_beam_topk(const float* logits, const int32_t* row_of_beam, const float* beam_scores, int B, int nb, int V, int K,
                    float* out_scores, int32_t* out_tokens, int32_t* out_beams, void* stream) {
    B2_CHECK_ARG(B >= 1 && nb >= 1 && nb <= 32 && K >= 1 && K <= 128, "b2_op_beam_topk: B=%d nb=%d K=%d", B, nb, K);
    cudaStream_t st = reinterpret_cast<cudaStream_t>(stream);
    void* ws = nullptr;
    B2_CUDA_CHECK(cudaMallocAsync(&ws, beam_topk_workspace_bytes(B, nb, K), st));
    const int r = beam_topk(logits, row_of_beam, beam_scores, B, nb, V, K, ws, out_scores, out_tokens, out_beams, st);
    B2_CUDA_CHECK(cudaFreeAsync(ws, st));
    return r;
}

int b2_beam_step(b2_model* m, b2_kv* kv, const b2_beam_step_args* a, void* stream) {
    B2_CHECK_ARG(m && kv && a && kv->m == m, "b2_beam_step: bad handle");
    B2_CHECK_ARG(m->finalized, "b2_beam_step: model not finalized");
    const int B = a->B, nb = a->nb, K = a->K, n = a->B * a->nb;
    B2_CHECK_ARG(B >= 1 && nb >= 1 && nb <= 32 && n <= kv->max_batch, "b2_beam_step: B=%d x nb=%d beams exceed the cache's %d slots",
                 B, nb, kv->max_batch);
    B2_CHECK_ARG(K >= 1 && K <= 128 && (long long)K <= (long long)nb * m->d.vocab, "b2_beam_step: K=%d outside [1, min(128, nb*V)]", K);
    B2_CHECK_ARG(a->tokens_host && a->slot_of_beam_host && a->beam_scores_host && a->out_scores_host && a->out_tokens_host &&
                 a->out_beams_host, "b2_beam_step: null array");
    std::lock_guard<std::mutex> lk(m->mu);
    DeviceGuard dg(m->device);
    cudaStream_t st = reinterpret_cast<cudaStream_t>(stream);
    std::vector<int32_t> end;
    B2_TRY(check_copies(kv, a->copy_src_host, a->copy_dst_host, a->n_copies, a->row_begin, end));
    std::vector<int32_t> len(kv->len_host.begin(), kv->len_host.begin() + n), tok(n, -1);
    for (int i = 0; i < a->n_copies; ++i)
        if (a->copy_dst_host[i] < n) len[a->copy_dst_host[i]] = end[i];
    for (int i = 0; i < n; ++i) {
        const int s = a->slot_of_beam_host[i];
        B2_CHECK_ARG(s >= 0 && s < n && tok[s] < 0, "b2_beam_step: slot_of_beam is not a permutation of [0, %d)", n);
        B2_CHECK_ARG(a->tokens_host[i] >= 0, "b2_beam_step: negative token %d for beam %d", a->tokens_host[i], i);
        tok[s] = a->tokens_host[i];
    }
    for (int s = 0; s < n; ++s)
        B2_CHECK_ARG(len[s] >= 1 && len[s] < kv->max_seq, "b2_beam_step: slot %d has cache length %d (capacity %d)", s, len[s],
                     kv->max_seq);
    if (kv->beam_in.p == nullptr) {
        B2_TRY(kv->beam_in.alloc((size_t)2 * kv->max_batch * 4));
        B2_TRY(kv->beam_ws.alloc(beam_topk_workspace_bytes(kv->max_batch, 1, 128)));
        B2_TRY(kv->beam_out.alloc((size_t)kv->max_batch * 128 * 12));
    }
    B2_TRY(ws_enter(m, st));
    B2_TRY(launch_copies(m, kv, a->copy_src_host, a->copy_dst_host, end, a->n_copies, a->row_begin, st));
    B2_TRY(copy_tokens_in(kv, tok.data(), n, st));
    B2_CUDA_CHECK(cudaMemsetAsync(kv->step_counter.p, 0, 4, st));
    B2_TRY(set_greedy_unpublished(kv, st));
    cudaStream_t run = nullptr;
    B2_TRY(fork_stream(kv, st, &run));
    B2_TRY(decode_step_run(m, kv, n, run));
    B2_TRY(join_stream(kv, st, run));
    for (int s = 0; s < n; ++s) kv->len_host[s]++;
    int32_t* rows = kv->beam_in.as<int32_t>();
    B2_TRY(set_i32_pairs(rows, a->slot_of_beam_host, rows + kv->max_batch, reinterpret_cast<const int32_t*>(a->beam_scores_host), n, st));
    float* o_s = kv->beam_out.as<float>();
    int32_t* o_t = reinterpret_cast<int32_t*>(o_s + B * K);
    int32_t* o_b = o_t + B * K;
    B2_TRY(beam_topk(m->logits.as<float>(), rows, reinterpret_cast<const float*>(rows + kv->max_batch), B, nb, m->d.vocab, K, kv->beam_ws.p,
                     o_s, o_t, o_b, st));
    B2_CUDA_CHECK(cudaMemcpyAsync(a->out_scores_host, o_s, (size_t)B * K * 4, cudaMemcpyDeviceToHost, st));
    B2_CUDA_CHECK(cudaMemcpyAsync(a->out_tokens_host, o_t, (size_t)B * K * 4, cudaMemcpyDeviceToHost, st));
    B2_CUDA_CHECK(cudaMemcpyAsync(a->out_beams_host, o_b, (size_t)B * K * 4, cudaMemcpyDeviceToHost, st));
    B2_TRY(ws_leave(m, st));
    B2_CUDA_CHECK(cudaStreamSynchronize(st));
    return 0;
}

int b2_stream_begin(b2_model* m, b2_kv* kv, const float* logits, int B, const b2_sampling* sp, void* stream) {
    B2_CHECK_ARG(m && kv && logits && kv->m == m, "b2_stream_begin: bad handle");
    B2_CHECK_ARG(m->finalized, "b2_stream_begin: model not finalized");
    B2_CHECK_ARG(B >= 1 && B <= kv->max_batch, "b2_stream_begin: B=%d exceeds cache batch %d", B, kv->max_batch);
    SampleState v = {};
    v.temperature = 1.f; v.top_p = 1.f;
    if (sp != nullptr && sp->do_sample) {
        B2_CHECK_ARG(sp->temperature > 0.f, "b2_stream_begin: temperature must be positive when sampling (got %g)", (double)sp->temperature);
        B2_CHECK_ARG(sp->top_p > 0.f && sp->top_p <= 1.f, "b2_stream_begin: top_p must be in (0, 1] (got %g)", (double)sp->top_p);
        B2_CHECK_ARG(sp->top_k >= 0, "b2_stream_begin: top_k must be >= 0");
        v.do_sample = 1; v.temperature = sp->temperature; v.top_p = sp->top_p; v.top_k = sp->top_k; v.seed = sp->seed;
    }
    std::lock_guard<std::mutex> lk(m->mu);
    DeviceGuard dg(m->device);
    cudaStream_t st = reinterpret_cast<cudaStream_t>(stream);
    for (int b = 0; b < B; ++b)
        B2_CHECK_ARG(kv->len_host[b] >= 1, "b2_stream_begin: sample %d has an empty cache (prefill first)", b);
    kv->epoch += 1;
    v.tag = 1 + kv->epoch % 2047;
    B2_TRY(ws_enter(m, st));
    B2_TRY(set_sampling(kv, v, true, st));
    B2_CUDA_CHECK(cudaMemsetAsync(kv->step_counter.p, 0, 4, st));
    B2_TRY(sample_publish(logits, m->d.vocab, B, kv->sstate.as<SampleState>(), kv->rows_dev.as<RowState>(), kv->tok.as<int32_t>(), nullptr,
                          kv->step_counter.as<int32_t>(), kv->len_dev.as<int32_t>(), kv->ring_dev, kv->ring_cap, SP_SELECT, 0, st));
    kv->stream_B = B; kv->stream_tag = v.tag; kv->stream_scheduled = 1;
    return ws_leave(m, st);
}

int b2_stream_enqueue(b2_model* m, b2_kv* kv, int n_steps, void* stream) {
    B2_CHECK_ARG(m && kv && kv->m == m && n_steps >= 1, "b2_stream_enqueue: bad argument");
    std::lock_guard<std::mutex> lk(m->mu);
    DeviceGuard dg(m->device);
    B2_CHECK_ARG(kv->stream_B >= 1, "b2_stream_enqueue: no streaming generation on this cache (b2_stream_begin first)");
    const int B = kv->stream_B;
    const bool per_row = kv->samp_host.per_row != 0;
    B2_CHECK_ARG(per_row || kv->stream_scheduled + n_steps <= kv->ring_cap, "b2_stream_enqueue: %d tokens exceed the ring capacity %d",
                 kv->stream_scheduled + n_steps, kv->ring_cap);
    for (int b = 0; b < B; ++b)
        B2_CHECK_ARG((per_row && !kv->rows_host[b].active) || kv->len_host[b] + n_steps <= kv->max_seq,
                     "b2_stream_enqueue: sample %d cache length %d + %d steps exceeds capacity %d", b, kv->len_host[b], n_steps, kv->max_seq);
    cudaStream_t st = reinterpret_cast<cudaStream_t>(stream);
    B2_TRY(ws_enter(m, st));
    cudaStream_t run = nullptr;
    B2_TRY(fork_stream(kv, st, &run));
    for (int s = 0; s < n_steps; ++s) B2_TRY(decode_step_run(m, kv, B, run));
    B2_TRY(join_stream(kv, st, run));
    for (int b = 0; b < B; ++b)
        if (!per_row || kv->rows_host[b].active) kv->len_host[b] += n_steps;
    kv->stream_scheduled += n_steps;
    return ws_leave(m, st);
}

int b2_batch_begin(b2_model* m, b2_kv* kv, int B, void* stream) {
    B2_CHECK_ARG(m && kv && kv->m == m && B >= 1 && B <= kv->max_batch, "b2_batch_begin: bad argument");
    std::lock_guard<std::mutex> lk(m->mu);
    DeviceGuard dg(m->device);
    cudaStream_t st = reinterpret_cast<cudaStream_t>(stream);
    SampleState v = {};
    v.temperature = 1.f; v.top_p = 1.f; v.per_row = 1;
    kv->epoch += 1;
    v.tag = 1 + kv->epoch % 2047;
    B2_TRY(ws_enter(m, st));
    B2_TRY(set_sampling(kv, v, true, st));
    B2_CUDA_CHECK(cudaMemsetAsync(kv->step_counter.p, 0, 4, st));
    B2_CUDA_CHECK(cudaMemsetAsync(kv->rows_dev.p, 0, (size_t)kv->max_batch * sizeof(RowState), st));
    B2_CUDA_CHECK(cudaMemsetAsync(kv->len_dev.p, 0, (size_t)kv->max_batch * 4, st));
    B2_CUDA_CHECK(cudaMemsetAsync(kv->tok.p, 0, (size_t)kv->max_batch * 4, st));
    kv->rows_host.assign(kv->max_batch, RowState{});
    kv->len_host.assign(kv->max_batch, 0);
    kv->stream_B = B; kv->stream_tag = v.tag; kv->stream_scheduled = 0;
    return ws_leave(m, st);
}

int b2_batch_set_row(b2_model* m, b2_kv* kv, int slot, int active, const b2_sampling* sp, int first_token, void* stream) {
    B2_CHECK_ARG(m && kv && kv->m == m && slot >= 0 && slot < kv->stream_B, "b2_batch_set_row: bad slot %d", slot);
    B2_CHECK_ARG(kv->samp_host.per_row != 0, "b2_batch_set_row: b2_batch_begin first");
    RowState v = {};
    v.active = active ? 1 : 0; v.temperature = 1.f; v.top_p = 1.f; v.index = 1;
    if (active && sp != nullptr && sp->do_sample) {
        B2_CHECK_ARG(sp->temperature > 0.f && sp->top_p > 0.f && sp->top_p <= 1.f && sp->top_k >= 0, "b2_batch_set_row: bad sampling parameters");
        v.do_sample = 1; v.temperature = sp->temperature; v.top_p = sp->top_p; v.top_k = sp->top_k; v.seed = sp->seed;
    }
    std::lock_guard<std::mutex> lk(m->mu);
    DeviceGuard dg(m->device);
    B2_CHECK_ARG(!active || kv->len_host[slot] >= 1, "b2_batch_set_row: slot %d has an empty cache (prefill it first)", slot);
    cudaStream_t st = reinterpret_cast<cudaStream_t>(stream);
    B2_TRY(ws_enter(m, st));
    B2_TRY(row_state_set(kv->rows_dev.as<RowState>() + slot, v, active ? kv->tok.as<int32_t>() + slot : nullptr, first_token, st));
    if (!active) {
        B2_CUDA_CHECK(cudaMemsetAsync(kv->len_dev.as<int32_t>() + slot, 0, 4, st));
        kv->len_host[slot] = 0;
    }
    kv->rows_host[slot] = v;
    return ws_leave(m, st);
}

int b2_stream_wait(b2_kv* kv, int index, int32_t* tokens_host, int timeout_ms) {
    B2_CHECK_ARG(kv && tokens_host && index >= 0, "b2_stream_wait: bad argument");
    const int B = kv->stream_B;
    B2_CHECK_ARG(B >= 1, "b2_stream_wait: no streaming generation on this cache");
    B2_CHECK_ARG(index < kv->stream_scheduled, "b2_stream_wait: token %d has not been scheduled (%d scheduled)", index,
                 kv->stream_scheduled);
    volatile int32_t* slot = kv->ring_host + (size_t)(index % kv->ring_cap) * B;
    const int tag = 1 + (kv->stream_tag - 1 + index / kv->ring_cap) % 2047;
    struct timespec t0, t1;
    clock_gettime(CLOCK_MONOTONIC, &t0);
    for (unsigned long long spins = 0;; ++spins) {
        bool ready = true;
        for (int b = 0; b < B; ++b)
            if ((slot[b] >> 20) != tag) { ready = false; break; }
        if (ready) {
            for (int b = 0; b < B; ++b) tokens_host[b] = slot[b] & 0xFFFFF;
            return 0;
        }
        if (spins < 4096) continue;
        struct timespec nap = {0, 20000};
        nanosleep(&nap, nullptr);
        if ((spins & 255) == 0) {
            clock_gettime(CLOCK_MONOTONIC, &t1);
            const double ms = (t1.tv_sec - t0.tv_sec) * 1e3 + (t1.tv_nsec - t0.tv_nsec) * 1e-6;
            cudaError_t e = cudaPeekAtLastError();
            if (e != cudaSuccess) { set_error("b2_stream_wait: CUDA error while waiting for token %d: %s", index, cudaGetErrorString(e)); return -2; }
            if (timeout_ms > 0 && ms > timeout_ms) { set_error("b2_stream_wait: token %d not published after %d ms", index, timeout_ms); return -3; }
        }
    }
}

int b2_op_preprocess_clip(const b2_preprocess_plan* pl, void* stream) {
    B2_CHECK_ARG(pl != nullptr, "b2_op_preprocess_clip: null plan");
    PreprocessArgs a;
    a.img = pl->img; a.H = pl->H; a.W = pl->W; a.pad_top = pl->pad_top; a.pad_left = pl->pad_left;
    for (int i = 0; i < 3; ++i) { a.bg[i] = pl->bg[i]; a.mean[i] = pl->mean[i]; a.stdv[i] = pl->stdv[i]; }
    a.h_bounds = pl->h_bounds; a.h_kk = pl->h_kk; a.h_ksize = pl->h_ksize; a.h_identity = pl->h_identity;
    a.v_bounds = pl->v_bounds; a.v_kk = pl->v_kk; a.v_ksize = pl->v_ksize; a.v_identity = pl->v_identity;
    a.y0 = pl->y0; a.rows = pl->rows; a.x_lo = pl->x_lo; a.y_lo = pl->y_lo; a.cols = pl->out; a.out = pl->out;
    a.tmp = pl->tmp; a.rescale = pl->rescale; a.pixels = pl->pixels; a.u8_out = pl->u8_out;
    return preprocess_clip_image(a, reinterpret_cast<cudaStream_t>(stream));
}

int b2_op_sample(const float* logits, int B, int V, const b2_sampling* sp, int index, int32_t* out_tokens, void* stream) {
    B2_CHECK_ARG(logits && out_tokens && B >= 1 && V >= 1 && index >= 0, "b2_op_sample: bad argument");
    SampleState v = {};
    v.temperature = 1.f; v.top_p = 1.f;
    if (sp != nullptr && sp->do_sample) {
        B2_CHECK_ARG(sp->temperature > 0.f && sp->top_p > 0.f && sp->top_p <= 1.f && sp->top_k >= 0, "b2_op_sample: bad sampling parameters");
        v.do_sample = 1; v.temperature = sp->temperature; v.top_p = sp->top_p; v.top_k = sp->top_k; v.seed = sp->seed;
    }
    v.pub_counter = index;
    cudaStream_t st = reinterpret_cast<cudaStream_t>(stream);
    DevBuf tmp;
    B2_TRY(tmp.alloc(sizeof(SampleState) + 64));
    int r = sample_state_set(tmp.as<SampleState>(), v, st);
    if (r == 0)
        r = sample_publish(logits, V, B, tmp.as<SampleState>(), nullptr, out_tokens, nullptr, nullptr, nullptr, nullptr, 0, SP_SELECT, 0, st);
    cudaError_t e = cudaStreamSynchronize(st);
    tmp.free();
    if (r != 0) return r;
    B2_CUDA_CHECK(e);
    return 0;
}

int b2_argmax(const float* logits, int B, int V, int32_t* out, void* stream) {
    B2_CHECK_ARG(logits && out, "b2_argmax: null argument");
    return argmax_f32(logits, B, V, out, reinterpret_cast<cudaStream_t>(stream));
}

int b2_op_gemm(const void* A, int lda, const void* W, int ldw, const void* bias, const void* residual, int ld_res,
               void* out, int ld_out, int out_fp32, int M, int N, int K, int act, int bn_override, void* stream) {
    B2_CHECK_ARG(A && W && out, "b2_op_gemm: null argument");
    GemmArgs g;
    g.A = A; g.lda = lda; g.W = W; g.ldw = ldw; g.bias = bias; g.residual = residual; g.ld_res = ld_res;
    g.out = out; g.ld_out = ld_out; g.out_fp32 = out_fp32; g.M = M; g.N = N; g.K = K; g.act = act;
    g.bn_override = bn_override;
    return gemm_bf16(g, reinterpret_cast<cudaStream_t>(stream));
}

int b2_op_gemv(const void* x, int64_t ldx, const void* W, int ldw, const void* norm_gamma, float eps,
               const void* residual, int ld_res, void* out, int ld_out, int out_fp32, int B, int N, int K, int act,
               void* stream) {
    B2_CHECK_ARG(x && W && out, "b2_op_gemv: null argument");
    return gemv(x, ldx, W, ldw, norm_gamma, eps, residual, ld_res, out, ld_out, out_fp32, B, N, K, act,
                reinterpret_cast<cudaStream_t>(stream));
}

int b2_op_quantize_nf4(const void* w, int N, int K, void* codes, float* absmax, void* stream) {
    return quantize_nf4(w, K, N, K, codes, absmax, 0, reinterpret_cast<cudaStream_t>(stream));
}

int b2_op_dequantize_nf4(const void* codes, const float* absmax, int N, int K, void* out, void* stream) {
    Nf4Matrix mt;
    mt.q = codes; mt.absmax = absmax; mt.out = out; mt.N = N; mt.K = K;
    return dequantize_nf4(&mt, 1, 0, reinterpret_cast<cudaStream_t>(stream));
}

int b2_op_gemv_nf4(const void* x, int64_t ldx, const void* codes, const float* absmax, const void* norm_gamma, float eps,
                   const void* residual, int ld_res, void* out, int ld_out, int B, int N, int K, int act, void* stream) {
    B2_CHECK_ARG(x && codes && absmax && out, "b2_op_gemv_nf4: null argument");
    GemvArgs g;
    g.x = x; g.ldx = ldx; g.norm_gamma = norm_gamma; g.eps = eps; g.residual = residual; g.ld_res = ld_res;
    g.out = out; g.ld_out = ld_out; g.B = B; g.N = N; g.K = K; g.act = act;
    return gemv_nf4(g, codes, absmax, reinterpret_cast<cudaStream_t>(stream));
}

int b2_op_gemm_skinny(const void* x, int ldx, const void* W, int ldw, const void* residual, int ld_res, void* out,
                      int ld_out, int out_fp32, int B, int N, int K, int act, void* workspace, int64_t workspace_bytes,
                      void* counters, void* stream) {
    B2_CHECK_ARG(x && W && out && workspace && counters, "b2_op_gemm_skinny: null argument");
    SkinnyArgs g;
    g.x = x; g.ldx = ldx; g.W = W; g.ldw = ldw; g.residual = residual; g.ld_res = ld_res;
    g.out = out; g.ld_out = ld_out; g.out_fp32 = out_fp32; g.B = B; g.N = N; g.K = K; g.act = act;
    g.partial = reinterpret_cast<float*>(workspace); g.partial_bytes = (size_t)workspace_bytes;
    g.counters = reinterpret_cast<int*>(counters);
    return gemm_skinny_bf16(g, reinterpret_cast<cudaStream_t>(stream));
}
int b2_op_gemm_skinny_fp8(const void* xq, int ldx, const float* x_scale, const void* Wq, int ldw, const float* w_scale,
                          const void* residual, int ld_res, void* out, int ld_out, int out_fp32, int B, int N, int K, int act,
                          void* workspace, int64_t workspace_bytes, void* counters, void* stream) {
    B2_CHECK_ARG(xq && Wq && x_scale && w_scale && out && workspace && counters, "b2_op_gemm_skinny_fp8: null argument");
    SkinnyArgs g;
    g.x = xq; g.ldx = ldx; g.W = Wq; g.ldw = ldw; g.residual = residual; g.ld_res = ld_res;
    g.out = out; g.ld_out = ld_out; g.out_fp32 = out_fp32; g.B = B; g.N = N; g.K = K; g.act = act;
    g.partial = reinterpret_cast<float*>(workspace); g.partial_bytes = (size_t)workspace_bytes;
    g.counters = reinterpret_cast<int*>(counters);
    g.w_scale = w_scale; g.x_scale = x_scale;
    return gemm_skinny_fp8(g, reinterpret_cast<cudaStream_t>(stream));
}
int b2_op_quantize_rows_e4m3(const void* x, int64_t ldx, int rows, int K, void* q, int64_t ldq, float* scale, void* stream) {
    B2_CHECK_ARG(x && q && scale, "b2_op_quantize_rows_e4m3: null argument");
    return quantize_rows_e4m3(x, ldx, rows, K, q, ldq, scale, reinterpret_cast<cudaStream_t>(stream));
}
int b2_op_rmsnorm_quant_e4m3(const void* x, const void* gamma, void* q, float* scale, int rows, int cols, float eps,
                             void* stream) {
    B2_CHECK_ARG(x && gamma && q && scale, "b2_op_rmsnorm_quant_e4m3: null argument");
    return rmsnorm_quant_e4m3(x, cols, gamma, q, cols, scale, rows, cols, eps, reinterpret_cast<cudaStream_t>(stream));
}
int64_t b2_op_gemm_skinny_workspace_bytes(int B, int N, int K) {
    if (B < 1 || B > 128 || N < 1 || K < 1) return -1;
    return (int64_t)gemm_skinny_workspace_bytes(B, N, K);
}
int64_t b2_op_gemm_skinny_counter_bytes(int N) { return N < 1 ? -1 : (int64_t)gemm_skinny_counter_bytes(N); }

int b2_op_layernorm(const void* x, const void* gamma, const void* beta, void* y, int rows, int cols, float eps,
                    void* stream) {
    B2_CHECK_ARG(x && gamma && beta && y, "b2_op_layernorm: null argument");
    return layernorm_bf16(x, gamma, beta, y, rows, cols, eps, reinterpret_cast<cudaStream_t>(stream));
}

int b2_op_rmsnorm(const void* x, const void* gamma, void* y, int rows, int cols, float eps, void* stream) {
    B2_CHECK_ARG(x && gamma && y, "b2_op_rmsnorm: null argument");
    return rmsnorm_bf16(x, cols, gamma, y, rows, cols, eps, reinterpret_cast<cudaStream_t>(stream));
}

int b2_op_flash_attn(const void* q, const void* k, const void* v, void* o, const int32_t* seq_lens, int B, int S,
                     int H, int D, int causal, float scale, void* stream) {
    B2_CHECK_ARG(q && k && v && o, "b2_op_flash_attn: null argument");
    FlashArgs fa;
    const int64_t ts = (int64_t)H * D, bs = (int64_t)S * H * D;
    fa.q = q; fa.q_bs = bs; fa.q_ts = ts; fa.q_hs = D;
    fa.k = k; fa.k_bs = bs; fa.k_ts = ts; fa.k_hs = D;
    fa.v = v; fa.v_bs = bs; fa.v_ts = ts; fa.v_hs = D;
    fa.o = o; fa.o_bs = bs; fa.o_ts = ts; fa.o_hs = D;
    fa.seq_lens = seq_lens; fa.B = B; fa.H = H; fa.S = S; fa.D = D; fa.causal = causal; fa.scale = scale;
    return flash_attn_bf16(fa, reinterpret_cast<cudaStream_t>(stream));
}

int b2_op_rope_kv_write(void* qkv, void* kcache, void* vcache, int B, int S, int H, int D, int Smax, float theta,
                        void* stream) {
    B2_CHECK_ARG(qkv && kcache && vcache, "b2_op_rope_kv_write: null argument");
    return rope_kv_write(qkv, kcache, vcache, B, S, H, D, Smax, theta, reinterpret_cast<cudaStream_t>(stream));
}

int64_t b2_op_decode_attn_scratch_bytes(int B, int H, int nsplit) {
    return (int64_t)B * H * 4  + 256 + (int64_t)B * H * nsplit * (128 + 2) * 4;
}

int b2_op_decode_attn(const void* qkv, void* kcache, void* vcache, const int32_t* cur_len, void* out, void* scratch,
                      int B, int H, int Smax, int nsplit, float theta, float scale, void* stream) {
    B2_CHECK_ARG(qkv && kcache && vcache && cur_len && out && scratch, "b2_op_decode_attn: null argument");
    DecodeAttnArgs da;
    da.qkv = qkv; da.kcache = kcache; da.vcache = vcache; da.cur_len = cur_len; da.out = out;
    da.counters = reinterpret_cast<int32_t*>(scratch);
    const size_t off = ((size_t)B * H * 4 + 255) / 256 * 256;
    da.partial = reinterpret_cast<float*>(reinterpret_cast<uint8_t*>(scratch) + off);
    da.B = B; da.H = H; da.D = 128; da.Smax = Smax; da.nsplit = nsplit; da.theta = theta; da.scale = scale;
    return decode_attn_bf16(da, reinterpret_cast<cudaStream_t>(stream));
}

int b2_op_decode_attn_e4m3(const void* qkv, void* k8, void* v8, float* kscale, float* vscale, const int32_t* cur_len, void* out,
                           void* scratch, int B, int H, int Smax, int nsplit, float theta, float scale, void* stream) {
    B2_CHECK_ARG(qkv && k8 && v8 && kscale && vscale && cur_len && out && scratch, "b2_op_decode_attn_e4m3: null argument");
    DecodeAttnArgs da;
    da.qkv = qkv; da.kcache = k8; da.vcache = v8; da.kscale = kscale; da.vscale = vscale; da.cur_len = cur_len; da.out = out;
    da.counters = reinterpret_cast<int32_t*>(scratch);
    da.partial = reinterpret_cast<float*>(reinterpret_cast<char*>(scratch) + (((size_t)B * H * 4 + 255) / 256) * 256);
    da.B = B; da.H = H; da.D = 128; da.Smax = Smax; da.nsplit = nsplit; da.theta = theta; da.scale = scale;
    return decode_attn_e4m3(da, reinterpret_cast<cudaStream_t>(stream));
}

int b2_op_decode_attn_nsplit(int B, int H, int Smax, int kv_dtype) {
    B2_CHECK_ARG(B >= 1 && H >= 1 && Smax >= 1, "b2_op_decode_attn_nsplit: bad shape");
    B2_CHECK_ARG(kv_dtype == B2_KV_BF16 || kv_dtype == B2_KV_E4M3, "b2_op_decode_attn_nsplit: unknown kv_dtype %d", kv_dtype);
    return decode_nsplit(B, H, Smax, kv_dtype == B2_KV_E4M3 ? decode_attn_e4m3_ctas_per_sm() : decode_attn_ctas_per_sm());
}

int b2_op_kv_quantize_e4m3(const void* kstage, const void* vstage, void* k8, void* v8, float* kscale, float* vscale,
                           const int32_t* seq_lens, int B, int S, int H, int Smax, void* stream) {
    B2_CHECK_ARG(kstage && vstage && k8 && v8 && kscale && vscale, "b2_op_kv_quantize_e4m3: null argument");
    return kv_quantize_e4m3(kstage, vstage, k8, v8, kscale, vscale, seq_lens, B, S, H, 128, Smax, reinterpret_cast<cudaStream_t>(stream));
}

int b2_op_flash_attn_kv(const void* q, const void* kcache, const void* vcache, void* o, const int32_t* pos0, const int32_t* seq_lens,
                        int B, int S, int H, int Smax, float scale, void* stream) {
    B2_CHECK_ARG(q && kcache && vcache && o && pos0, "b2_op_flash_attn_kv: null argument");
    B2_CHECK_ARG(B >= 1 && S >= 1 && H >= 1 && Smax >= 1, "b2_op_flash_attn_kv: bad shape B=%d S=%d H=%d Smax=%d", B, S, H, Smax);
    const int D = 128;
    FlashArgs fa;
    fa.q = q; fa.q_bs = (int64_t)S * H * D; fa.q_ts = (int64_t)H * D; fa.q_hs = D;
    fa.k = kcache; fa.k_bs = (int64_t)H * Smax * D; fa.k_ts = D; fa.k_hs = (int64_t)Smax * D;
    fa.v = vcache; fa.v_bs = fa.k_bs; fa.v_ts = D; fa.v_hs = fa.k_hs;
    fa.o = o; fa.o_bs = fa.q_bs; fa.o_ts = fa.q_ts; fa.o_hs = D;
    fa.seq_lens = seq_lens; fa.pos0 = pos0; fa.Skv = Smax;
    fa.B = B; fa.H = H; fa.S = S; fa.D = D; fa.causal = 1; fa.scale = scale;
    return flash_attn_bf16(fa, reinterpret_cast<cudaStream_t>(stream));
}

int b2_op_rope_kv_write_at(void* qkv, void* kcache, void* vcache, const int32_t* pos0, int B, int S, int H, int D, int Smax,
                           float theta, void* stream) {
    B2_CHECK_ARG(qkv && kcache && vcache && pos0, "b2_op_rope_kv_write_at: null argument");
    return rope_kv_write(qkv, kcache, vcache, B, S, H, D, Smax, theta, reinterpret_cast<cudaStream_t>(stream), pos0);
}

int b2_op_kv_dequantize_e4m3(const void* k8, const void* v8, const float* kscale, const float* vscale, const int32_t* pos0,
                             void* kdst, void* vdst, int B, int H, int Smax, int S_dst, void* stream) {
    return kv_dequantize_e4m3(k8, v8, kscale, vscale, pos0, kdst, vdst, B, H, Smax, S_dst, reinterpret_cast<cudaStream_t>(stream));
}

int b2_op_kv_quantize_e4m3_at(const void* kstage, const void* vstage, void* k8, void* v8, float* kscale, float* vscale,
                              const int32_t* pos0, const int32_t* seq_lens, int B, int S, int S_src, int H, int Smax, void* stream) {
    B2_CHECK_ARG(kstage && vstage && k8 && v8 && kscale && vscale && pos0, "b2_op_kv_quantize_e4m3_at: null argument");
    B2_CHECK_ARG(S_src >= 1, "b2_op_kv_quantize_e4m3_at: S_src=%d", S_src);
    return kv_quantize_e4m3(kstage, vstage, k8, v8, kscale, vscale, seq_lens, B, S, H, 128, Smax, reinterpret_cast<cudaStream_t>(stream),
                            pos0, S_src);
}

int b2_op_interleave_gate_up(const void* gate, const void* up, void* out, int I, int h, void* stream) {
    B2_CHECK_ARG(gate && up && out, "b2_op_interleave_gate_up: null argument");
    return interleave_gate_up(gate, up, out, I, h, reinterpret_cast<cudaStream_t>(stream));
}

int b2_op_im2col(const void* pixels, void* out, int B, int img, int patch, int kpad, void* stream) {
    B2_CHECK_ARG(pixels && out, "b2_op_im2col: null argument");
    return vit_im2col(pixels, out, B, img, patch, kpad, reinterpret_cast<cudaStream_t>(stream));
}

}
```

Measured before the change: 724.1.

## Stream attention KV through producer ring and replace post-QKV grid barrier with per-head readiness

Attention in the decode megakernel now reads K/V tiles from the shared-memory ring filled by the producer warps, replacing direct streaming global loads. The grid barrier after the QKV phase is removed and replaced by per-head release counters, so each attention CTA waits only for the CTAs that wrote its head's Q/K/V rows. The change also drops the L2-prefetch and slow-prologue options, always uses the register-based gamma preload, and adds per-CTA tracing. The aim is to overlap KV fetch with compute and cut one global barrier per layer. The costs are tighter constraints (B*H must fit within the CTA count), extra counter state keyed on a launch sequence, and more complex producer scheduling.

```diff
diff --git a/llava-plus-codebase_b200/csrc/decode_mega.cu b/llava-plus-codebase_b200/csrc/decode_mega.cu
--- a/llava-plus-codebase_b200/csrc/decode_mega.cu
+++ b/llava-plus-codebase_b200/csrc/decode_mega.cu
@@ -12,7 +12,8 @@
 constexpr int MK_PROD_WARPS = 4;
 constexpr int MK_THREADS = MK_CONS + 32 * MK_PROD_WARPS;
 constexpr int MK_D = 128;
-constexpr int MK_U = 4;
+constexpr int MK_KX = 4;
+constexpr int MK_KWARP_BYTES = MK_KX * MK_D * 2 * 2;
 constexpr int MK_KT = 2048;
 constexpr int MK_ROW_PAD = 64;
 constexpr int MK_ROW_STRIDE = MK_KT * 2 + MK_ROW_PAD;
@@ -20,6 +21,8 @@
 constexpr int MK_MAXNB = 32;
 constexpr int MK_MAXL = 48;
 constexpr int MK_MAX_STAGES = 12;
+constexpr int MK_TRACE = 8;
+static_assert(MK_CONS_WARPS * MK_KWARP_BYTES <= MK_TILE_BYTES, "an attention round must fit one ring slot");
 
 __device__ __forceinline__ void unpack8(const uint4& u, float (&f)[8]) {
     f[0] = bf16_lo(u.x); f[1] = bf16_hi(u.x); f[2] = bf16_lo(u.y); f[3] = bf16_hi(u.y);
@@ -29,17 +32,26 @@
 
 __device__ __forceinline__ void cons_sync() { asm volatile("bar.sync 1, %0;" ::"n"(MK_CONS) : "memory"); }
 
+__device__ __forceinline__ void wait_counter(const unsigned int* counter, unsigned int target) {
+    unsigned int cur, spins = 0;
+    do {
+        asm volatile("ld.acquire.gpu.global.u32 %0, [%1];" : "=r"(cur) : "l"(counter) : "memory");
+        if (++spins > (1u << 26)) asm volatile("trap;");
+    } while ((int)(cur - target) < 0);
+}
 __device__ __forceinline__ void grid_sync(unsigned int* counter, unsigned int target) {
     cons_sync();
     if (threadIdx.x == 0) {
         asm volatile("red.release.gpu.global.add.u32 [%0], 1;" ::"l"(counter) : "memory");
-        unsigned int cur, spins = 0;
-        do {
-            asm volatile("ld.acquire.gpu.global.u32 %0, [%1];" : "=r"(cur) : "l"(counter) : "memory");
-            if (++spins > (1u << 26)) asm volatile("trap;");
-        } while ((int)(cur - target) < 0);
+        wait_counter(counter, target);
     }
     cons_sync();
+}
+
+__device__ __forceinline__ unsigned long long globaltimer_ns() {
+    unsigned long long t;
+    asm volatile("mov.u64 %0, %%globaltimer;" : "=l"(t));
+    return t;
 }
 
 __device__ __forceinline__ void bulk_g2s(void* smem_dst, const void* gsrc, uint32_t bytes, uint64_t* bar) {
@@ -113,63 +125,7 @@
 }
 
 template <int NB>
-__device__ __forceinline__ void mk_prologue(const PhaseIO& c, int K, int B, float eps, int tid, int lane, int warp,
-                                            __nv_bfloat16* xs, float (*s_red)[NB], float* s_rstd,
-                                            const __nv_bfloat16* gamma_smem) {
-    const int nvec = K >> 3;
-    float ss[NB];
-#pragma unroll
-    for (int b = 0; b < NB; ++b) ss[b] = 0.f;
-    for (int i = tid; i < nvec; i += MK_CONS) {
-#pragma unroll
-        for (int b = 0; b < NB; ++b) {
-            uint4 u = make_uint4(0, 0, 0, 0);
-            if (b < B) u = ldcg16(c.xin + (size_t)b * K + i * 8);
-            *reinterpret_cast<uint4*>(xs + (size_t)b * K + i * 8) = u;
-            if (c.gamma != nullptr) {
-                float f[8];
-                unpack8(u, f);
-#pragma unroll
-                for (int e = 0; e < 8; ++e) ss[b] += f[e] * f[e];
-            }
-        }
-    }
-    if (c.gamma != nullptr) {
-#pragma unroll
-        for (int b = 0; b < NB; ++b) {
-            const float v = warp_sum(ss[b]);
-            if (lane == 0) s_red[warp][b] = v;
-        }
-        cons_sync();
-        if (tid < NB) {
-            float t = 0.f;
-            for (int i = 0; i < MK_CONS_WARPS; ++i) t += s_red[i][tid];
-            s_rstd[tid] = rsqrtf(t / K + eps);
-        }
-        cons_sync();
-        if (gamma_smem != nullptr) asm volatile("cp.async.wait_all;" ::: "memory");
-        const __nv_bfloat16* gsrc = gamma_smem != nullptr ? gamma_smem : c.gamma;
-        for (int i = tid; i < nvec; i += MK_CONS) {
-            float gf[8];
-            unpack8(*reinterpret_cast<const uint4*>(gsrc + i * 8), gf);
-#pragma unroll
-            for (int b = 0; b < NB; ++b) {
-                uint4* px = reinterpret_cast<uint4*>(xs + (size_t)b * K + i * 8);
-                float f[8], o[8];
-                unpack8(*px, f);
-                const float rstd = s_rstd[b];
-#pragma unroll
-                for (int e = 0; e < 8; ++e) o[e] = gf[e] * round_bf16(f[e] * rstd);
-                *px = make_uint4(pack_bf16(o[0], o[1]), pack_bf16(o[2], o[3]), pack_bf16(o[4], o[5]),
-                                 pack_bf16(o[6], o[7]));
-            }
-        }
-    }
-    cons_sync();
-}
-
-template <int NB>
-__device__ __forceinline__ void mk_prologue_fast(const PhaseIO& c, int K, float eps, int tid, int lane, int warp,
+__device__ __forceinline__ void mk_prologue(const PhaseIO& c, int K, float eps, int tid, int lane, int warp,
                                                  __nv_bfloat16* xs, float (*s_red)[NB], const uint4 (&gpre)[2]) {
     const int nvec = K >> 3;
     if (c.gamma == nullptr) {
@@ -250,18 +206,17 @@
     cons_sync();
 }
 
-__device__ __forceinline__ bool mk_gamma_preload(const MegaParams& p, const MegaLayer* layers, int ph, int n_phases,
+__device__ __forceinline__ void mk_gamma_preload(const MegaParams& p, const MegaLayer* layers, int ph, int n_phases,
                                                  int tid, uint4 (&gpre)[2]) {
-    if (ph >= n_phases || mk_is_attention(p, ph)) return false;
+    if (ph >= n_phases || mk_is_attention(p, ph)) return;
     const PhaseIO io = mk_phase_io(p, layers, ph);
     const int nvec = p.h >> 3;
-    if (io.gamma == nullptr || nvec > 2 * MK_CONS) return false;
+    if (io.gamma == nullptr) return;
 #pragma unroll
     for (int j = 0; j < 2; ++j) {
         const int idx = j * MK_CONS + tid;
         gpre[j] = idx < nvec ? __ldg(reinterpret_cast<const uint4*>(io.gamma) + idx) : make_uint4(0, 0, 0, 0);
     }
-    return true;
 }
 
 __device__ __forceinline__ void mk_mma(float (&c)[4], uint32_t a0, uint32_t a2, uint32_t b0, uint32_t b1) {
@@ -306,26 +261,71 @@
     }
 }
 
-__device__ __forceinline__ void mk_attention(const MegaParams& p, const MegaLayer& Lw, int tid, int lane, int warp,
-                                             float (*s_part)[MK_D + 2], int* s_flag, const float* s_cos,
-                                             const float* s_sin) {
+struct AttnSpan {
+    int b, head, split, G;
+    int pos;
+    int cb, ce;
+    int wchunk;
+    int rounds;
+};
+__device__ __forceinline__ bool mk_attn_span(const MegaParams& p, const int* s_len, AttnSpan& a) {
+    const int pairs = p.B * p.H;
+    a.G = (int)gridDim.x / pairs;
+    const int pair = (int)blockIdx.x / a.G;
+    if (pair >= pairs) return false;
+    a.split = (int)blockIdx.x % a.G;
+    a.head = pair % p.H; a.b = pair / p.H;
+    a.pos = s_len[a.b];
+    const int total = a.pos + 1;
+    const int cchunk = (total + a.G - 1) / a.G;
+    a.cb = a.split * cchunk;
+    a.ce = min(a.cb + cchunk, total);
+    a.wchunk = (max(a.ce - a.cb, 0) + MK_CONS_WARPS - 1) / MK_CONS_WARPS;
+    a.rounds = (a.wchunk + MK_KX - 1) / MK_KX;
+    return true;
+}
+
+__device__ __forceinline__ int mk_qkv_owner(int r, int N) {
+    return (int)(((long long)(r + 1) * gridDim.x + N - 1) / N) - 1;
+}
+__device__ __forceinline__ unsigned int mk_head_writers(const MegaParams& p, int head) {
+    const int N = 3 * p.h;
+    unsigned int n = 0;
+#pragma unroll
+    for (int s = 0; s < 3; ++s) {
+        const int r0 = s * p.h + head * MK_D;
+        n += (unsigned int)(mk_qkv_owner(r0 + MK_D - 1, N) - mk_qkv_owner(r0, N) + 1);
+    }
+    return n;
+}
+__device__ __forceinline__ void mk_signal_heads(const MegaParams& p, const GemvCtx& c, int tid) {
+    cons_sync();
+    if (tid == 0 && c.nu > 0) {
+        for (int j = c.u_lo / MK_D; j <= (c.u_lo + c.nu - 1) / MK_D; ++j)
+            asm volatile("red.release.gpu.global.add.u32 [%0], 1;" ::"l"(p.head_ready + j % p.H) : "memory");
+    }
+}
+
+__device__ __forceinline__ void mk_attention(const MegaParams& p, const MegaLayer& Lw, int l, const AttnSpan& a, int tid,
+                                             int lane, int warp, float (*s_part)[MK_D + 2], int* s_flag,
+                                             const float* s_cos, const float* s_sin, const uint8_t* ring,
+                                             uint64_t* full_bar, uint64_t* empty_bar, int n_stages, uint32_t& tile,
+                                             long long* tr) {
     const int h = p.h, H = p.H;
-    const int pairs = p.B * H;
-    const int grid = gridDim.x;
-    const int G = pairs <= grid ? grid / pairs : 1;
+    const int G = a.G;
     const int hw = lane >> 4, c = lane & 15;
-    const int split = pairs <= grid ? (int)blockIdx.x % G : 0;
-    for (int pair = pairs <= grid ? (int)blockIdx.x / G : (int)blockIdx.x; pair < pairs;
-         pair += (pairs <= grid ? pairs : grid)) {
-        const int head = pair % H, b = pair / H;
-        const int pos = p.cur_len[b];
-        const int total = pos + 1;
-        const int cchunk = (total + G - 1) / G;
-        const int cb = split * cchunk;
-        const int ce = min(cb + cchunk, total);
-        const int wchunk = (max(ce - cb, 0) + MK_CONS_WARPS - 1) / MK_CONS_WARPS;
+    const int split = a.split;
+    {
+        const int head = a.head, b = a.b;
+        const int pos = a.pos;
+        const int cb = a.cb, ce = a.ce, wchunk = a.wchunk;
         const int k_begin = cb + warp * wchunk;
         const int k_end = min(k_begin + wchunk, ce);
+        const int pair = b * H + head;
+        if (tid == 0)
+            wait_counter(p.head_ready + head, (p.launch_seq * (unsigned int)p.L + (unsigned int)l + 1u) * mk_head_writers(p, head));
+        cons_sync();
+        if (tr != nullptr && tid == 0) tr[1] = clock64();
         const __nv_bfloat16* qrow = p.qkv + (size_t)b * 3 * h + head * MK_D;
         float qreg[8], knew[8], vnew[8];
         {
@@ -356,23 +356,30 @@
         float m_run = -INFINITY, l_run = 0.f, av[8];
 #pragma unroll
         for (int e = 0; e < 8; ++e) av[e] = 0.f;
-        const __nv_bfloat16* kb_ = Lw.kcache + cbase + c * 8;
-        const __nv_bfloat16* vb_ = Lw.vcache + cbase + c * 8;
-        for (int kbase = k_begin; kbase < k_end; kbase += 2 * MK_U) {
-            uint4 kraw[MK_U], vraw[MK_U];
-#pragma unroll
-            for (int u = 0; u < MK_U; ++u) {
-                const int key = kbase + hw + 2 * u;
+        const uint8_t* kv_w = ring + (size_t)warp * MK_KWARP_BYTES + c * 16;
+#pragma unroll 1
+        for (int r = 0; r < a.rounds; ++r, ++tile) {
+            const uint32_t stage = tile % (uint32_t)n_stages;
+            const int kbase = k_begin + r * MK_KX;
+            const uint8_t* slot = kv_w + (size_t)stage * MK_TILE_BYTES;
+            mbar_wait(&full_bar[stage], (tile / (uint32_t)n_stages) & 1u);
+            uint4 kraw[2], vraw[2];
+#pragma unroll
+            for (int u = 0; u < 2; ++u) {
+                const int j = hw + 2 * u;
+                const int key = kbase + j;
                 if (key < k_end && key != pos) {
-                    kraw[u] = ld_stream_16(kb_ + (size_t)key * MK_D);
-                    vraw[u] = ld_stream_16(vb_ + (size_t)key * MK_D);
+                    kraw[u] = *reinterpret_cast<const uint4*>(slot + j * (MK_D * 2));
+                    vraw[u] = *reinterpret_cast<const uint4*>(slot + (MK_KX + j) * (MK_D * 2));
                 } else {
                     kraw[u] = make_uint4(0, 0, 0, 0);
                     vraw[u] = make_uint4(0, 0, 0, 0);
                 }
             }
-#pragma unroll
-            for (int u = 0; u < MK_U; ++u) {
+            __syncwarp();
+            if (lane == 0) mbar_arrive(&empty_bar[stage]);
+#pragma unroll
+            for (int u = 0; u < 2; ++u) {
                 const int key = kbase + hw + 2 * u;
                 float kf[8], vf[8];
                 unpack8(kraw[u], kf);
@@ -400,6 +407,7 @@
                 }
             }
         }
+        if (tr != nullptr && tid == 0) tr[2] = clock64();
         {
             const float m_o = __shfl_xor_sync(0xffffffffu, m_run, 16);
             const float l_o = __shfl_xor_sync(0xffffffffu, l_run, 16);
@@ -470,35 +478,36 @@
     GemvCtx c;
     int ph, rb, kc;
     uint32_t tile;
-    bool valid;
+    bool valid, attn;
 };
-__device__ __forceinline__ void cursor_seek(TileCursor& t, const MegaParams& p, const MegaLayer* layers, int n_phases) {
+__device__ __forceinline__ void cursor_seek(TileCursor& t, const MegaParams& p, const MegaLayer* layers, int n_phases,
+                                            int attn_rounds) {
     while (t.ph < n_phases) {
-        if (!mk_is_attention(p, t.ph)) {
+        t.rb = 0; t.kc = 0;
+        t.attn = mk_is_attention(p, t.ph);
+        if (t.attn) {
+            if (attn_rounds > 0) { t.c.nb = attn_rounds; t.c.nchunk = 1; t.valid = true; return; }
+        } else {
             t.c = mk_phase_ctx(p, layers, t.ph);
-            if (t.c.nb > 0) { t.rb = 0; t.kc = 0; t.valid = true; return; }
+            if (t.c.nb > 0) { t.valid = true; return; }
         }
         ++t.ph;
     }
     t.valid = false;
 }
-__device__ __forceinline__ void cursor_begin(TileCursor& t, const MegaParams& p, const MegaLayer* layers, int n_phases) {
-    t.ph = 0; t.tile = 0; t.rb = 0; t.kc = 0;
-    cursor_seek(t, p, layers, n_phases);
-}
-__device__ __forceinline__ void cursor_next(TileCursor& t, const MegaParams& p, const MegaLayer* layers, int n_phases) {
+__device__ __forceinline__ void cursor_begin(TileCursor& t, const MegaParams& p, const MegaLayer* layers, int n_phases,
+                                             int attn_rounds) {
+    t.ph = 0; t.tile = 0;
+    cursor_seek(t, p, layers, n_phases, attn_rounds);
+}
+__device__ __forceinline__ void cursor_next(TileCursor& t, const MegaParams& p, const MegaLayer* layers, int n_phases,
+                                            int attn_rounds) {
     ++t.tile;
     if (++t.kc < t.c.nchunk) return;
     t.kc = 0;
     if (++t.rb < t.c.nb) return;
     ++t.ph;
-    cursor_seek(t, p, layers, n_phases);
-}
-__device__ __forceinline__ void prefetch_l2_line(const void* gsrc) {
-    asm volatile("prefetch.global.L2 [%0];" ::"l"(gsrc) : "memory");
-}
-__device__ __forceinline__ void bulk_prefetch_l2(const void* gsrc, uint32_t bytes) {
-    asm volatile("cp.async.bulk.prefetch.L2.global [%0], %1;" ::"l"(gsrc), "r"(bytes) : "memory");
+    cursor_seek(t, p, layers, n_phases, attn_rounds);
 }
 
 template <int NB>
@@ -510,13 +519,13 @@
     uint64_t* full_bar = reinterpret_cast<uint64_t*>(s_gpart + (size_t)MK_CONS_WARPS * MK_MAXNB * NB * 8);
     uint64_t* empty_bar = full_bar + MK_MAX_STAGES;
     __shared__ float s_red[MK_CONS_WARPS][NB];
-    __shared__ float s_rstd[NB];
     __shared__ float s_av[MK_CONS_WARPS];
     __shared__ int s_ai[MK_CONS_WARPS];
     __shared__ float s_part[MK_CONS_WARPS][MK_D + 2];
     __shared__ int s_flag;
     __shared__ float s_cos[NB * 64], s_sin[NB * 64];
     __shared__ __align__(16) MegaLayer s_layers[MK_MAXL];
+    __shared__ int s_len[NB];
 
     const int tid = threadIdx.x, lane = tid & 31, warp = tid >> 5;
     const int B = p.B;
@@ -526,6 +535,7 @@
         const uint4* src = reinterpret_cast<const uint4*>(p.layers);
         uint4* dst = reinterpret_cast<uint4*>(s_layers);
         for (int i = tid; i < p.L * (int)(sizeof(MegaLayer) / 16); i += MK_THREADS) dst[i] = src[i];
+        if (tid < B) s_len[tid] = p.cur_len[tid];
         if (tid == 0) {
             for (int s = 0; s < n_stages; ++s) {
                 mbar_init(&full_bar[s], 1);
@@ -535,51 +545,58 @@
         }
         __syncthreads();
     }
+    AttnSpan span;
+    const bool has_attn = mk_attn_span(p, s_len, span);
+    const int attn_rounds = has_attn ? span.rounds : 0;
+    long long* const trace_cta = p.trace != nullptr ? p.trace + (size_t)blockIdx.x * (n_phases + 1) * MK_TRACE : nullptr;
 
     if (warp >= MK_CONS_WARPS) {
         const uint32_t pw = (uint32_t)(warp - MK_CONS_WARPS);
-        const uint32_t ahead = (uint32_t)p.l2_ahead;
-        TileCursor cp, pf;
-        cursor_begin(cp, p, s_layers, n_phases);
-        cursor_begin(pf, p, s_layers, n_phases);
+        auto slot_wait = [&](uint32_t stage, uint32_t parity, int ph) {
+            const long long t0 = trace_cta != nullptr ? clock64() : 0;
+            mbar_wait(&empty_bar[stage], parity ^ 1u);
+            if (trace_cta != nullptr)
+                atomicAdd(reinterpret_cast<unsigned long long*>(&trace_cta[ph * MK_TRACE + 4]), (unsigned long long)(clock64() - t0));
+        };
+        TileCursor cp;
+        cursor_begin(cp, p, s_layers, n_phases, attn_rounds);
         while (cp.valid) {
             if (cp.tile % (uint32_t)MK_PROD_WARPS == pw) {
-                if (ahead != 0) {
-                    while (pf.valid && pf.tile < cp.tile + ahead) cursor_next(pf, p, s_layers, n_phases);
-                    if (pf.valid) {
-                        const uint32_t pbytes = (uint32_t)min(MK_KT, pf.c.K - pf.kc * MK_KT) * 2u;
-                        if (p.l2_mode == 2) {
-                            bool pvalid;
-                            const int pfrow = mk_phys_row(pf.c, pf.rb, lane & 7, pvalid);
-                            if (lane < 8 && pvalid)
-                                bulk_prefetch_l2(pf.c.W + (size_t)pfrow * pf.c.K + (size_t)pf.kc * MK_KT, pbytes);
-                        } else {
-                            bool pvalid;
-                            const int pfrow = mk_phys_row(pf.c, pf.rb, lane >> 2, pvalid);
-                            if (pvalid) {
-                                const char* base = reinterpret_cast<const char*>(pf.c.W + (size_t)pfrow * pf.c.K +
-                                                                                 (size_t)pf.kc * MK_KT);
-                                for (uint32_t off = (uint32_t)(lane & 3) * 128u; off < pbytes; off += 512u)
-                                    prefetch_l2_line(base + off);
-                            }
-                        }
-                    }
-                }
                 const uint32_t stage = cp.tile % (uint32_t)n_stages;
                 const uint32_t parity = (cp.tile / (uint32_t)n_stages) & 1u;
-                const uint32_t row_bytes = (uint32_t)min(MK_KT, cp.c.K - cp.kc * MK_KT) * 2u;
-                if (lane == 0) {
-                    mbar_wait(&empty_bar[stage], parity ^ 1u);
-                    mbar_arrive_expect_tx(&full_bar[stage], (uint32_t)mk_rows_in_block(cp.c, cp.rb) * row_bytes);
+                uint8_t* slot = ring + (size_t)stage * MK_TILE_BYTES;
+                if (cp.attn) {
+                    const MegaLayer& Lw = s_layers[cp.ph / 5];
+                    const int kb = span.cb + lane * span.wchunk + cp.rb * MK_KX;
+                    const int ke = min(min(span.cb + (lane + 1) * span.wchunk, span.ce), span.pos);
+                    const int n = lane < MK_CONS_WARPS ? max(0, min(kb + MK_KX, ke) - kb) : 0;
+                    const int total = __reduce_add_sync(0xffffffffu, n);
+                    if (lane == 0) {
+                        slot_wait(stage, parity, cp.ph);
+                        mbar_arrive_expect_tx(&full_bar[stage], (uint32_t)total * (MK_D * 2u) * 2u);
+                    }
+                    __syncwarp();
+                    if (n > 0) {
+                        const size_t off = (((size_t)span.b * p.H + span.head) * p.Smax + kb) * MK_D;
+                        uint8_t* dst = slot + (size_t)lane * MK_KWARP_BYTES;
+                        bulk_g2s(dst, Lw.kcache + off, (uint32_t)n * (MK_D * 2u), &full_bar[stage]);
+                        bulk_g2s(dst + MK_KX * MK_D * 2, Lw.vcache + off, (uint32_t)n * (MK_D * 2u), &full_bar[stage]);
+                    }
+                } else {
+                    const uint32_t row_bytes = (uint32_t)min(MK_KT, cp.c.K - cp.kc * MK_KT) * 2u;
+                    if (lane == 0) {
+                        slot_wait(stage, parity, cp.ph);
+                        mbar_arrive_expect_tx(&full_bar[stage], (uint32_t)mk_rows_in_block(cp.c, cp.rb) * row_bytes);
+                    }
+                    __syncwarp();
+                    bool row_valid;
+                    const int prow = mk_phys_row(cp.c, cp.rb, lane & 7, row_valid);
+                    if (lane < 8 && row_valid)
+                        bulk_g2s(slot + (size_t)lane * MK_ROW_STRIDE, cp.c.W + (size_t)prow * cp.c.K + (size_t)cp.kc * MK_KT,
+                                 row_bytes, &full_bar[stage]);
                 }
-                __syncwarp();
-                bool row_valid;
-                const int prow = mk_phys_row(cp.c, cp.rb, lane & 7, row_valid);
-                if (lane < 8 && row_valid)
-                    bulk_g2s(ring + (size_t)stage * MK_TILE_BYTES + (size_t)lane * MK_ROW_STRIDE,
-                             cp.c.W + (size_t)prow * cp.c.K + (size_t)cp.kc * MK_KT, row_bytes, &full_bar[stage]);
-            }
-            cursor_next(cp, p, s_layers, n_phases);
+            }
+            cursor_next(cp, p, s_layers, n_phases, attn_rounds);
         }
         return;
     }
@@ -588,7 +605,7 @@
         const int b = i >> 6, f = i & 63;
         const float inv_freq = exp2f(-(2.0f * f / MK_D) * log2f(p.theta));
         float sv, cv;
-        sincosf((float)p.cur_len[b] * inv_freq, &sv, &cv);
+        sincosf((float)s_len[b] * inv_freq, &sv, &cv);
         s_cos[i] = round_bf16(cv);
         s_sin[i] = round_bf16(sv);
     }
@@ -600,30 +617,23 @@
         for (int i = tid; i < p.h / 8; i += MK_CONS) dst[i] = src[i];
     }
     uint4 gpre[2] = {make_uint4(0, 0, 0, 0), make_uint4(0, 0, 0, 0)};
-    bool gpre_ok = p.fast_prologue != 0 && mk_gamma_preload(p, s_layers, 0, n_phases, tid, gpre);
-    __nv_bfloat16* gsm = xs + (size_t)NB * p.h;
-    const bool gsm_fits = p.gamma_smem != 0 && (size_t)(NB + 1) * p.h <= (size_t)NB * (p.h > p.I ? p.h : p.I);
-    auto gamma_prefetch = [&](int ph) -> bool {
-        if (!gsm_fits || ph >= n_phases || mk_is_attention(p, ph)) return false;
-        const PhaseIO io = mk_phase_io(p, s_layers, ph);
-        if (io.gamma == nullptr) return false;
-        for (int i = tid; i < (p.h >> 3); i += MK_CONS)
-            asm volatile("cp.async.cg.shared.global [%0], [%1], 16;" ::"r"(smem_u32(gsm + i * 8)), "l"(io.gamma + i * 8) : "memory");
-        asm volatile("cp.async.commit_group;" ::: "memory");
-        return true;
-    };
-    bool gsm_ok = gamma_prefetch(0);
+    mk_gamma_preload(p, s_layers, 0, n_phases, tid, gpre);
     unsigned int bar_target = p.bar_base + gridDim.x;
     grid_sync(p.bar_count, bar_target);
 
-    const bool tracing = p.trace != nullptr && blockIdx.x == 0 && tid == 0;
+    const bool tracing = trace_cta != nullptr && tid == 0;
+    if (tracing) trace_cta[n_phases * MK_TRACE + 1] = (long long)globaltimer_ns();
     const int g = lane >> 2, t4 = lane & 3;
     uint32_t tile = 0;
 #pragma unroll 1
     for (int ph = 0; ph < n_phases; ++ph) {
-        if (tracing) p.trace[ph * 4 + 0] = clock64();
+        long long* const tr = tracing ? trace_cta + ph * MK_TRACE : nullptr;
+        const bool qkv = ph % 5 == 0 && ph < 5 * p.L;
+        if (tracing) tr[0] = clock64();
         if (mk_is_attention(p, ph)) {
-            mk_attention(p, s_layers[ph / 5], tid, lane, warp, s_part, &s_flag, s_cos, s_sin);
+            if (has_attn)
+                mk_attention(p, s_layers[ph / 5], ph / 5, span, tid, lane, warp, s_part, &s_flag, s_cos, s_sin, ring,
+                             full_bar, empty_bar, n_stages, tile, tr);
         } else {
             const GemvCtx c = mk_phase_ctx(p, s_layers, ph);
             const PhaseIO io = mk_phase_io(p, s_layers, ph);
@@ -633,11 +643,8 @@
                 const int b = tid / c.nu, r = tid - b * c.nu;
                 res_pref = __bfloat162float(__ldcg(io.residual + (size_t)b * io.ld_out + (size_t)c.u_lo + r));
             }
-            if (p.fast_prologue != 0 && (io.gamma == nullptr || gpre_ok))
-                mk_prologue_fast<NB>(io, c.K, p.eps, tid, lane, warp, xs, s_red, gpre);
-            else
-                mk_prologue<NB>(io, c.K, B, p.eps, tid, lane, warp, xs, s_red, s_rstd, gsm_ok ? gsm : nullptr);
-            if (tracing) p.trace[ph * 4 + 1] = clock64();
+            mk_prologue<NB>(io, c.K, p.eps, tid, lane, warp, xs, s_red, gpre);
+            if (tracing) tr[1] = clock64();
 #pragma unroll 1
             for (int rb = 0; rb < c.nb; ++rb) {
                 float acc[4] = {0.f, 0.f, 0.f, 0.f}, acc2[4] = {0.f, 0.f, 0.f, 0.f};
@@ -665,16 +672,21 @@
                         make_float2(acc[0] + acc2[0], acc[1] + acc2[1]);
             }
             cons_sync();
-            if (tracing) p.trace[ph * 4 + 2] = clock64();
+            if (tracing) tr[2] = clock64();
             mk_epilogue<NB>(p, s_layers, ph, c, B, tid, s_gpart, res_pref, have_res);
-        }
-        if (tracing) p.trace[ph * 4 + 3] = clock64();
-        gpre_ok = p.fast_prologue != 0 && mk_gamma_preload(p, s_layers, ph + 1, n_phases, tid, gpre);
-        gsm_ok = gamma_prefetch(ph + 1);
-        bar_target += gridDim.x;
-        grid_sync(p.bar_count, bar_target);
-    }
-    if (tracing) p.trace[n_phases * 4] = clock64();
+            if (qkv) mk_signal_heads(p, c, tid);
+        }
+        if (tracing) tr[3] = clock64();
+        mk_gamma_preload(p, s_layers, ph + 1, n_phases, tid, gpre);
+        if (!qkv) {
+            bar_target += gridDim.x;
+            grid_sync(p.bar_count, bar_target);
+        }
+    }
+    if (tracing) {
+        trace_cta[n_phases * MK_TRACE + 0] = clock64();
+        trace_cta[n_phases * MK_TRACE + 2] = (long long)globaltimer_ns();
+    }
 
     if (blockIdx.x < B) {
         const int b = blockIdx.x;
@@ -746,6 +758,8 @@
 
 bool decode_mega_fits(int B, int h, int I) {
     if (B < 1 || B > 2) return false;
+    if (B * (h / MK_D) > num_sms()) return false;
+    if (h / 8 > 2 * MK_CONS) return false;
     return mega_stages(B, h, I) >= 4;
 }
 
@@ -754,6 +768,9 @@
     B2_CHECK_ARG(p.L <= MK_MAXL, "decode_mega: %d layers exceed the shared layer table (%d)", p.L, MK_MAXL);
     B2_CHECK_ARG(p.h % 256 == 0 && p.I % 256 == 0 && p.V % 8 == 0 && p.h / p.H == MK_D,
                  "decode_mega: unsupported dims h=%d I=%d V=%d H=%d", p.h, p.I, p.V, p.H);
+    B2_CHECK_ARG(p.B * p.H <= num_sms(), "decode_mega: %d (sample, head) pairs exceed the %d CTAs", p.B * p.H, num_sms());
+    B2_CHECK_ARG(p.head_ready != nullptr, "decode_mega: no head-readiness counters");
+    B2_CHECK_ARG(p.h / 8 <= 2 * MK_CONS, "decode_mega: hidden size %d exceeds the prologue's RMSNorm registers", p.h);
     {
         const int grid = num_sms();
         const int nmax = p.V > 3 * p.h ? (p.V > 2 * p.I ? p.V : 2 * p.I) : (3 * p.h > 2 * p.I ? 3 * p.h : 2 * p.I);
diff --git a/llava-plus-codebase_b200/csrc/kernels.h b/llava-plus-codebase_b200/csrc/kernels.h
--- a/llava-plus-codebase_b200/csrc/kernels.h
+++ b/llava-plus-codebase_b200/csrc/kernels.h
@@ -145,11 +145,9 @@
     int32_t* attn_counters = nullptr;
     unsigned int *bar_count = nullptr, *done_count = nullptr;
     unsigned int bar_base = 0;
+    unsigned int* head_ready = nullptr;
+    unsigned int launch_seq = 0;
     float eps = 1e-5f, theta = 10000.f, scale_log2 = 1.f;
-    int l2_ahead = 0;
-    int l2_mode = 1;
-    int fast_prologue = 0;
-    int gamma_smem = 0;
     long long* trace = nullptr;
     struct SampleState* sstate = nullptr;
     int32_t* ring = nullptr;
diff --git a/llava-plus-codebase_b200/csrc/model.cu b/llava-plus-codebase_b200/csrc/model.cu
--- a/llava-plus-codebase_b200/csrc/model.cu
+++ b/llava-plus-codebase_b200/csrc/model.cu
@@ -124,6 +124,7 @@
     cudaGraphExec_t graph = nullptr;
     int graph_B = 0;
     unsigned int mega_bar_base = 0;
+    unsigned int mega_launches = 0;
     DevBuf mega_layers, mega_sync;
     DevBuf rope_tab;
     cudaStream_t own_stream = nullptr;
@@ -641,9 +642,6 @@
     return flag == 1;
 }
 
-constexpr int kMegaL2AheadDefault = 0;
-constexpr int kMegaFastPrologueDefault = 0;
-
 int decode_step_mega(b2_model* m, b2_kv* kv, int B, cudaStream_t st) {
     const b2_model_desc& d = m->d;
     MegaParams p;
@@ -658,51 +656,48 @@
     p.logits = m->logits.as<float>();
     p.attn_partial = kv->attn_partial.as<float>(); p.attn_counters = kv->attn_counters.as<int32_t>();
     unsigned int* sync = kv->mega_sync.as<unsigned int>();
-    p.bar_count = sync; p.done_count = sync + 2;
+    p.bar_count = sync; p.done_count = sync + 2; p.head_ready = sync + 16;
     p.bar_base = kv->mega_bar_base;
-    kv->mega_bar_base += (unsigned int)(5 * d.layers + 2) * (unsigned int)num_sms();
+    p.launch_seq = kv->mega_launches;
     p.eps = d.rms_eps; p.theta = d.rope_theta;
     p.scale_log2 = (1.0f / sqrtf((float)m->hd)) * 1.4426950408889634f;
     const bool sampling = kv->samp_host.do_sample != 0 || kv->samp_host.per_row != 0;
     if (!sampling && kv->samp_host.tag != 0) { p.sstate = kv->sstate.as<SampleState>(); p.ring = kv->ring_dev; p.ring_cap = kv->ring_cap; }
     if (kv->samp_host.per_row) p.rows = kv->rows_dev.as<RowState>();
-    {
-        const char* e = getenv("B2_MEGA_L2_AHEAD");
-        int ahead = e ? atoi(e) : kMegaL2AheadDefault;
-        p.l2_ahead = ahead < 0 ? 0 : (ahead > 64 ? 64 : ahead) / 4 * 4;
-        e = getenv("B2_MEGA_L2_MODE");
-        p.l2_mode = (e && e[0] == '2') ? 2 : 1;
-        e = getenv("B2_MEGA_FAST_PROLOGUE");
-        p.fast_prologue = e ? (e[0] != '0') : kMegaFastPrologueDefault;
-        e = getenv("B2_MEGA_GAMMA_SMEM");
-        p.gamma_smem = e ? (e[0] != '0') : 1;
-    }
     static int trace_mode = -1;
     if (trace_mode < 0) { const char* e = getenv("B2_MEGA_TRACE"); trace_mode = (e && e[0] != 0) ? 1 : 0; }
-    if (trace_mode == 1) {
-        static int steps_seen = 0;
-        if (++steps_seen == 40) {
-            const int n = (5 * d.layers + 2) * 4;
-            DevBuf tb;
-            B2_TRY(tb.alloc((size_t)n * 8));
-            cudaMemset(tb.p, 0, (size_t)n * 8);
-            p.trace = tb.as<long long>();
-            int r = decode_mega(p, st);
-            cudaStreamSynchronize(st);
-            std::vector<long long> host(n);
-            cudaMemcpy(host.data(), tb.p, (size_t)n * 8, cudaMemcpyDeviceToHost);
-            FILE* f = fopen(getenv("B2_MEGA_TRACE"), "w");
-            if (f) {
-                for (int ph = 0; ph <= 5 * d.layers; ++ph)
-                    fprintf(f, "%d %lld %lld %lld %lld %lld\n", ph, host[ph * 4], host[ph * 4 + 1], host[ph * 4 + 2],
-                            host[ph * 4 + 3], host[(ph + 1) * 4]);
-                fclose(f);
+    static int steps_seen = 0;
+    const bool trace_step = trace_mode == 1 && ++steps_seen == 40;
+    const int grid = num_sms(), n_phases = 5 * d.layers + 1, per_cta = (n_phases + 1) * 8;
+    DevBuf tb;
+    if (trace_step) {
+        B2_TRY(tb.alloc((size_t)grid * per_cta * 8));
+        cudaMemset(tb.p, 0, (size_t)grid * per_cta * 8);
+        p.trace = tb.as<long long>();
+    }
+    const int r = decode_mega(p, st);
+    if (r == 0) {
+        kv->mega_bar_base += (unsigned int)(4 * d.layers + 2) * (unsigned int)grid;
+        kv->mega_launches++;
+    }
+    if (trace_step) {
+        std::vector<long long> host((size_t)grid * per_cta);
+        cudaStreamSynchronize(st);
+        cudaMemcpy(host.data(), tb.p, host.size() * 8, cudaMemcpyDeviceToHost);
+        tb.free();
+        FILE* f = r == 0 ? fopen(getenv("B2_MEGA_TRACE"), "w") : nullptr;
+        if (f) {
+            for (int c = 0; c < grid; ++c) {
+                const long long* t = host.data() + (size_t)c * per_cta;
+                for (int ph = 0; ph < n_phases; ++ph)
+                    fprintf(f, "P %d %d %lld %lld %lld %lld %lld %lld\n", c, ph, t[ph * 8], t[ph * 8 + 1], t[ph * 8 + 2],
+                            t[ph * 8 + 3], t[(ph + 1) * 8], t[ph * 8 + 4]);
+                fprintf(f, "T %d %lld %lld %lld\n", c, t[n_phases * 8], t[n_phases * 8 + 1], t[n_phases * 8 + 2]);
             }
-            tb.free();
-            return r;
-        }
-    }
-    B2_TRY(decode_mega(p, st));
+            fclose(f);
+        }
+    }
+    B2_TRY(r);
     if (sampling)
         B2_TRY(sample_publish(m->logits.as<float>(), d.vocab, B, kv->sstate.as<SampleState>(), kv->rows_dev.as<RowState>(), kv->tok.as<int32_t>(),
                               kv->out_tokens.as<int32_t>(), kv->step_counter.as<int32_t>(), kv->len_dev.as<int32_t>(),
@@ -1132,12 +1127,13 @@
             tbl[l].kcache = reinterpret_cast<bf16*>(kv->k_layer(l));
             tbl[l].vcache = reinterpret_cast<bf16*>(kv->v_layer(l));
         }
-        if ((r = kv->mega_layers.alloc(tbl.size() * sizeof(MegaLayer))) != 0 || (r = kv->mega_sync.alloc(64)) != 0) {
+        const size_t sync_bytes = 64 + (size_t)m->d.heads * 4;
+        if ((r = kv->mega_layers.alloc(tbl.size() * sizeof(MegaLayer))) != 0 || (r = kv->mega_sync.alloc(sync_bytes)) != 0) {
             b2_kv_destroy(kv);
             return r;
         }
         cudaMemcpy(kv->mega_layers.p, tbl.data(), tbl.size() * sizeof(MegaLayer), cudaMemcpyHostToDevice);
-        cudaMemset(kv->mega_sync.p, 0, 64);
+        cudaMemset(kv->mega_sync.p, 0, sync_bytes);
     }
     if ((r = kv->out_tokens.alloc((size_t)kv->out_capacity * max_batch * 4)) != 0 ||
         (r = kv->attn_partial.alloc(((size_t)max_batch * m->d.heads * max_split + 1024) * (128 + 2) * 4)) != 0 ||
```

Result: faster. 735.8, median of 6 (+1.6%).
